# danihae/bio-image-unet

Hardware: AMD Instinct MI355X
Metric: voxels/sec fwd+bwd (higher is better)
Workload: dtype bf16; 1 GPU; cfg4: UNet3D(in_channels=1, out_channels=1, n_filter=32) input (4, 1, 128, 128, 128) per GPU, train step = forward + reference loss + backward + Adam; parallelism=dp1

## Files before the change

bio_image_unet_amd/_lib.py:

```python
from __future__ import annotations

import ctypes as C
import os

import torch

_HERE = os.path.dirname(os.path.abspath(__file__))
LIB_PATH = os.environ.get("BIU_LIB_PATH") or os.path.join(_HERE, "libbiu_hip.so")

BIU_F32, BIU_BF16 = 0, 1
BN_MAX_PARTIALS = 1024


class BiuError(RuntimeError):
    pass


class biu_act(C.Structure):
    _fields_ = [("p", C.c_void_p), ("n", C.c_int32), ("d", C.c_int32), ("h", C.c_int32), ("w", C.c_int32),
                ("c", C.c_int32), ("pitch", C.c_int32)]


class biu_pack_job(C.Structure):
    _fields_ = [("w", C.c_void_p), ("packed", C.c_void_p), ("transposed", C.c_int32), ("kind", C.c_int32), ("cin", C.c_int32),
                ("cout", C.c_int32), ("kd", C.c_int32), ("kh", C.c_int32), ("kw", C.c_int32), ("reserved", C.c_int32)]


class biu_xform(C.Structure):
    _fields_ = [("scale", C.c_void_p), ("shift", C.c_void_p), ("slope", C.c_void_p)]


class biu_mo2d_term(C.Structure):
    _fields_ = [("kind", C.c_int32), ("nb", C.c_int32), ("partial_off", C.c_longlong), ("numel", C.c_longlong), ("pixels", C.c_longlong),
                ("p0", C.c_float), ("p1", C.c_float), ("p2", C.c_float), ("weight", C.c_float)]


class biu_aug_params(C.Structure):
    _fields_ = [("flags", C.c_uint32), ("rot_k", C.c_uint32), ("blur_k", C.c_uint32), ("index", C.c_uint32), ("m", C.c_double * 6),
                ("alpha", C.c_float), ("beta", C.c_float), ("noise_a", C.c_float), ("noise_b", C.c_float),
                ("angle", C.c_float), ("scale", C.c_float), ("dx", C.c_float), ("dy", C.c_float)]


class biu_augf_params(C.Structure):
    _fields_ = [("flags", C.c_uint32), ("rot_k", C.c_uint32), ("blur_k", C.c_uint32), ("index", C.c_uint32), ("m", C.c_double * 6),
                ("cos_t", C.c_float), ("sin_t", C.c_float), ("alpha", C.c_float), ("beta", C.c_float), ("shot_s", C.c_float),
                ("gauss_sigma", C.c_float), ("angle", C.c_float), ("scale", C.c_float), ("dx", C.c_float), ("dy", C.c_float)]


_P = C.c_void_p
_A = C.POINTER(biu_act)
_X = C.POINTER(biu_xform)
_I = C.c_int
_F = C.c_float
_D = C.c_double
_Z = C.c_size_t

SIGNATURES = {
    "biu_last_error": (C.c_char_p, []),
    "biu_version": (_I, []),
    "biu_set_fp32_products": (_I, [_I]),
    "biu_set_fp32_products_3d": (_I, [_I]),
    "biu_conv_packed_bytes": (_Z, [_I, _I, _I, _I, _I, _I, _I, _I]),
    "biu_conv_pack": (_I, [_I, _P, _I, _I, _I, _I, _I, _I, _P, _P]),
    "biu_pack_batch": (_I, [_P, _I, _I, _P]),
    "biu_conv_split_workspace": (_Z, [_I, _A, _A, _I, _I, _I, _I, _I]),
    "biu_conv_fwd": (_I, [_A, _X, _P, _P, _P, _I, _I, _I, _I, _A, _P, _Z, _I, _P]),
    "biu_conv_fwd_stats_floats": (_Z, [_A, _I]),
    "biu_conv_fwd_stats": (_I, [_A, _X, _P, _P, _P, _I, _I, _I, _I, _A, _P, _Z, C.POINTER(C.c_int), _P, _Z, _I, _P]),
    "biu_conv_bwd_data": (_I, [_A, _P, _P, _I, _I, _I, _I, _A, _I, _P, _Z, _I, _P]),
    "biu_bwd_data_bnred_floats": (_Z, [_A, _I, _I]),
    "biu_conv_bwd_data_bnred": (_I, [_A, _P, _P, _I, _I, _I, _I, _A, _A, _P, _P, _P, _P, _P, _P, _Z, C.POINTER(C.c_int), _P, _Z, _I, _P]),
    "biu_convt_bwd_data_bnred": (_I, [_A, _P, _P, _I, _A, _A, _P, _P, _P, _P, _P, _P, _Z, C.POINTER(C.c_int), _I, _P]),
    "biu_conv_bwd_weight_workspace": (_Z, [_I, _I, _I, _I, _I, _I]),
    "biu_conv_bwd_weight": (_I, [_A, _X, _A, _I, _I, _I, _I, _P, _P, _P, _Z, _I, _P]),
    "biu_conv_bwd_weight_bn": (_I, [_A, _X, _A, _A, _P, _P, _P, _P, _P, _P, _I, _I, _I, _I, _P, _P, _Z, _I, _P]),
    "biu_bn_stats": (_I, [_A, _P, C.POINTER(C.c_int), _I, _P]),
    "biu_bn_finalize": (_I, [_P, _I, _I, _D, _P, _P, _P, _P, _F, _F, _P, _P, _P, _P, _P]),
    "biu_bn_eval_affine": (_I, [_I, _P, _P, _P, _P, _F, _P, _P, _P]),
    "biu_xform_apply": (_I, [_A, _X, _A, _I, _P]),
    "biu_bn_bwd_reduce": (_I, [_A, _A, _P, _P, _P, _P, _P, _P, C.POINTER(C.c_int), _I, _P]),
    "biu_bn_bwd_finalize": (_I, [_P, _I, _I, _D, _P, _P, _P, _P, _P, _P, _P, _P, _P]),
    "biu_bn_bwd_finalize_eval": (_I, [_P, _I, _I, _P, _P, _P, _P, _P, _P, _P, _P]),
    "biu_bn_bwd_apply": (_I, [_A, _A, _P, _P, _P, _P, _P, _P, _A, _I, _P]),
    "biu_maxpool_fwd": (_I, [_A, _X, _A, _I, _P]),
    "biu_maxpool_bwd": (_I, [_A, _X, _A, _A, _I, _I, _P]),
    "biu_maxpool_bwd_bnred": (_I, [_A, _X, _A, _A, _I, _P, _P, _P, _Z, C.POINTER(C.c_int), _I, _P]),
    "biu_nearest_down_fwd": (_I, [_A, _X, _A, _I, _P]),
    "biu_nearest_down_bwd": (_I, [_A, _A, _I, _I, _P]),
    "biu_nearest_up_fwd": (_I, [_A, _X, _A, _I, _P]),
    "biu_upconv_ok": (_I, [_A, _A, _I]),
    "biu_upconv_packed_bytes": (_Z, [_I, _I, _I, _I]),
    "biu_upconv_pack": (_I, [_I, _P, _I, _I, _I, _P, _P]),
    "biu_upconv_bwd_data": (_I, [_A, _P, _A, _I, _I, _P]),
    "biu_upconv_bwd_weight_workspace": (_Z, [_I, _I, _I]),
    "biu_upconv_bwd_weight_bn": (_I, [_A, _X, _A, _A, _P, _P, _P, _P, _P, _P, _P, _P, _Z, _I, _P]),
    "biu_upconv_fwd_stats_floats": (_Z, [_A, _A]),
    "biu_upconv_fwd": (_I, [_A, _X, _P, _P, _A, _P, _Z, C.POINTER(C.c_int), _I, _P]),
    "biu_nearest_up_bwd": (_I, [_A, _A, _I, _I, _P]),
    "biu_bce_dice_blocks": (_I, [C.c_longlong]),
    "biu_bce_dice_fwd": (_I, [_P, _P, _I, C.c_longlong, _P, _P]),
    "biu_bce_dice_bwd": (_I, [_P, _P, _I, C.c_longlong, _P, _P, _I, _P]),
    "biu_pair_smooth_l1_blocks": (_I, [C.c_longlong]),
    "biu_pair_smooth_l1_fwd": (_I, [_P, _I, C.c_longlong, _P, _P]),
    "biu_pair_smooth_l1_bwd": (_I, [_P, _I, C.c_longlong, _P, _P, _I, _P]),
    "biu_seg_loss_finish": (_I, [_P, _I, _I, C.c_longlong, _P, _I, _F, _F, _F, _I, _F, _F, _F, _I, _F, _P, _P]),
    "biu_seg_loss_coef": (_I, [_P, _P, _I, C.c_longlong, _F, _F, _F, _I, _F, _F, _F, _I, _F, _P, _P, _P]),
    "biu_head_dlogits": (_I, [_P, _P, _P, _I, _I, _I, C.c_longlong, _P, _I, _I, _P]),
    "biu_mo2d_loss_blocks": (_I, [C.c_longlong]),
    "biu_mo2d_loss_fwd": (_I, [_I, _F, _F, _P, _I, _P, _I, _I, _I, _I, _P, _P]),
    "biu_mo2d_loss_finish": (_I, [_P, _I, _P, _P, _P]),
    "biu_mo2d_loss_coef": (_I, [_P, _I, _P, _P, _P, _P]),
    "biu_mo2d_loss_bwd": (_I, [_I, _F, _F, _P, _I, _P, _I, _I, _I, _I, _P, _P, _P]),
    "biu_trilinear_up_fwd": (_I, [_A, _X, _A, _I, _P]),
    "biu_trilinear_up_bwd": (_I, [_A, _A, _I, _I, _P]),
    "biu_bilinear_up_fwd": (_I, [_A, _X, _A, _I, _P]),
    "biu_bilinear_up_bwd": (_I, [_A, _A, _I, _I, _P]),
    "biu_xcorr_fwd": (_I, [_A, _X, _A, _X, _A, _I, _P]),
    "biu_xcorr_bwd": (_I, [_A, _X, _A, _X, _A, _A, _A, _I, _I, _P]),
    "biu_conv_cat_ok": (_I, [_A, _A, _A, _I, _I, _I, _I, _I]),
    "biu_conv_fwd_cat": (_I, [_A, _X, _A, _X, _P, _P, _P, _I, _I, _I, _I, _A, _P, _Z, C.POINTER(C.c_int), _P, _Z, _I, _P]),
    "biu_conv_bwd_data_cat": (_I, [_A, _P, _P, _I, _I, _I, _I, _A, _I, _A, _I, _P, _Z, _I, _P]),
    "biu_conv_bwd_weight_cat": (_I, [_A, _X, _A, _X, _A, _A, _P, _P, _P, _P, _P, _P, _I, _I, _I, _I, _P, _P, _Z, _I, _P]),
    "biu_convt_packed_bytes": (_Z, [_I, _I, _I, _I, _I]),
    "biu_convt_pack": (_I, [_I, _P, _I, _I, _I, _I, _P, _P]),
    "biu_foldt_ok": (_I, [_A, _A, _A, _I]),
    "biu_foldt_packed_bytes": (_Z, [_I, _I, _I, _I]),
    "biu_foldt_pack": (_I, [_P, _P, _P, _P, _I, _I, _I, _I, _I, _P, _P]),
    "biu_foldt_fwd_stats_floats": (_Z, [_A, _A]),
    "biu_foldt_fwd_form": (_I, [_A, _A, _A, _I]),
    "biu_foldt_fwd": (_I, [_A, _X, _A, _X, _P, _A, _P, _Z, C.POINTER(C.c_int), _I, _P]),
    "biu_foldt_bwd_data_bnred_floats": (_Z, [_A]),
    "biu_foldt_bwd_data": (_I, [_A, _P, _A, _I, _A, _I, _A, _P, _P, _P, _P, _P, _P, _Z, C.POINTER(C.c_int), _P, _Z, _I, _P]),
    "biu_foldt_bwd_weight_workspace": (_Z, [_I, _I, _I, _I]),
    "biu_foldt_bwd_weight_bn": (_I, [_A, _X, _A, _X, _A, _A, _P, _P, _P, _P, _P, _P, _P, _P, _P, _P, _I, _P, _P, _P, _P, _Z, _I, _P]),
    "biu_foldt_bwd_weight_bn_phase": (_I, [_A, _X, _A, _X, _A, _A, _P, _P, _P, _P, _P, _P, _P, _P, _P, _P, _I, _P, _P, _P, _P, _Z, _I, _I, _P]),
    "biu_convt_fwd": (_I, [_A, _X, _P, _P, _P, _I, _A, _I, _P]),
    "biu_convt_bwd_data": (_I, [_A, _P, _P, _I, _A, _I, _I, _P]),
    "biu_convt_bwd_weight_workspace": (_Z, [_I, _I, _I, _I]),
    "biu_convt_bwd_weight": (_I, [_A, _X, _A, _I, _P, _P, _P, _Z, _I, _P]),
    "biu_head_fwd": (_I, [_A, _X, _P, _P, _I, _I, _P, _P, _I, _P]),
    "biu_head_bwd_workspace": (_Z, [_I]),
    "biu_head_bwd": (_I, [_A, _X, _P, _I, _P, _A, _P, _P, _P, _Z, _I, _P]),
    "biu_head_bwd_bnred": (_I, [_A, _X, _P, _I, _P, _A, _P, _P, _P, _Z, _P, _P, _P, _Z, C.POINTER(C.c_int), _I, _P]),
    "biu_max_join_fwd": (_I, [_A, _X, _A, _X, _A, _I, _P]),
    "biu_max_join_bwd": (_I, [_A, _X, _A, _X, _A, _A, _A, _I, _I, _P]),
    "biu_act_add": (_I, [_A, _A, _I, _I, _P]),
    "biu_add_relu_fwd": (_I, [_A, _X, _A, _X, _A, _I, _P]),
    "biu_add_relu_bwd": (_I, [_A, _A, _A, _A, _I, _I, _P]),
    "biu_gate_fwd": (_I, [_A, _X, _A, _X, _A, _I, _P]),
    "biu_gate_bwd": (_I, [_A, _X, _A, _X, _A, _A, _I, _A, _I, _P]),
    "biu_from_nchw": (_I, [_P, _A, _I, _P]),
    "biu_from_nchw_u8": (_I, [_P, _F, _A, _I, _P]),
    "biu_u8_to_f32": (_I, [_P, _F, _P, C.c_longlong, _P]),
    "biu_quantize_u8": (_I, [_P, _F, _P, C.c_longlong, _P]),
    "biu_stitch_add": (_I, [_P, _I, _P, _I, _I, _I, _I, _P, _P, _I, _I, _I, _I, _I, _I, _I, _P]),
    "biu_stitch_finish": (_I, [_P, _P, _I, _I, C.c_longlong, _P, _I, _P]),
    "biu_to_nchw": (_I, [_A, _X, _P, _I, _P]),
    "biu_augment_u8": (_I, [_P, _P, _I, _I, _I, _I, _I, _P, _I, _I, C.c_ulonglong, C.c_uint, C.c_uint, _P]),
    "biu_augment_f32": (_I, [_P, _I, _P, _I, _I, _I, _I, _I, _P, _I, C.c_ulonglong, C.c_uint, C.c_uint, _P]),
    "biu_philox_u32": (_I, [_P, C.c_longlong, C.c_ulonglong, C.c_uint, C.c_uint, C.c_uint, C.c_uint, _P]),
    "biu_adam_step": (_I, [_I, _P, _P, _P, _P, _P, _F, _F, _F, _F, _I, _F, _P]),
    "biu_adam_set_hyper": (_I, [_P, _F, _F, _F, _F, _I, _F, _P]),
    "biu_adam_step_hyper": (_I, [_I, _P, _P, _P, _P, _P, _P, _P]),
    "biu_grad_clip_scratch_floats": (_Z, [_I]),
    "biu_grad_clip": (_I, [_I, _P, _P, _F, _P, _Z, _P, _P]),
}


def _load():
    if not os.path.exists(LIB_PATH):
        raise ImportError(
            f"{LIB_PATH} is missing: the HIP kernels are not built. Run `python -c 'import __graft_entry__ as g; "
            f"g.build()'` from the repository root (needs hipcc). There is no CPU fallback.")
    lib = C.CDLL(LIB_PATH)
    for name, (res, args) in SIGNATURES.items():
        fn = getattr(lib, name)
        fn.restype = res
        fn.argtypes = args
    return lib


class _Lib:

    def __init__(self, cdll):
        object.__setattr__(self, "_c", cdll)
        object.__setattr__(self, "prof", None)
        object.__setattr__(self, "watch", None)
        object.__setattr__(self, "watched", [])
        object.__setattr__(self, "label", "")

    def __setattr__(self, k, v):
        object.__setattr__(self, k, v)

    def __getattr__(self, name):
        fn = getattr(self._c, name)
        if self.prof is None and self.watch is None:
            return fn
        if self.prof is None and self.watch != (name, self.label):
            return fn
        import torch

        def timed(*args):
            e0, e1 = torch.cuda.Event(enable_timing=True), torch.cuda.Event(enable_timing=True)
            e0.record()
            rc = fn(*args)
            e1.record()
            (self.prof if self.prof is not None else self.watched).append((name, self.label, e0, e1))
            return rc

        return timed


lib = _Lib(_load())


def check(status: int, what: str = ""):
    if status != 0:
        msg = lib.biu_last_error()
        raise BiuError(f"{what}: biu status {status}: {msg.decode() if msg else ''}")
```

bio_image_unet_amd/csrc/biu_api.hip:

```cpp
#include "biu_common.h"
#include "biu_internal.h"

#include <stdlib.h>
#include <string.h>

static const char* const kOffTokens[] = {
    "conv_fwd", "conv_dgrad", "conv_wgrad", "convt_fwd", "convt_dgrad", "convt_wgrad", "convt_all", "c1", "c1_mfma", "cat",
    "fused_stats", "wgrad_bn", "dgrad_bnred", "pool_pair", "pool_pipe", "pool_bnred", "head_bnred", "ksplit", "m16", "m16x2", "rr16",
    "wroll", "wroll16", "wroll2d", "upconv", "foldt", "foldall", "foldck8", "foldgemm", "croll", "froll", "prepack", "wsplitbn",
    "capturefork", "sidechain",
};
constexpr int kNumOffTokens = sizeof(kOffTokens) / sizeof(kOffTokens[0]);
static_assert(kNumOffTokens <= 64, "BiuEnv::off holds one bit per token");

static int off_index(const char* tok, size_t n) {
    for (int i = 0; i < kNumOffTokens; ++i)
        if (strlen(kOffTokens[i]) == n && strncmp(kOffTokens[i], tok, n) == 0) return i;
    return -1;
}
static void env_unknown(const char* var, const char* val, int n) {
    fprintf(stderr, "[biu] %s: unknown %s '%.*s' ignored\n", var, strcmp(var, "BIU_DISABLE") == 0 ? "token" : "value", n, val);
}
static bool parse_int(const char* s, int* v) {
    char* end = nullptr;
    const long r = strtol(s, &end, 10);
    if (end == s || *end) return false;
    *v = (int)r;
    return true;
}

const BiuEnv& biu_env() {
    static const BiuEnv env = [] {
        BiuEnv v{0, false, false, 0, 2, 0, 128};
        if (const char* p = getenv("BIU_DISABLE")) {
            while (true) {
                const size_t n = strcspn(p, ",");
                const int i = off_index(p, n);
                if (i >= 0) v.off |= 1ull << i;
                else if (n > 0) env_unknown("BIU_DISABLE", p, (int)n);
                if (!p[n]) break;
                p += n + 1;
            }
        }
        if (const char* e = getenv("BIU_ROLL"); e && *e) {
            if (strcmp(e, "always") == 0) v.roll_always = true;
            else env_unknown("BIU_ROLL", e, (int)strlen(e));
        }
        if (const char* e = getenv("BIU_FOLDT"); e && *e) {
            int n = 0;
            if (strcmp(e, "always") == 0) v.foldt_always = true;
            else if (strncmp(e, "cmax:", 5) == 0 && parse_int(e + 5, &n) && n > 0) v.foldt_cmax = n;
            else if (strcmp(e, "size") != 0) env_unknown("BIU_FOLDT", e, (int)strlen(e));
        }
        if (const char* e = getenv("BIU_FP32_PRODUCTS"); e && *e) {
            if (strcmp(e, "exact") == 0) v.fp32_products = 0;
            else if (strcmp(e, "bf16x3") == 0) v.fp32_products = 1;
            else if (strcmp(e, "bf16x6") != 0) env_unknown("BIU_FP32_PRODUCTS", e, (int)strlen(e));
        }
        if (const char* e = getenv("BIU_FP32_PRODUCTS_3D"); e && *e) {
            if (strcmp(e, "bf16x3") == 0) v.fp32_products_3d = 1;
            else if (strcmp(e, "bf16x6") == 0) v.fp32_products_3d = 2;
            else if (strcmp(e, "exact") != 0) env_unknown("BIU_FP32_PRODUCTS_3D", e, (int)strlen(e));
        }
        if (const char* e = getenv("BIU_FALL_MAXCA"); e && *e) {
            int n = 0;
            if (parse_int(e, &n)) v.fall_maxca = n;
            else env_unknown("BIU_FALL_MAXCA", e, (int)strlen(e));
        }
        return v;
    }();
    return env;
}

bool biu_off(const char* token) {
    const int i = off_index(token, strlen(token));
    return i >= 0 && ((biu_env().off >> i) & 1);
}

static void warn_slow_path(const char* op, const biu_act* x, const biu_act* y, int taps) {
    const double macs = (double)nvox(y) * x->c * y->c * taps;
    if (macs < 4e9) return;
    static int shown = 0;
    if (shown++ < 8)
        fprintf(stderr, "[biu] %s: %d->%d channels on %lld voxels takes the any-shape kernel (%.1f GMAC): expect it to be slow; "
                        "the MFMA path needs channel counts that are multiples of 8 (>= 16), dilation 1, 16-byte aligned slices "
                        "and samples under 4 GB\n", op, x->c, y->c, (long long)nvox(y), macs * 1e-9);
}

static bool conv_args_ok(const biu_act* x, const biu_act* y, int kd, int kh, int kw, int dil) {
    if (!valid_act(x) || !valid_act(y) || !same_space(x, y)) return false;
    if (!((kd == 1 || kd == 3) && kh == 3 && kw == 3) && !(kd == 1 && kh == 1 && kw == 1)) return false;
    return dil >= 1;
}

extern "C" size_t biu_conv_packed_bytes(int kind, int cin, int cout, int kd, int kh, int kw, int dilation, int dtype) {
    return biu_mfma_packed_bytes(kind, cin, cout, kd, kh, kw, dilation, dtype);
}

extern "C" int biu_conv_pack(int kind, const float* w, int cin, int cout, int kd, int kh, int kw, int dtype,
                             void* packed, biu_stream stream) {
    BIU_REQUIRE(w && packed, BIU_ERR_SHAPE, "conv_pack: null pointer");
    BIU_REQUIRE(biu_mfma_packed_bytes(kind, cin, cout, kd, kh, kw, 1, dtype) > 0, BIU_ERR_UNSUPPORTED,
                "conv_pack: shape (cin=%d, cout=%d, k=%dx%dx%d) is served by the direct kernels", cin, cout, kd, kh, kw);
    return biu_mfma_pack(kind, w, cin, cout, kd, kh, kw, dtype, packed, (hipStream_t)stream);
}

extern "C" int biu_pack_batch(const biu_pack_job* jobs, int n, int dtype, biu_stream stream) {
    BIU_REQUIRE(n >= 0 && (jobs || n == 0), BIU_ERR_SHAPE, "pack_batch: null job table");
    BIU_REQUIRE(n <= 65535, BIU_ERR_UNSUPPORTED, "pack_batch: more than 65535 jobs");
    return biu_mfma_pack_batch(jobs, n, dtype, (hipStream_t)stream);
}

static bool will_split(int cin, const biu_act* y, const biu_act* y1, int kd, int dtype, const void* ws, size_t ws_bytes) {
    const size_t need = biu_mfma_conv_split_bytes(cin, y, y1, kd, dtype);
    return need > 0 && ws && ws_bytes >= need;
}

extern "C" size_t biu_conv_split_workspace(int cin, const biu_act* y, const biu_act* y1, int kd, int kh, int kw, int dilation, int dtype) {
    if (!y || !valid_act(y) || (y1 && !valid_act(y1)) || kh != 3 || kw != 3 || (kd != 1 && kd != 3) || dilation != 1) return 0;
    biu_act xprobe = *y;
    xprobe.c = xprobe.pitch = cin;
    biu_act yall = *y;
    if (y1) yall.c = y->c + y1->c;
    if (!biu_mfma_conv_ok(&xprobe, &yall, kd, kh, kw, dilation, dtype)) return 0;
    return biu_mfma_conv_split_bytes(cin, y, y1, kd, dtype);
}

extern "C" int biu_conv_fwd_stats(const biu_act* x, const biu_xform* xf, const float* w, const void* packed,
                                  const float* bias, int kd, int kh, int kw, int dilation, const biu_act* y,
                                  float* bn_partial, size_t bn_partial_floats, int* bn_nblk, void* ws, size_t ws_bytes, int dtype,
                                  biu_stream stream) {
    BIU_REQUIRE(conv_args_ok(x, y, kd, kh, kw, dilation), BIU_ERR_SHAPE,
                "conv_fwd: x/y extents differ or unsupported kernel %dx%dx%d dil %d", kd, kh, kw, dilation);
    BIU_REQUIRE(w && bn_partial && bn_nblk, BIU_ERR_SHAPE, "conv_fwd_stats: null pointer");
    *bn_nblk = 0;
    if (!biu_off("c1") && !biu_off("fused_stats") && biu_c1m_ok(x, y, kd, kh, kw, dilation, dtype)) {
        const int nb = biu_c1m_fwd_rows(y, kd);
        if ((size_t)nb * y->c * 2 <= bn_partial_floats) {
            int rc = biu_c1m_fwd(x, xf, w, bias, kd, y, bn_partial, (hipStream_t)stream);
            if (rc == BIU_OK) *bn_nblk = nb;
            return rc;
        }
    }
    if (packed && !biu_off("conv_fwd") && !biu_off("fused_stats") && biu_mfma_conv_ok(x, y, kd, kh, kw, dilation, dtype) &&
        !will_split(x->c, y, nullptr, kd, dtype, ws, ws_bytes)) {
        const int nb = biu_mfma_conv_stat_rows(y, kd, x, dtype);
        if ((size_t)nb * y->c * 2 <= bn_partial_floats) {
            int rc = biu_mfma_conv(x, xf, packed, bias, kd, kh, kw, y, 0, bn_partial, dtype, (hipStream_t)stream);
            if (rc == BIU_OK) *bn_nblk = nb;
            return rc;
        }
    }
    int rc = biu_conv_fwd(x, xf, w, packed, bias, kd, kh, kw, dilation, y, ws, ws_bytes, dtype, stream);
    if (rc != BIU_OK) return rc;
    BIU_REQUIRE(bn_partial_floats >= (size_t)BIU_BN_MAX_PARTIALS * y->c * 2, BIU_ERR_WORKSPACE, "conv_fwd_stats: partial buffer too small");
    return biu_bn_stats(y, bn_partial, bn_nblk, dtype, stream);
}

extern "C" size_t biu_conv_fwd_stats_floats(const biu_act* y, int kd) {
    size_t a = (size_t)BIU_BN_MAX_PARTIALS * y->c * 2, b = (size_t)biu_mfma_conv_bricks(y, kd == 3 ? 3 : 1) * y->c * 2;
    return a > b ? a : b;
}

extern "C" int biu_conv_fwd(const biu_act* x, const biu_xform* xf, const float* w, const void* packed,
                            const float* bias, int kd, int kh, int kw, int dilation, const biu_act* y, void* ws, size_t ws_bytes,
                            int dtype, biu_stream stream) {
    BIU_REQUIRE(conv_args_ok(x, y, kd, kh, kw, dilation), BIU_ERR_SHAPE,
                "conv_fwd: x/y extents differ or unsupported kernel %dx%dx%d dil %d", kd, kh, kw, dilation);
    BIU_REQUIRE(w, BIU_ERR_SHAPE, "conv_fwd: null weight");
    if (!biu_off("c1") && biu_c1m_ok(x, y, kd, kh, kw, dilation, dtype))
        return biu_c1m_fwd(x, xf, w, bias, kd, y, nullptr, (hipStream_t)stream);
    if (!biu_off("c1") && biu_c1_conv_ok(x, y, kd, kh, kw, dilation, dtype))
        return biu_c1_conv_fwd(x, xf, w, bias, kd, y, dtype, (hipStream_t)stream);
    if (packed && !biu_off("conv_fwd") && biu_mfma_conv_ok(x, y, kd, kh, kw, dilation, dtype))
        return biu_mfma_conv(x, xf, packed, bias, kd, kh, kw, y, 0, nullptr, dtype, (hipStream_t)stream, nullptr, nullptr, ws, ws_bytes);
    warn_slow_path("conv_fwd", x, y, kd * kh * kw);
    return biu_conv_fwd_direct(x, xf, w, bias, kd, kh, kw, dilation, y, dtype, (hipStream_t)stream);
}

extern "C" int biu_conv_bwd_data(const biu_act* dy, const float* w, const void* packed, int kd, int kh, int kw,
                                 int dilation, const biu_act* dx, int accumulate, void* ws, size_t ws_bytes, int dtype, biu_stream stream) {
    BIU_REQUIRE(conv_args_ok(dy, dx, kd, kh, kw, dilation), BIU_ERR_SHAPE, "conv_bwd_data: dy/dx extents differ");
    BIU_REQUIRE(w, BIU_ERR_SHAPE, "conv_bwd_data: null weight");
    if (packed && !biu_off("conv_dgrad") && biu_mfma_conv_ok(dy, dx, kd, kh, kw, dilation, dtype))
        return biu_mfma_conv(dy, nullptr, packed, nullptr, kd, kh, kw, dx, accumulate, nullptr, dtype, (hipStream_t)stream, nullptr, nullptr, ws, ws_bytes);
    warn_slow_path("conv_bwd_data", dx, dy, kd * kh * kw);
    return biu_conv_bwd_data_direct(dy, w, kd, kh, kw, dilation, dx, accumulate, dtype, (hipStream_t)stream);
}

extern "C" size_t biu_bwd_data_bnred_floats(const biu_act* dx, int kd, int transposed) {
    size_t a = (size_t)BIU_BN_MAX_PARTIALS * dx->c * 2;
    size_t b = (size_t)(transposed ? biu_mfma_convt_dgrad_bricks(dx, kd) : biu_mfma_conv_bricks(dx, kd == 3 ? 3 : 1)) * dx->c * 2;
    return a > b ? a : b;
}
extern "C" int biu_conv_bwd_data_bnred(const biu_act* dy, const float* w, const void* packed, int kd, int kh, int kw, int dilation,
                                       const biu_act* dx, const biu_act* y_up, const float* scale, const float* shift,
                                       const float* slope, const float* mean, const float* invstd, float* partial,
                                       size_t partial_floats, int* nblk, void* ws, size_t ws_bytes, int dtype, biu_stream stream) {
    BIU_REQUIRE(conv_args_ok(dy, dx, kd, kh, kw, dilation) && valid_act(y_up) && same_space(y_up, dx) && y_up->c == dx->c, BIU_ERR_SHAPE,
                "conv_bwd_data_bnred: extents differ");
    BIU_REQUIRE(w && scale && shift && mean && invstd && partial && nblk, BIU_ERR_SHAPE, "conv_bwd_data_bnred: null pointer");
    const size_t es = dsize(dtype);
    const bool yok = ((uintptr_t)y_up->p % 16) == 0 && ((size_t)y_up->pitch * es) % 16 == 0;
    if (packed && yok && !biu_off("conv_dgrad") && !biu_off("dgrad_bnred") && biu_mfma_conv_ok(dy, dx, kd, kh, kw, dilation, dtype) &&
        !will_split(dy->c, dx, nullptr, kd, dtype, ws, ws_bytes)) {
        const int nb = biu_mfma_conv_stat_rows(dx, kd, dy, dtype, true);
        if ((size_t)nb * dx->c * 2 <= partial_floats) {
            BnRedFuse red{y_up, scale, shift, slope, mean, invstd};
            int rc = biu_mfma_conv(dy, nullptr, packed, nullptr, kd, kh, kw, dx, 0, partial, dtype, (hipStream_t)stream, &red);
            if (rc == BIU_OK) *nblk = nb;
            return rc;
        }
    }
    int rc = biu_conv_bwd_data(dy, w, packed, kd, kh, kw, dilation, dx, 0, ws, ws_bytes, dtype, stream);
    if (rc != BIU_OK) return rc;
    BIU_REQUIRE(partial_floats >= (size_t)BIU_BN_MAX_PARTIALS * dx->c * 2, BIU_ERR_WORKSPACE, "conv_bwd_data_bnred: partial buffer too small");
    return biu_bn_bwd_reduce(dx, y_up, scale, shift, slope, mean, invstd, partial, nblk, dtype, stream);
}
extern "C" int biu_convt_bwd_data_bnred(const biu_act* dy, const float* w, const void* packed, int kd, const biu_act* dx,
                                        const biu_act* y_up, const float* scale, const float* shift, const float* slope,
                                        const float* mean, const float* invstd, float* partial, size_t partial_floats, int* nblk,
                                        int dtype, biu_stream stream) {
    BIU_REQUIRE(valid_act(dx) && valid_act(dy) && w && biu_convt_shapes_ok(dx, dy, kd) && valid_act(y_up) && same_space(y_up, dx) &&
                    y_up->c == dx->c, BIU_ERR_SHAPE, "convt_bwd_data_bnred: extents differ");
    BIU_REQUIRE(scale && shift && mean && invstd && partial && nblk, BIU_ERR_SHAPE, "convt_bwd_data_bnred: null pointer");
    const size_t es = dsize(dtype);
    const bool yok = ((uintptr_t)y_up->p % 16) == 0 && ((size_t)y_up->pitch * es) % 16 == 0;
    if (packed && yok && !biu_off("convt_dgrad") && !biu_off("dgrad_bnred") && biu_mfma_convt_ok(1, dx, dy, kd, dtype) &&
        biu_convt_all_ok(dx, dy, kd, dtype)) {
        const int nb = biu_convt_all_dgrad_rows(dx, dy, kd);
        if ((size_t)nb * dx->c * 2 <= partial_floats) {
            BnRedFuse red{y_up, scale, shift, slope, mean, invstd};
            int rc = biu_convt_all_dgrad(dy, packed, kd, dx, 0, (hipStream_t)stream, partial, &red);
            if (rc == BIU_OK) *nblk = nb;
            return rc;
        }
    }
    if (packed && yok && !biu_off("convt_dgrad") && !biu_off("dgrad_bnred") && biu_mfma_convt_ok(1, dx, dy, kd, dtype)) {
        const int nb = biu_mfma_convt_dgrad_rows(dx, kd, dy->c, dtype);
        if ((size_t)nb * dx->c * 2 <= partial_floats) {
            BnRedFuse red{y_up, scale, shift, slope, mean, invstd};
            int rc = biu_mfma_convt_dgrad(dy, packed, kd, dx, 0, dtype, (hipStream_t)stream, partial, &red);
            if (rc == BIU_OK) *nblk = nb;
            return rc;
        }
    }
    int rc = biu_convt_bwd_data(dy, w, packed, kd, dx, 0, dtype, stream);
    if (rc != BIU_OK) return rc;
    BIU_REQUIRE(partial_floats >= (size_t)BIU_BN_MAX_PARTIALS * dx->c * 2, BIU_ERR_WORKSPACE, "convt_bwd_data_bnred: partial buffer too small");
    return biu_bn_bwd_reduce(dx, y_up, scale, shift, slope, mean, invstd, partial, nblk, dtype, stream);
}

extern "C" size_t biu_conv_bwd_weight_workspace(int cin, int cout, int kd, int kh, int kw, int dtype) {
    if (cin == 1 && kh == 3 && kw == 3) {
        const size_t a = biu_c1_wgrad_workspace(cout, kd), b = biu_c1m_wgrad_workspace(cout, kd);
        return a > b ? a : b;
    }
    return biu_mfma_wgrad_workspace(cin, cout, kd, kh, kw, dtype);
}

extern "C" int biu_conv_bwd_weight(const biu_act* x, const biu_xform* xf, const biu_act* dy, int kd, int kh, int kw,
                                   int dilation, float* dw, float* dbias, void* ws, size_t ws_bytes, int dtype,
                                   biu_stream stream) {
    BIU_REQUIRE(conv_args_ok(x, dy, kd, kh, kw, dilation), BIU_ERR_SHAPE, "conv_bwd_weight: x/dy extents differ");
    BIU_REQUIRE(dw, BIU_ERR_SHAPE, "conv_bwd_weight: null dw");
    if (!biu_off("c1") && biu_c1m_ok(x, dy, kd, kh, kw, dilation, dtype) && ws && ws_bytes >= biu_c1m_wgrad_workspace(dy->c, kd)) {
        int rc = biu_c1m_wgrad(x, xf, dy, nullptr, kd, dw, ws, ws_bytes, (hipStream_t)stream);
        if (rc == BIU_OK && dbias) rc = biu_chan_sum(dy, dbias, dtype, (hipStream_t)stream);
        return rc;
    }
    if (!biu_off("c1") && biu_c1_conv_ok(x, dy, kd, kh, kw, dilation, dtype) && ws && ws_bytes >= biu_c1_wgrad_workspace(dy->c, kd)) {
        int rc = biu_c1_conv_wgrad(x, xf, dy, kd, dw, ws, ws_bytes, dtype, (hipStream_t)stream);
        if (rc == BIU_OK && dbias) rc = biu_chan_sum(dy, dbias, dtype, (hipStream_t)stream);
        return rc;
    }
    if (!biu_off("conv_wgrad") && biu_mfma_wgrad_ok(x, dy, kd, kh, kw, dilation, dtype)) {
        BIU_REQUIRE(ws && ws_bytes >= biu_mfma_wgrad_workspace(x->c, dy->c, kd, kh, kw, dtype), BIU_ERR_WORKSPACE,
                    "conv_bwd_weight: workspace too small");
        return biu_mfma_wgrad(x, xf, dy, kd, kh, kw, dw, dbias, ws, ws_bytes, dtype, (hipStream_t)stream);
    }
    warn_slow_path("conv_bwd_weight", x, dy, kd * kh * kw);
    return biu_conv_bwd_weight_direct(x, xf, dy, kd, kh, kw, dilation, dw, dbias, dtype, (hipStream_t)stream);
}

extern "C" int biu_conv_bwd_weight_bn(const biu_act* x, const biu_xform* xf, const biu_act* da, const biu_act* y,
                                      const float* scale, const float* shift, const float* slope, const float* coefA,
                                      const float* coefB, const float* coefC, int kd, int kh, int kw, int dilation,
                                      float* dw, void* ws, size_t ws_bytes, int dtype, biu_stream stream) {
    BIU_REQUIRE(conv_args_ok(x, da, kd, kh, kw, dilation) && valid_act(y) && same_space(y, da) && y->c == da->c, BIU_ERR_SHAPE,
                "conv_bwd_weight_bn: extents differ");
    BIU_REQUIRE(dw && scale && shift && coefA && coefB && coefC, BIU_ERR_SHAPE, "conv_bwd_weight_bn: null pointer");
    const size_t es = dsize(dtype);
    const bool yok = ((uintptr_t)y->p % 16) == 0 && ((size_t)y->pitch * es) % 16 == 0 &&
                     (i64)y->d * y->h * y->w * y->pitch * (i64)es < (1LL << 32) - 65536;
    if (!biu_off("c1") && !biu_off("wgrad_bn") && yok && biu_c1m_ok(x, da, kd, kh, kw, dilation, dtype) && ws &&
        ws_bytes >= biu_c1m_wgrad_workspace(da->c, kd)) {
        BnBwdFuse bn{y, scale, shift, slope, coefA, coefB, coefC};
        return biu_c1m_wgrad(x, xf, da, &bn, kd, dw, ws, ws_bytes, (hipStream_t)stream);
    }
    if (!biu_off("conv_wgrad") && !biu_off("wgrad_bn") && yok && biu_mfma_wgrad_ok(x, da, kd, kh, kw, dilation, dtype)) {
        BIU_REQUIRE(ws && ws_bytes >= biu_mfma_wgrad_workspace(x->c, da->c, kd, kh, kw, dtype), BIU_ERR_WORKSPACE,
                    "conv_bwd_weight_bn: workspace too small");
        BnBwdFuse bn{y, scale, shift, slope, coefA, coefB, coefC};
        return biu_mfma_wgrad(x, xf, da, kd, kh, kw, dw, nullptr, ws, ws_bytes, dtype, (hipStream_t)stream, &bn);
    }
    int rc = biu_bn_bwd_apply(da, y, scale, shift, slope, coefA, coefB, coefC, da, dtype, stream);
    if (rc != BIU_OK) return rc;
    return biu_conv_bwd_weight(x, xf, da, kd, kh, kw, dilation, dw, nullptr, ws, ws_bytes, dtype, stream);
}

extern "C" int biu_conv_cat_ok(const biu_act* x0, const biu_act* x1, const biu_act* y, int kd, int kh, int kw, int dilation, int dtype) {
    if (!x0 || !x1 || !y || !valid_act(x0) || !valid_act(x1) || !valid_act(y) || !same_space(x0, y) || !same_space(x1, y)) return 0;
    if (biu_off("conv_fwd") || biu_off("conv_dgrad") || biu_off("conv_wgrad") || biu_off("cat")) return 0;
    return biu_mfma_conv_cat_ok(x0, x1, y, kd, kh, kw, dilation, dtype) ? 1 : 0;
}
extern "C" int biu_conv_fwd_cat(const biu_act* x0, const biu_xform* xf0, const biu_act* x1, const biu_xform* xf1, const float* w,
                                const void* packed, const float* bias, int kd, int kh, int kw, int dilation, const biu_act* y,
                                float* bn_partial, size_t bn_partial_floats, int* bn_nblk, void* ws, size_t ws_bytes, int dtype,
                                biu_stream stream) {
    BIU_REQUIRE(biu_conv_cat_ok(x0, x1, y, kd, kh, kw, dilation, dtype) && w && packed, BIU_ERR_UNSUPPORTED,
                "conv_fwd_cat: shapes not served by the two-source kernels (ask biu_conv_cat_ok)");
    ConvCat cat{x1, xf1, nullptr, 0};
    if (bn_partial && will_split(x0->c + x1->c, y, nullptr, kd, dtype, ws, ws_bytes)) {
        BIU_REQUIRE(bn_nblk, BIU_ERR_SHAPE, "conv_fwd_cat: null bn_nblk");
        int rc = biu_mfma_conv(x0, xf0, packed, bias, kd, kh, kw, y, 0, nullptr, dtype, (hipStream_t)stream, nullptr, &cat, ws, ws_bytes);
        if (rc != BIU_OK) return rc;
        BIU_REQUIRE(bn_partial_floats >= (size_t)BIU_BN_MAX_PARTIALS * y->c * 2, BIU_ERR_WORKSPACE, "conv_fwd_cat: partial buffer too small");
        return biu_bn_stats(y, bn_partial, bn_nblk, dtype, stream);
    }
    if (bn_partial) {
        BIU_REQUIRE(bn_nblk, BIU_ERR_SHAPE, "conv_fwd_cat: null bn_nblk");
        const int nb = dtype == BIU_F32 ? biu_mfma_conv_stat_rows(y, kd, x0, dtype, false, x0->c + x1->c) : biu_mfma_conv_stat_rows(y, kd);
        BIU_REQUIRE((size_t)nb * y->c * 2 <= bn_partial_floats, BIU_ERR_WORKSPACE, "conv_fwd_cat: partial buffer too small");
        int rc = biu_mfma_conv(x0, xf0, packed, bias, kd, kh, kw, y, 0, bn_partial, dtype, (hipStream_t)stream, nullptr, &cat);
        if (rc == BIU_OK) *bn_nblk = nb;
        return rc;
    }
    return biu_mfma_conv(x0, xf0, packed, bias, kd, kh, kw, y, 0, nullptr, dtype, (hipStream_t)stream, nullptr, &cat, ws, ws_bytes);
}
extern "C" int biu_conv_bwd_data_cat(const biu_act* dy, const float* w, const void* packed, int kd, int kh, int kw, int dilation,
                                     const biu_act* dx0, int accumulate0, const biu_act* dx1, int accumulate1, void* ws, size_t ws_bytes,
                                     int dtype, biu_stream stream) {
    BIU_REQUIRE(biu_conv_cat_ok(dx0, dx1, dy, kd, kh, kw, dilation, dtype) && w && packed, BIU_ERR_UNSUPPORTED,
                "conv_bwd_data_cat: shapes not served by the two-source kernels (ask biu_conv_cat_ok)");
    ConvCat cat{nullptr, nullptr, dx1, accumulate1};
    return biu_mfma_conv(dy, nullptr, packed, nullptr, kd, kh, kw, dx0, accumulate0, nullptr, dtype, (hipStream_t)stream, nullptr, &cat, ws, ws_bytes);
}
extern "C" int biu_conv_bwd_weight_cat(const biu_act* x0, const biu_xform* xf0, const biu_act* x1, const biu_xform* xf1,
                                       const biu_act* da, const biu_act* y, const float* scale, const float* shift,
                                       const float* slope, const float* coefA, const float* coefB, const float* coefC, int kd,
                                       int kh, int kw, int dilation, float* dw, void* ws, size_t ws_bytes, int dtype,
                                       biu_stream stream) {
    BIU_REQUIRE(biu_conv_cat_ok(x0, x1, da, kd, kh, kw, dilation, dtype) && dw, BIU_ERR_UNSUPPORTED,
                "conv_bwd_weight_cat: shapes not served by the two-source kernels (ask biu_conv_cat_ok)");
    BIU_REQUIRE(ws && ws_bytes >= biu_mfma_wgrad_workspace(x0->c + x1->c, da->c, kd, kh, kw, dtype), BIU_ERR_WORKSPACE,
                "conv_bwd_weight_cat: workspace too small");
    if (y) {
        const size_t es = dsize(dtype);
        BIU_REQUIRE(valid_act(y) && same_space(y, da) && y->c == da->c && scale && shift && coefA && coefB && coefC, BIU_ERR_SHAPE,
                    "conv_bwd_weight_cat: BatchNorm operands missing");
        BIU_REQUIRE(((uintptr_t)y->p % 16) == 0 && ((size_t)y->pitch * es) % 16 == 0 && (i64)y->d * y->h * y->w * y->pitch * (i64)es < (1LL << 32) - 65536,
                    BIU_ERR_UNSUPPORTED, "conv_bwd_weight_cat: y alignment / size");
        BnBwdFuse bn{y, scale, shift, slope, coefA, coefB, coefC};
        return biu_mfma_wgrad(x0, xf0, da, kd, kh, kw, dw, nullptr, ws, ws_bytes, dtype, (hipStream_t)stream, &bn, x1, xf1);
    }
    return biu_mfma_wgrad(x0, xf0, da, kd, kh, kw, dw, nullptr, ws, ws_bytes, dtype, (hipStream_t)stream, nullptr, x1, xf1);
}

extern "C" size_t biu_convt_packed_bytes(int kind, int cin, int cout, int kd, int dtype) {
    return biu_mfma_convt_packed_bytes(kind, cin, cout, kd, dtype);
}
extern "C" int biu_convt_pack(int kind, const float* w, int cin, int cout, int kd, int dtype, void* packed, biu_stream stream) {
    BIU_REQUIRE(w && packed, BIU_ERR_SHAPE, "convt_pack: null pointer");
    return biu_mfma_convt_pack(kind, w, cin, cout, kd, dtype, packed, (hipStream_t)stream);
}
extern "C" int biu_upconv_ok(const biu_act* x, const biu_act* y, int dtype) {
    return (x && y && !biu_off("upconv") && biu_mfma_upconv_ok(x, y, dtype)) ? 1 : 0;
}
extern "C" size_t biu_upconv_packed_bytes(int kind, int cin, int cout, int dtype) { return biu_mfma_upconv_packed_bytes(kind, cin, cout, dtype); }
extern "C" int biu_upconv_pack(int kind, const float* w, int cin, int cout, int dtype, void* packed, biu_stream stream) {
    BIU_REQUIRE(w && packed && biu_mfma_upconv_packed_bytes(kind, cin, cout, dtype) > 0, BIU_ERR_SHAPE,
                "upconv_pack: null pointer, kind %d or unsupported channels %d -> %d", kind, cin, cout);
    return biu_mfma_upconv_pack(kind, w, cin, cout, dtype, packed, (hipStream_t)stream);
}
extern "C" size_t biu_upconv_bwd_weight_workspace(int cin, int cout, int dtype) { return biu_mfma_upconv_wgrad_workspace(cin, cout, dtype); }
extern "C" int biu_upconv_bwd_weight_bn(const biu_act* x, const biu_xform* xf, const biu_act* da, const biu_act* y, const float* scale,
                                        const float* shift, const float* slope, const float* coefA, const float* coefB, const float* coefC,
                                        float* dw, void* ws, size_t ws_bytes, int dtype, biu_stream stream) {
    BIU_REQUIRE(x && da && dw && ws, BIU_ERR_SHAPE, "upconv_bwd_weight_bn: null pointer");
    BIU_REQUIRE(biu_mfma_upconv_ok(x, da, dtype) && biu_mfma_upconv_wgrad_workspace(x->c, da->c, dtype) > 0, BIU_ERR_UNSUPPORTED,
                "upconv_bwd_weight_bn: shape %dx%dx%dx%d c%d / %dx%dx%dx%d c%d is not served by the folded kernel", x->n, x->d, x->h, x->w, x->c,
                da->n, da->d, da->h, da->w, da->c);
    if (y) {
        BIU_REQUIRE(valid_act(y) && same_space(y, da) && y->c == da->c && scale && shift && coefA && coefB && coefC, BIU_ERR_SHAPE,
                    "upconv_bwd_weight_bn: y / coefficient vectors do not match da");
        const size_t es = dsize(dtype);
        BIU_REQUIRE(((uintptr_t)y->p % 16) == 0 && ((size_t)y->pitch * es) % 16 == 0 && (i64)y->d * y->h * y->w * y->pitch * (i64)es < (1LL << 32) - 65536,
                    BIU_ERR_UNSUPPORTED, "upconv_bwd_weight_bn: y is not 16-byte aligned or a sample exceeds 4 GB");
        BnBwdFuse bn{y, scale, shift, slope, coefA, coefB, coefC};
        return biu_mfma_upconv_wgrad(x, xf, da, dw, ws, ws_bytes, dtype, (hipStream_t)stream, &bn);
    }
    return biu_mfma_upconv_wgrad(x, xf, da, dw, ws, ws_bytes, dtype, (hipStream_t)stream, nullptr);
}
extern "C" int biu_upconv_bwd_data(const biu_act* dy, const void* packed, const biu_act* dx, int accumulate, int dtype, biu_stream stream) {
    BIU_REQUIRE(dy && dx && packed, BIU_ERR_SHAPE, "upconv_bwd_data: null pointer");
    BIU_REQUIRE(biu_mfma_upconv_ok(dx, dy, dtype) && biu_mfma_upconv_packed_bytes(1, dx->c, dy->c, dtype) > 0, BIU_ERR_UNSUPPORTED,
                "upconv_bwd_data: shape %dx%dx%dx%d c%d <- %dx%dx%dx%d c%d is not served by the folded kernel", dx->n, dx->d, dx->h, dx->w, dx->c,
                dy->n, dy->d, dy->h, dy->w, dy->c);
    return biu_mfma_upconv_dgrad(dy, packed, dx, accumulate, dtype, (hipStream_t)stream);
}
extern "C" size_t biu_upconv_fwd_stats_floats(const biu_act* x, const biu_act* y) {
    return (size_t)biu_mfma_upconv_stat_rows(x, y) * y->c * 2;
}
extern "C" int biu_upconv_fwd(const biu_act* x, const biu_xform* xf, const void* packed, const float* bias, const biu_act* y,
                              float* bn_partial, size_t bn_partial_floats, int* bn_nblk, int dtype, biu_stream stream) {
    BIU_REQUIRE(x && y && packed, BIU_ERR_SHAPE, "upconv_fwd: null pointer");
    BIU_REQUIRE(biu_mfma_upconv_ok(x, y, dtype), BIU_ERR_UNSUPPORTED, "upconv_fwd: shape %dx%dx%dx%d c%d -> %dx%dx%dx%d c%d is not served by the folded kernel",
                x->n, x->d, x->h, x->w, x->c, y->n, y->d, y->h, y->w, y->c);
    if (bn_nblk) *bn_nblk = 0;
    if (bn_partial) {
        BIU_REQUIRE(bn_nblk, BIU_ERR_SHAPE, "upconv_fwd: bn_partial without bn_nblk");
        const int nb = biu_mfma_upconv_stat_rows(x, y);
        BIU_REQUIRE((size_t)nb * y->c * 2 <= bn_partial_floats, BIU_ERR_WORKSPACE, "upconv_fwd: partial buffer too small (%zu floats, need %zu)",
                    bn_partial_floats, (size_t)nb * y->c * 2);
        int rc = biu_mfma_upconv_fwd(x, xf, packed, bias, y, bn_partial, dtype, (hipStream_t)stream);
        if (rc == BIU_OK) *bn_nblk = nb;
        return rc;
    }
    return biu_mfma_upconv_fwd(x, xf, packed, bias, y, nullptr, dtype, (hipStream_t)stream);
}

extern "C" int biu_foldt_ok(const biu_act* x_low, const biu_act* skip, const biu_act* y, int dtype) {
    if (!(x_low && skip && y) || biu_off("foldt") || !biu_mfma_foldt_ok(x_low, skip, y, dtype)) return 0;
    const BiuEnv& env = biu_env();
    if (env.foldt_cmax > 0) return x_low->c <= env.foldt_cmax ? 1 : 0;
    return (env.foldt_always || biu_mfma_foldt_worth(x_low, y)) ? 1 : 0;
}
extern "C" size_t biu_foldt_packed_bytes(int cin_low, int cskip, int cout, int dtype) { return biu_mfma_foldt_packed_bytes(cin_low, cskip, cout, dtype); }
extern "C" int biu_foldt_pack(const float* w_conv, const float* b_conv, const float* w_t, const float* b_t, int cin_low, int cup, int cskip, int cout,
                              int dtype, void* packed, biu_stream stream) {
    BIU_REQUIRE(w_conv && w_t && packed && cin_low > 0 && cup > 0 && cskip > 0 && cout > 0, BIU_ERR_SHAPE, "foldt_pack: null pointer or empty shape");
    return biu_mfma_foldt_pack(w_conv, b_conv, w_t, b_t, cin_low, cup, cskip, cout, dtype, packed, (hipStream_t)stream);
}
extern "C" int biu_foldt_fwd_form(const biu_act* x_low, const biu_act* skip, const biu_act* y, int dtype) {
    if (!x_low || !skip || !y) return 0;
    return biu_mfma_foldt_form(x_low, skip, y, dtype);
}
extern "C" size_t biu_foldt_fwd_stats_floats(const biu_act* x_low, const biu_act* y) {
    const size_t a = (size_t)biu_mfma_foldt_stat_rows(x_low, y) * y->c * 2, b = (size_t)1024 * y->c * 2;
    return a > b ? a : b;
}
extern "C" int biu_foldt_fwd(const biu_act* x_low, const biu_xform* xf_low, const biu_act* skip, const biu_xform* xf_skip, const void* packed,
                             const biu_act* y, float* bn_partial, size_t bn_partial_floats, int* bn_nblk, int dtype, biu_stream stream) {
    BIU_REQUIRE(x_low && skip && y && packed, BIU_ERR_SHAPE, "foldt_fwd: null pointer");
    BIU_REQUIRE(biu_mfma_foldt_ok(x_low, skip, y, dtype), BIU_ERR_UNSUPPORTED, "foldt_fwd: shapes are not served by the folded kernels");
    if (bn_nblk) *bn_nblk = 0;
    if (bn_partial) {
        BIU_REQUIRE(bn_nblk, BIU_ERR_SHAPE, "foldt_fwd: bn_partial without bn_nblk");
        const int nb = biu_mfma_foldt_stat_rows(x_low, y, skip, dtype);
        BIU_REQUIRE((size_t)nb * y->c * 2 <= bn_partial_floats, BIU_ERR_WORKSPACE, "foldt_fwd: partial buffer too small");
        int rc = biu_mfma_foldt_fwd(x_low, xf_low, skip, xf_skip, packed, y, bn_partial, dtype, (hipStream_t)stream);
        if (rc == BIU_OK) *bn_nblk = nb;
        return rc;
    }
    return biu_mfma_foldt_fwd(x_low, xf_low, skip, xf_skip, packed, y, nullptr, dtype, (hipStream_t)stream);
}

extern "C" size_t biu_foldt_bwd_data_bnred_floats(const biu_act* dx_low) { return (size_t)biu_mfma_upconv_dgrad_rows(dx_low) * dx_low->c * 2; }
extern "C" int biu_foldt_bwd_data(const biu_act* dy, const void* packed, const biu_act* dx_low, int acc_low, const biu_act* dskip, int acc_skip,
                                  const biu_act* y_low, const float* scale, const float* shift, const float* slope, const float* mean,
                                  const float* invstd, float* partial, size_t partial_floats, int* nblk, void* ws, size_t ws_bytes, int dtype,
                                  biu_stream stream) {
    BIU_REQUIRE(dy && packed && dx_low && dskip, BIU_ERR_SHAPE, "foldt_bwd_data: null pointer");
    BIU_REQUIRE(biu_mfma_foldt_ok(dx_low, dskip, dy, dtype), BIU_ERR_UNSUPPORTED, "foldt_bwd_data: shapes are not served by the folded kernels");
    if (nblk) *nblk = 0;
    if (y_low) {
        BIU_REQUIRE(!acc_low && valid_act(y_low) && same_space(y_low, dx_low) && y_low->c == dx_low->c && scale && shift && mean && invstd && partial && nblk,
                    BIU_ERR_SHAPE, "foldt_bwd_data: fused reduction needs acc_low = 0, y_low like dx_low and its vectors");
        const int nb = biu_mfma_upconv_dgrad_rows(dx_low);
        BIU_REQUIRE((size_t)nb * dx_low->c * 2 <= partial_floats, BIU_ERR_WORKSPACE, "foldt_bwd_data: partial buffer too small");
        BnRedFuse red{y_low, scale, shift, slope, mean, invstd};
        int rc = biu_mfma_foldt_dgrad(dy, packed, dx_low, 0, dskip, acc_skip, dtype, (hipStream_t)stream, partial, &red, ws, ws_bytes);
        if (rc == BIU_OK) *nblk = nb;
        return rc;
    }
    return biu_mfma_foldt_dgrad(dy, packed, dx_low, acc_low, dskip, acc_skip, dtype, (hipStream_t)stream, nullptr, nullptr, ws, ws_bytes);
}
extern "C" size_t biu_foldt_bwd_weight_workspace(int cin_low, int cskip, int cout, int dtype) { return biu_mfma_foldt_wgrad_workspace(cin_low, cskip, cout, dtype); }
extern "C" int biu_foldt_bwd_weight_bn_phase(const biu_act* x_low, const biu_xform* xf_low, const biu_act* skip, const biu_xform* xf_skip, const biu_act* da,
                                             const biu_act* y, const float* scale, const float* shift, const float* slope, const float* coefA,
                                             const float* coefB, const float* coefC, const float* dy_sum, const float* w_conv, const float* w_t, const float* b_t,
                                             int cup, float* dw_conv, float* dw_t, float* db_t, void* ws, size_t ws_bytes, int dtype, int phases, biu_stream stream) {
    BIU_REQUIRE(phases >= 1 && phases <= 7, BIU_ERR_SHAPE, "foldt_bwd_weight_bn: phases is a mask of 1 (skip half, da -> dy), 4 (G), 2 (border sums + chain rule)");
    BIU_REQUIRE(x_low && skip && da && w_conv && w_t && dw_conv && dw_t && ws && cup > 0, BIU_ERR_SHAPE, "foldt_bwd_weight_bn: null pointer");
    BIU_REQUIRE(biu_mfma_foldt_ok(x_low, skip, da, dtype) && biu_mfma_wgrad_ok(skip, da, 3, 3, 3, 1, dtype), BIU_ERR_UNSUPPORTED,
                "foldt_bwd_weight_bn: shapes are not served by the folded kernels");
    BIU_REQUIRE(y || dy_sum || !(b_t || db_t), BIU_ERR_UNSUPPORTED,
                "foldt_bwd_weight_bn: a plain dy (y = NULL) needs dy_sum, its per-channel sum over all voxels (it is zero only behind a train-mode BatchNorm)");
    if (y) {
        BIU_REQUIRE(valid_act(y) && same_space(y, da) && y->c == da->c && scale && shift && coefA && coefB && coefC, BIU_ERR_SHAPE,
                    "foldt_bwd_weight_bn: y / coefficient vectors do not match da");
        const size_t es = dsize(dtype);
        const bool yok = ((uintptr_t)y->p % 16) == 0 && ((size_t)y->pitch * es) % 16 == 0 &&
                         (i64)y->d * y->h * y->w * y->pitch * (i64)es < (1LL << 32) - 65536;
        if (!yok) {
            int rc = (phases & 1) ? biu_bn_bwd_apply(da, y, scale, shift, slope, coefA, coefB, coefC, da, dtype, stream) : BIU_OK;
            if (rc != BIU_OK) return rc;
            return biu_mfma_foldt_wgrad(x_low, xf_low, skip, xf_skip, da, nullptr, dy_sum, w_conv, w_t, b_t, cup, dw_conv, dw_t, db_t, ws, ws_bytes, dtype,
                                        (hipStream_t)stream, phases);
        }
        BnBwdFuse bn{y, scale, shift, slope, coefA, coefB, coefC};
        return biu_mfma_foldt_wgrad(x_low, xf_low, skip, xf_skip, da, &bn, dy_sum, w_conv, w_t, b_t, cup, dw_conv, dw_t, db_t, ws, ws_bytes, dtype, (hipStream_t)stream, phases);
    }
    return biu_mfma_foldt_wgrad(x_low, xf_low, skip, xf_skip, da, nullptr, dy_sum, w_conv, w_t, b_t, cup, dw_conv, dw_t, db_t, ws, ws_bytes, dtype, (hipStream_t)stream, phases);
}

extern "C" int biu_foldt_bwd_weight_bn(const biu_act* x_low, const biu_xform* xf_low, const biu_act* skip, const biu_xform* xf_skip, const biu_act* da,
                                       const biu_act* y, const float* scale, const float* shift, const float* slope, const float* coefA,
                                       const float* coefB, const float* coefC, const float* dy_sum, const float* w_conv, const float* w_t, const float* b_t,
                                       int cup, float* dw_conv, float* dw_t, float* db_t, void* ws, size_t ws_bytes, int dtype, biu_stream stream) {
    return biu_foldt_bwd_weight_bn_phase(x_low, xf_low, skip, xf_skip, da, y, scale, shift, slope, coefA, coefB, coefC, dy_sum, w_conv, w_t, b_t, cup, dw_conv, dw_t,
                                         db_t, ws, ws_bytes, dtype, 7, stream);
}

extern "C" int biu_convt_fwd(const biu_act* x, const biu_xform* xf, const float* w, const void* packed, const float* bias,
                             int kd, const biu_act* y, int dtype, biu_stream stream) {
    BIU_REQUIRE(valid_act(x) && valid_act(y) && w && biu_convt_shapes_ok(x, y, kd), BIU_ERR_SHAPE,
                "convt_fwd: output must be 2x the input extent (kd=%d)", kd);
    if (packed && !biu_off("convt_fwd") && biu_mfma_convt_ok(0, x, y, kd, dtype)) {
        if (biu_convt_all_ok(x, y, kd, dtype)) return biu_convt_all_fwd(x, xf, packed, bias, kd, y, (hipStream_t)stream);
        return biu_mfma_convt_fwd(x, xf, packed, bias, kd, y, dtype, (hipStream_t)stream);
    }
    return biu_convt_fwd_direct(x, xf, w, bias, kd, y, dtype, (hipStream_t)stream);
}
extern "C" int biu_convt_bwd_data(const biu_act* dy, const float* w, const void* packed, int kd, const biu_act* dx,
                                  int accumulate, int dtype, biu_stream stream) {
    BIU_REQUIRE(valid_act(dx) && valid_act(dy) && w && biu_convt_shapes_ok(dx, dy, kd), BIU_ERR_SHAPE,
                "convt_bwd_data: dy must be 2x the dx extent (kd=%d)", kd);
    if (packed && !biu_off("convt_dgrad") && biu_mfma_convt_ok(1, dx, dy, kd, dtype)) {
        if (biu_convt_all_ok(dx, dy, kd, dtype)) return biu_convt_all_dgrad(dy, packed, kd, dx, accumulate, (hipStream_t)stream);
        return biu_mfma_convt_dgrad(dy, packed, kd, dx, accumulate, dtype, (hipStream_t)stream);
    }
    return biu_convt_bwd_data_direct(dy, w, kd, dx, accumulate, dtype, (hipStream_t)stream);
}
extern "C" size_t biu_convt_bwd_weight_workspace(int cin, int cout, int kd, int dtype) {
    return biu_mfma_wgrad_workspace(cin, cout, kd, 2, 2, dtype);
}
extern "C" int biu_convt_bwd_weight(const biu_act* x, const biu_xform* xf, const biu_act* dy, int kd, float* dw,
                                    float* dbias, void* ws, size_t ws_bytes, int dtype, biu_stream stream) {
    BIU_REQUIRE(valid_act(x) && valid_act(dy) && dw && biu_convt_shapes_ok(x, dy, kd), BIU_ERR_SHAPE,
                "convt_bwd_weight: dy must be 2x the x extent (kd=%d)", kd);
    if (!biu_off("convt_wgrad") && biu_mfma_convt_wgrad_ok(x, dy, kd, dtype)) {
        BIU_REQUIRE(ws && ws_bytes >= biu_mfma_wgrad_workspace(x->c, dy->c, kd, 2, 2, dtype), BIU_ERR_WORKSPACE,
                    "convt_bwd_weight: workspace too small");
        return biu_mfma_convt_wgrad(x, xf, dy, kd, dw, dbias, ws, ws_bytes, dtype, (hipStream_t)stream);
    }
    return biu_convt_bwd_weight_direct(x, xf, dy, kd, dw, dbias, dtype, (hipStream_t)stream);
}
```

bio_image_unet_amd/csrc/biu_c1.hip:

```cpp
#include "biu_internal.h"
#include <stdlib.h>
#include <string.h>

namespace {

typedef float floatx16 __attribute__((ext_vector_type(16)));
typedef __bf16 bf16x8 __attribute__((ext_vector_type(8)));
typedef __bf16 bf16x4 __attribute__((ext_vector_type(4)));
typedef unsigned u32x2 __attribute__((ext_vector_type(2)));

constexpr int ROWB = 80;

struct C1Args {
    const char* x; int xpitch;
    char* y; int ypitch;
    const char* yraw; int yrawpitch;
    const float* w;
    const float* bias;
    const float* xs; const float* xb; const float* xl;
    int N, D, H, W, co0, cout;
    int nbd, nbh, nbw, nbricks;
    float* partial;
    int ctot;
    const float* bn_scale; const float* bn_shift; const float* bn_slope; const float* bn_cA; const float* bn_cB; const float* bn_cC;
};

__device__ __forceinline__ unsigned pack2(float a, float b) {
    typedef __bf16 bf2 __attribute__((ext_vector_type(2)));
    const bf2 p = {(__bf16)a, (__bf16)b};
    return __builtin_bit_cast(unsigned, p);
}
__device__ __forceinline__ void unpack8(const uint4& v, float* f) {
    const unsigned u[4] = {v.x, v.y, v.z, v.w};
#pragma unroll
    for (int i = 0; i < 4; ++i) { f[2 * i] = __uint_as_float(u[i] << 16); f[2 * i + 1] = __uint_as_float(u[i] & 0xffff0000u); }
}
__device__ __forceinline__ float bf2f(unsigned short u) { return __uint_as_float((unsigned)u << 16); }

template <int KD, int HALF = 0> struct Geo {
    static constexpr int TD = (KD == 3) ? (HALF ? 1 : 2) : 1, TH = (KD == 3) ? 8 : (HALF ? 8 : 16), TW = 32;
    static constexpr int BV = TD * TH * TW;
    static constexpr int HD = TD + KD - 1, HH = TH + 2, HW = TW + 2;
    static constexpr int HV = HD * HH * HW;
    static constexpr int TAPS = KD * 9;
};

template <int KD, int NTHR, int HALF = 0>
struct XpRegs { unsigned short v[(Geo<KD, HALF>::HV + NTHR - 1) / NTHR]; unsigned inside; };

template <int KD, int NTHR, int HALF = 0>
__device__ __forceinline__ void xp_request(const C1Args& a, int n, int d0, int h0, int w0, XpRegs<KD, NTHR, HALF>& xr) {
    using G = Geo<KD, HALF>;
    constexpr int NX = (G::HV + NTHR - 1) / NTHR;
    const int tid = threadIdx.x;
    xr.inside = 0;
#pragma unroll
    for (int k = 0; k < NX; ++k) {
        const int i = tid + NTHR * k;
        const int hw = i % G::HW, t = i / G::HW;
        const int hh = t % G::HH, hd = t / G::HH;
        const int gd = d0 + hd - (KD == 3 ? 1 : 0), gh = h0 + hh - 1, gw = w0 + hw - 1;
        const bool ok = i < G::HV && gd >= 0 && gd < a.D && gh >= 0 && gh < a.H && gw >= 0 && gw < a.W;
        xr.v[k] = ok ? *(const unsigned short*)(a.x + ((size_t)(((size_t)n * a.D + gd) * a.H + gh) * a.W + gw) * a.xpitch * 2) : (unsigned short)0;
        xr.inside |= ok ? (1u << k) : 0u;
    }
}
template <int KD, int NTHR, int HALF = 0>
__device__ __forceinline__ void xp_commit(const C1Args& a, const XpRegs<KD, NTHR, HALF>& xr, unsigned short* lx, char* lxp) {
    using G = Geo<KD, HALF>;
    constexpr int NX = (G::HV + NTHR - 1) / NTHR;
    const int tid = threadIdx.x;
    const bool has_xf = a.xs != nullptr;
    const float xs = has_xf ? a.xs[0] : 1.f, xb = has_xf ? a.xb[0] : 0.f, xl = has_xf ? a.xl[0] : 1.f;
#pragma unroll
    for (int k = 0; k < NX; ++k) {
        const int i = tid + NTHR * k;
        if (i < G::HV) {
            unsigned short v = xr.v[k];
            if (has_xf && ((xr.inside >> k) & 1u)) {
                const float tt = fmaf(xs, bf2f(v), xb);
                const float o = tt > 0.f ? tt : xl * tt;
                v = (unsigned short)(pack2(o, 0.f) & 0xffffu);
            }
            lx[i] = v;
        }
    }
    __syncthreads();
    for (int v = tid; v < G::BV; v += NTHR) {
        const int lw = v % G::TW, t = v / G::TW;
        const int lh = t % G::TH, ld = t / G::TH;
        unsigned short val[32];
#pragma unroll
        for (int tap = 0; tap < 32; ++tap) {
            if (tap < G::TAPS) {
                const int ta = tap / 9, tb = (tap / 3) % 3, tc = tap % 3;
                val[tap] = lx[((ld + ta) * G::HH + (lh + tb)) * G::HW + (lw + tc)];
            } else {
                val[tap] = 0;
            }
        }
        uint4* dst = (uint4*)(lxp + v * ROWB);
#pragma unroll
        for (int q = 0; q < 4; ++q)
            dst[q] = make_uint4(val[8 * q] | ((unsigned)val[8 * q + 1] << 16), val[8 * q + 2] | ((unsigned)val[8 * q + 3] << 16),
                                val[8 * q + 4] | ((unsigned)val[8 * q + 5] << 16), val[8 * q + 6] | ((unsigned)val[8 * q + 7] << 16));
    }
    __syncthreads();
}

template <int KD, int NQ >
__global__ __launch_bounds__(256) void k_c1_fwd_mfma(C1Args a) {
    using G = Geo<KD>;
    __shared__ __attribute__((aligned(16))) char smem[G::BV * ROWB + G::HV * 2 + 16 + 4 * 64 * 4 + 32 * 4];
    char* lxp = smem;
    unsigned short* lx = (unsigned short*)(smem + G::BV * ROWB);
    float* lred = (float*)(smem + G::BV * ROWB + ((G::HV * 2 + 15) & ~15));
    float* lbias = lred + 4 * 64;
    const int tid = threadIdx.x, lane = tid & 63, wave = tid >> 6, r = lane & 31, hf = lane >> 5;
    lred[tid] = 0.f;
    if (tid < 32) lbias[tid] = (a.bias && tid < a.cout) ? a.bias[a.co0 + tid] : 0.f;
    uint4 wf[2];
#pragma unroll
    for (int ks = 0; ks < 2; ++ks) {
        float f[8];
#pragma unroll
        for (int e = 0; e < 8; ++e) {
            const int tap = 16 * ks + 8 * hf + e;
            f[e] = (r < a.cout && tap < G::TAPS) ? a.w[(size_t)(a.co0 + r) * G::TAPS + tap] : 0.f;
        }
        wf[ks] = make_uint4(pack2(f[0], f[1]), pack2(f[2], f[3]), pack2(f[4], f[5]), pack2(f[6], f[7]));
    }
    float s1[NQ][8], s2[NQ][8];
#pragma unroll
    for (int q = 0; q < NQ; ++q)
#pragma unroll
        for (int e = 0; e < 8; ++e) s1[q][e] = s2[q][e] = 0.f;
    __syncthreads();

    auto origin_of = [&](int brick, int& n, int& d0, int& h0, int& w0) {
        int b = brick;
        w0 = (b % a.nbw) * G::TW; b /= a.nbw;
        h0 = (b % a.nbh) * G::TH; b /= a.nbh;
        d0 = (b % a.nbd) * G::TD;
        n = b / a.nbd;
    };
    XpRegs<KD, 256> xr;
    if ((int)blockIdx.x < a.nbricks) { int n, d0, h0, w0; origin_of(blockIdx.x, n, d0, h0, w0); xp_request<KD, 256>(a, n, d0, h0, w0, xr); }
    for (int brick = blockIdx.x; brick < a.nbricks; brick += gridDim.x) {
        int n, d0, h0, w0;
        origin_of(brick, n, d0, h0, w0);
        xp_commit<KD, 256>(a, xr, lx, lxp);
        if (brick + (int)gridDim.x < a.nbricks) { int n2, d2, h2, w2; origin_of(brick + gridDim.x, n2, d2, h2, w2); xp_request<KD, 256>(a, n2, d2, h2, w2, xr); }
        for (int tile = wave; tile < G::BV / 32; tile += 4) {
            const int v = tile * 32 + r;
            floatx16 acc;
#pragma unroll
            for (int e = 0; e < 16; ++e) acc[e] = lbias[8 * (e >> 2) + 4 * hf + (e & 3)];
#pragma unroll
            for (int ks = 0; ks < 2; ++ks) {
                const uint4 bx = *(const uint4*)(lxp + v * ROWB + (16 * ks + 8 * hf) * 2);
                acc = __builtin_amdgcn_mfma_f32_32x32x16_bf16(__builtin_bit_cast(bf16x8, wf[ks]), __builtin_bit_cast(bf16x8, bx), acc, 0, 0, 0);
            }
            const int lw = v % G::TW, t = v / G::TW;
            const int gd = d0 + t / G::TH, gh = h0 + t % G::TH, gw = w0 + lw;
            const bool vok = gd < a.D && gh < a.H && gw < a.W;
            char* orow = a.y + ((size_t)(((size_t)n * a.D + gd) * a.H + gh) * a.W + gw) * a.ypitch * 2;
#pragma unroll
            for (int q = 0; q < NQ; ++q) {
                unsigned a0 = pack2(acc[8 * q + 0], acc[8 * q + 1]), a1 = pack2(acc[8 * q + 2], acc[8 * q + 3]);
                unsigned b0 = pack2(acc[8 * q + 4], acc[8 * q + 5]), b1 = pack2(acc[8 * q + 6], acc[8 * q + 7]);
                const u32x2 r0 = __builtin_amdgcn_permlane32_swap(a0, b0, false, false);
                const u32x2 r1 = __builtin_amdgcn_permlane32_swap(a1, b1, false, false);
                const uint4 piece = make_uint4(r0[0], r1[0], r0[1], r1[1]);
                const int c = 16 * q + 8 * hf;
                if (vok && c < a.cout) {
                    *(uint4*)(orow + (size_t)(a.co0 + c) * 2) = piece;
                    float f[8];
                    unpack8(piece, f);
#pragma unroll
                    for (int e = 0; e < 8; ++e) { s1[q][e] += f[e]; s2[q][e] = fmaf(f[e], f[e], s2[q][e]); }
                }
            }
        }
        __syncthreads();
    }
    if (a.partial) {
#pragma unroll
        for (int q = 0; q < NQ; ++q)
#pragma unroll
            for (int e = 0; e < 8; ++e) {
                float u = s1[q][e], w_ = s2[q][e];
#pragma unroll
                for (int o = 16; o > 0; o >>= 1) { u += __shfl_xor(u, o, 64); w_ += __shfl_xor(w_, o, 64); }
                if (r == 0) { lred[wave * 64 + 2 * (16 * q + 8 * hf + e)] = u; lred[wave * 64 + 2 * (16 * q + 8 * hf + e) + 1] = w_; }
            }
        __syncthreads();
        if (tid < a.cout) {
            float* dst = a.partial + ((size_t)blockIdx.x * a.ctot + a.co0 + tid) * 2;
            dst[0] = (lred[2 * tid] + lred[64 + 2 * tid]) + (lred[128 + 2 * tid] + lred[192 + 2 * tid]);
            dst[1] = (lred[2 * tid + 1] + lred[64 + 2 * tid + 1]) + (lred[128 + 2 * tid + 1] + lred[192 + 2 * tid + 1]);
        }
    }
}

template <int KD>
__global__ __launch_bounds__(256, 3) void k_c1_wgrad_mfma(C1Args a) {
    using G = Geo<KD, 1>;
    constexpr int NTHR = 256, NWV = 4;
    extern __shared__ __attribute__((aligned(16))) char smem[];
    char* lxp = smem;
    char* ldy = smem + G::BV * ROWB;
    unsigned short* lx = (unsigned short*)(ldy + G::BV * ROWB);
    float* lacc = (float*)((char*)lx + ((G::HV * 2 + 15) & ~15));
    const int tid = threadIdx.x, lane = tid & 63, wave = tid >> 6;
    const bool fused = a.yraw != nullptr;
    const int ppv = a.cout / 8;
    const int mypiece = tid % 4;
    float ks[8], kh[8], kl[8], ka[8], kb[8], kc[8];
    if (fused && mypiece < ppv) {
#pragma unroll
        for (int e = 0; e < 8; ++e) {
            const int c = a.co0 + mypiece * 8 + e;
            ks[e] = a.bn_scale[c]; kh[e] = a.bn_shift[c]; kl[e] = a.bn_slope ? a.bn_slope[c] : 1.f;
            ka[e] = a.bn_cA[c]; kb[e] = a.bn_cB[c]; kc[e] = a.bn_cC[c];
        }
    }
    for (int i = tid; i < 32 * 32; i += NTHR) lacc[i] = 0.f;
    floatx16 acc;
#pragma unroll
    for (int e = 0; e < 16; ++e) acc[e] = 0.f;
    const int g = lane >> 4, li = lane & 15, qrow = li >> 2, p = li & 3, cg = g & 1, h = g >> 1;
    const int tr_lane = (8 * h + qrow) * ROWB + (16 * cg + 4 * p) * 2;

    constexpr int NPC = G::BV * 4 / NTHR;
    uint4 pda[NPC], pyr[NPC];
    size_t pvox[NPC];
    unsigned pmask = 0;
    auto origin = [&](int brick, int& n, int& d0, int& h0, int& w0) {
        int b = brick;
        w0 = (b % a.nbw) * G::TW; b /= a.nbw;
        h0 = (b % a.nbh) * G::TH; b /= a.nbh;
        d0 = (b % a.nbd) * G::TD;
        n = b / a.nbd;
    };
    auto request = [&](int brick) {
        int n, d0, h0, w0;
        origin(brick, n, d0, h0, w0);
        pmask = 0;
#pragma unroll
        for (int k = 0; k < NPC; ++k) {
            const int v = (tid + NTHR * k) / 4;
            const int lw = v % G::TW, t = v / G::TW;
            const int gd = d0 + t / G::TH, gh = h0 + t % G::TH, gw = w0 + lw;
            pda[k] = make_uint4(0, 0, 0, 0);
            pyr[k] = make_uint4(0, 0, 0, 0);
            if (mypiece < ppv && gd < a.D && gh < a.H && gw < a.W) {
                const size_t vox = (((size_t)n * a.D + gd) * a.H + gh) * a.W + gw;
                pvox[k] = vox;
                pda[k] = *(const uint4*)(a.y + (vox * a.ypitch + a.co0 + mypiece * 8) * 2);
                if (fused) pyr[k] = *(const uint4*)(a.yraw + (vox * a.yrawpitch + a.co0 + mypiece * 8) * 2);
                pmask |= 1u << k;
            }
        }
    };
    XpRegs<KD, NTHR, 1> xr;
    if ((int)blockIdx.x < a.nbricks) {
        request(blockIdx.x);
        int n0, d00, h00, w00;
        origin(blockIdx.x, n0, d00, h00, w00);
        xp_request<KD, NTHR, 1>(a, n0, d00, h00, w00, xr);
    }
    for (int brick = blockIdx.x; brick < a.nbricks; brick += gridDim.x) {
        int n, d0, h0, w0;
        origin(brick, n, d0, h0, w0);
#pragma unroll
        for (int k = 0; k < NPC; ++k) {
            const int v = (tid + NTHR * k) / 4;
            uint4 out = pda[k];
            if (fused && ((pmask >> k) & 1u)) {
                float gg[8], yy[8];
                unpack8(out, gg);
                unpack8(pyr[k], yy);
#pragma unroll
                for (int e = 0; e < 8; ++e) {
                    const float dz = gg[e] * (fmaf(ks[e], yy[e], kh[e]) > 0.f ? 1.f : kl[e]);
                    gg[e] = fmaf(ka[e], dz, fmaf(kb[e], yy[e], kc[e]));
                }
                out = make_uint4(pack2(gg[0], gg[1]), pack2(gg[2], gg[3]), pack2(gg[4], gg[5]), pack2(gg[6], gg[7]));
                *(uint4*)(a.y + (pvox[k] * a.ypitch + a.co0 + mypiece * 8) * 2) = out;
            }
            *(uint4*)(ldy + v * ROWB + mypiece * 16) = out;
        }
        xp_commit<KD, NTHR, 1>(a, xr, lx, lxp);
        if (brick + (int)gridDim.x < a.nbricks) {
            request(brick + gridDim.x);
            int n2, d2, h2, w2;
            origin(brick + gridDim.x, n2, d2, h2, w2);
            xp_request<KD, NTHR, 1>(a, n2, d2, h2, w2, xr);
        }
        typedef bf16x4 __attribute__((address_space(3))) * lp;
        for (int ksx = wave; ksx < G::BV / 16; ksx += NWV) {
            const char* ap = lxp + ksx * 16 * ROWB + tr_lane;
            const char* bp = ldy + ksx * 16 * ROWB + tr_lane;
            const bf16x4 a0 = __builtin_amdgcn_ds_read_tr16_b64_v4bf16((lp)(ap));
            const bf16x4 a1 = __builtin_amdgcn_ds_read_tr16_b64_v4bf16((lp)(ap + 4 * ROWB));
            const bf16x4 b0 = __builtin_amdgcn_ds_read_tr16_b64_v4bf16((lp)(bp));
            const bf16x4 b1 = __builtin_amdgcn_ds_read_tr16_b64_v4bf16((lp)(bp + 4 * ROWB));
            acc = __builtin_amdgcn_mfma_f32_32x32x16_bf16(__builtin_shufflevector(a0, a1, 0, 1, 2, 3, 4, 5, 6, 7),
                                                          __builtin_shufflevector(b0, b1, 0, 1, 2, 3, 4, 5, 6, 7), acc, 0, 0, 0);
        }
        __syncthreads();
    }
    {
        const int j = lane & 31, hf = lane >> 5;
#pragma unroll
        for (int e = 0; e < 16; ++e) atomicAdd(&lacc[((e & 3) + 8 * (e >> 2) + 4 * hf) * 32 + j], acc[e]);
    }
    __syncthreads();
    for (int i = tid; i < G::TAPS * a.cout; i += NTHR) {
        const int tap = i / a.cout, co = i % a.cout;
        a.partial[(size_t)blockIdx.x * (G::TAPS * a.cout) + i] = lacc[tap * 32 + co];
    }
}

__global__ void k_c1m_finalize(const float* __restrict__ partial, int nblk, int taps, int cout, int co0, float* __restrict__ dw) {
    __shared__ double red[256];
    const int o = blockIdx.x;
    double s = 0;
    for (int b = threadIdx.x; b < nblk; b += 256) s += partial[(size_t)b * (taps * cout) + o];
    red[threadIdx.x] = s;
    __syncthreads();
    for (int st = 128; st > 0; st >>= 1) {
        if (threadIdx.x < st) red[threadIdx.x] += red[threadIdx.x + st];
        __syncthreads();
    }
    if (threadIdx.x == 0) dw[(size_t)(co0 + o % cout) * taps + o / cout] = (float)red[0];
}

int cus() {
    static int n = 0;
    if (!n) {
        hipDeviceProp_t p;
        int dev = 0;
        if (hipGetDevice(&dev) == hipSuccess && hipGetDeviceProperties(&p, dev) == hipSuccess) n = p.multiProcessorCount;
        if (n <= 0) n = 256;
    }
    return n;
}

template <int KD, int HALF = 0> void bricks_of(C1Args& a) {
    using G = Geo<KD, HALF>;
    a.nbd = (a.D + G::TD - 1) / G::TD; a.nbh = (a.H + G::TH - 1) / G::TH; a.nbw = (a.W + G::TW - 1) / G::TW;
    a.nbricks = a.N * a.nbd * a.nbh * a.nbw;
}

}

bool biu_c1m_ok(const biu_act* x, const biu_act* y, int kd, int kh, int kw, int dil, int dtype) {
    if (biu_off("c1_mfma") || dtype != BIU_BF16 || x->c != 1 || dil != 1 || kh != 3 || kw != 3 || (kd != 1 && kd != 3)) return false;
    if (y->c % 16 != 0 || y->c < 16) return false;
    if ((uintptr_t)y->p % 16 || (y->pitch * 2) % 16 || (uintptr_t)x->p % 2) return false;
    return nvox(y) < (1LL << 31);
}

int biu_c1m_fwd_rows(const biu_act* y, int kd) {
    C1Args a{};
    a.N = y->n; a.D = y->d; a.H = y->h; a.W = y->w;
    if (kd == 3) bricks_of<3>(a); else bricks_of<1>(a);
    const int g = 3 * cus();
    return g < a.nbricks ? g : a.nbricks;
}

int biu_c1m_fwd(const biu_act* x, const biu_xform* xf, const float* w, const float* bias, int kd, const biu_act* y, float* bn_partial, hipStream_t st) {
    C1Args a{};
    a.x = (const char*)x->p; a.xpitch = x->pitch; a.y = (char*)y->p; a.ypitch = y->pitch; a.w = w; a.bias = bias;
    if (xf && (xf->scale || xf->shift || xf->slope)) {
        BIU_REQUIRE(xf->scale && xf->shift && xf->slope, BIU_ERR_UNSUPPORTED, "c1 conv: partial biu_xform");
        a.xs = xf->scale; a.xb = xf->shift; a.xl = xf->slope;
    }
    a.N = y->n; a.D = y->d; a.H = y->h; a.W = y->w; a.ctot = y->c; a.partial = bn_partial;
    const int rows = biu_c1m_fwd_rows(y, kd);
    if (kd == 3) bricks_of<3>(a); else bricks_of<1>(a);
    for (int co0 = 0; co0 < y->c;) {
        const int chunk = (y->c - co0) >= 32 ? 32 : 16;
        a.co0 = co0; a.cout = chunk;
        if (kd == 3) { if (chunk == 32) hipLaunchKernelGGL((k_c1_fwd_mfma<3, 2>), dim3(rows), dim3(256), 0, st, a); else hipLaunchKernelGGL((k_c1_fwd_mfma<3, 1>), dim3(rows), dim3(256), 0, st, a); }
        else { if (chunk == 32) hipLaunchKernelGGL((k_c1_fwd_mfma<1, 2>), dim3(rows), dim3(256), 0, st, a); else hipLaunchKernelGGL((k_c1_fwd_mfma<1, 1>), dim3(rows), dim3(256), 0, st, a); }
        co0 += chunk;
    }
    BIU_CHECK_LAUNCH("c1_fwd_mfma");
    return BIU_OK;
}

size_t biu_c1m_wgrad_workspace(int cout, int kd) { return (size_t)3 * cus() * kd * 9 * 32 * sizeof(float); }

int biu_c1m_wgrad(const biu_act* x, const biu_xform* xf, const biu_act* da, const BnBwdFuse* bn, int kd, float* dw, void* ws, size_t ws_bytes,
                  hipStream_t st) {
    BIU_REQUIRE(ws && ws_bytes >= biu_c1m_wgrad_workspace(da->c, kd), BIU_ERR_WORKSPACE, "c1_wgrad_mfma: workspace too small");
    C1Args a{};
    if (xf && (xf->scale || xf->shift || xf->slope)) {
        BIU_REQUIRE(xf->scale && xf->shift && xf->slope, BIU_ERR_UNSUPPORTED, "c1 conv: partial biu_xform");
        a.xs = xf->scale; a.xb = xf->shift; a.xl = xf->slope;
    }
    a.x = (const char*)x->p; a.xpitch = x->pitch; a.y = (char*)da->p; a.ypitch = da->pitch;
    a.N = da->n; a.D = da->d; a.H = da->h; a.W = da->w; a.partial = (float*)ws; a.ctot = da->c;
    if (bn) {
        a.yraw = (const char*)bn->y->p; a.yrawpitch = bn->y->pitch;
        a.bn_scale = bn->scale; a.bn_shift = bn->shift; a.bn_slope = bn->slope; a.bn_cA = bn->cA; a.bn_cB = bn->cB; a.bn_cC = bn->cC;
    }
    const int taps = kd * 9;
    if (kd == 3) bricks_of<3, 1>(a); else bricks_of<1, 1>(a);
    int grid = 3 * cus();
    if (grid > a.nbricks) grid = a.nbricks;
    const size_t hv = kd == 3 ? (size_t)Geo<3, 1>::HV : (size_t)Geo<1, 1>::HV;
    const size_t lds = (size_t)2 * 256 * ROWB + ((hv * 2 + 15) & ~(size_t)15) + 32 * 32 * sizeof(float);
    for (int co0 = 0; co0 < da->c;) {
        const int chunk = (da->c - co0) >= 32 ? 32 : 16;
        a.co0 = co0; a.cout = chunk;
        if (kd == 3) hipLaunchKernelGGL(k_c1_wgrad_mfma<3>, dim3(grid), dim3(256), lds, st, a);
        else hipLaunchKernelGGL(k_c1_wgrad_mfma<1>, dim3(grid), dim3(256), lds, st, a);
        BIU_CHECK_LAUNCH("c1_wgrad_mfma");
        hipLaunchKernelGGL(k_c1m_finalize, dim3(taps * chunk), dim3(256), 0, st, (const float*)ws, grid, taps, chunk, co0, dw);
        BIU_CHECK_LAUNCH("c1_wgrad_mfma_finalize");
        co0 += chunk;
    }
    return BIU_OK;
}
```

bio_image_unet_amd/csrc/biu_internal.h:

```cpp
#pragma once
#include "biu_common.h"

struct BiuEnv {
    unsigned long long off;
    bool roll_always;
    bool foldt_always;
    int foldt_cmax;
    int fp32_products;
    int fp32_products_3d;
    int fall_maxca;
};
const BiuEnv& biu_env();
bool biu_off(const char* token);

#define BIU_HIDDEN __attribute__((visibility("hidden")))
extern "C" BIU_HIDDEN int biu_conv_fwd_direct(const biu_act* x, const biu_xform* xf, const float* w, const float* bias, int kd,
                                   int kh, int kw, int dil, const biu_act* y, int dtype, hipStream_t st);
extern "C" BIU_HIDDEN int biu_conv_bwd_data_direct(const biu_act* dy, const float* w, int kd, int kh, int kw, int dil,
                                        const biu_act* dx, int accumulate, int dtype, hipStream_t st);
extern "C" BIU_HIDDEN int biu_conv_bwd_weight_direct(const biu_act* x, const biu_xform* xf, const biu_act* dy, int kd, int kh,
                                          int kw, int dil, float* dw, float* dbias, int dtype, hipStream_t st);
extern "C" BIU_HIDDEN int biu_convt_fwd_direct(const biu_act* x, const biu_xform* xf, const float* w, const float* bias, int kd,
                                    const biu_act* y, int dtype, hipStream_t st);
extern "C" BIU_HIDDEN int biu_convt_bwd_data_direct(const biu_act* dy, const float* w, int kd, const biu_act* dx, int accumulate,
                                         int dtype, hipStream_t st);
extern "C" BIU_HIDDEN int biu_convt_bwd_weight_direct(const biu_act* x, const biu_xform* xf, const biu_act* dy, int kd, float* dw,
                                           float* dbias, int dtype, hipStream_t st);
int biu_chan_sum(const biu_act* a, float* out, int dtype, hipStream_t st);
bool biu_convt_shapes_ok(const biu_act* lo, const biu_act* hi, int kd);

size_t biu_mfma_packed_bytes(int kind, int cin, int cout, int kd, int kh, int kw, int dilation, int dtype);
int biu_mfma_pack(int kind, const float* w, int cin, int cout, int kd, int kh, int kw, int dtype, void* packed,
                  hipStream_t st);
bool biu_mfma_conv_ok(const biu_act* x, const biu_act* y, int kd, int kh, int kw, int dilation, int dtype);
struct BnRedFuse {
    const biu_act* y;
    const float *scale, *shift, *slope, *mean, *invstd;
};
bool biu_mfma_conv_cat_ok(const biu_act* x0, const biu_act* x1, const biu_act* y, int kd, int kh, int kw, int dilation, int dtype);
struct ConvCat {
    const biu_act* x1; const biu_xform* xf1;
    const biu_act* y1; int accumulate1;
};
int biu_mfma_conv(const biu_act* x, const biu_xform* xf, const void* packed, const float* bias, int kd, int kh, int kw,
                  const biu_act* y, int accumulate, float* bn_partial, int dtype, hipStream_t st, const BnRedFuse* red = nullptr,
                  const ConvCat* cat = nullptr, void* split_ws = nullptr, size_t split_ws_bytes = 0);
bool biu_conv_roll_ok(const biu_act* x, const biu_act* y, int dtype, bool has_cat, int accumulate, bool red);
int biu_conv_roll_mshape(const biu_act* x, const biu_act* y, int dtype);
int biu_conv_roll_rows(const biu_act* x, const biu_act* y, int dtype);
int biu_conv_roll(const biu_act* x, const biu_xform* xf, const void* packed, const float* bias, const biu_act* y, float* bn_partial, const BnRedFuse* red,
                  hipStream_t st, int accumulate = 0);
bool biu_fold_roll_ok(const biu_act* x_low, const biu_act* y, int dtype);
int biu_fold_roll(const biu_act* x_low, const biu_xform* xf, const void* packed_fwd, const float* bias_sum, const float* fix, const biu_act* y, hipStream_t st);
size_t biu_fold_gemm_layout_floats(int cin_low, int cup, int cout);
bool biu_fold_gemm_ok(int cin_low, int cup, int cout);
int biu_fold_gemm_layouts(const float* w_conv, int ccat, int cup, int cout, const float* w_t, int cin_low, float* layouts, hipStream_t st);
int biu_fold_gemm_compose(const float* layouts, int cin_low, int cup, int cout, const float* b_t, float* wfold, float* wb, hipStream_t st);
int biu_fold_gemm_chain(const float* G, size_t slice_f, const float* layouts, int cin_low, int cup, int cout, int ccat, float* dw_conv, float* dw_t,
                        const float* b_t, const float* Sk, hipStream_t st);
size_t biu_mfma_conv_split_bytes(int cin, const biu_act* y, const biu_act* y1, int kd, int dtype);
int biu_mfma_convt_dgrad_bricks(const biu_act* dx, int kd);
int biu_mfma_convt_dgrad_rows(const biu_act* dx, int kd, int cdy, int dtype);
int biu_mfma_pack_batch(const biu_pack_job* jobs_device, int n, int dtype, hipStream_t st);
int biu_mfma_set_fp32_products(int mode);
int biu_mfma_set_fp32_products_3d(int mode);
int biu_mfma_conv_ksplit(int cin, const biu_act* y, int kd, int dtype);
int biu_mfma_conv_stat_rows(const biu_act* y, int kd, const biu_act* x = nullptr, int dtype = -1, bool red = false, int cin = -1);
int biu_mfma_conv_bricks(const biu_act* y, int kd, const biu_act* x = nullptr, int dtype = -1, int cin = -1);
size_t biu_mfma_wgrad_workspace(int cin, int cout, int kd, int kh, int kw, int dtype);
bool biu_mfma_wgrad_ok(const biu_act* x, const biu_act* dy, int kd, int kh, int kw, int dilation, int dtype);
struct BnBwdFuse {
    const biu_act* y;
    const float *scale, *shift, *slope, *cA, *cB, *cC;
};
int biu_mfma_wgrad(const biu_act* x, const biu_xform* xf, const biu_act* dy, int kd, int kh, int kw, float* dw,
                   float* dbias, void* ws, size_t ws_bytes, int dtype, hipStream_t st, const BnBwdFuse* bn = nullptr,
                   const biu_act* x1 = nullptr, const biu_xform* xf1 = nullptr, int dw_ld_cols = 0, int dw_c_off = 0);

size_t biu_mfma_convt_packed_bytes(int kind, int cin, int cout, int kd, int dtype);
int biu_mfma_convt_pack(int kind, const float* w, int cin, int cout, int kd, int dtype, void* packed, hipStream_t st);
bool biu_mfma_upconv_ok(const biu_act* x, const biu_act* y, int dtype);
size_t biu_mfma_upconv_packed_bytes(int kind, int cin, int cout, int dtype);
int biu_mfma_upconv_pack(int kind, const float* w, int cin, int cout, int dtype, void* packed, hipStream_t st, const float* wf = nullptr);
int biu_mfma_upconv_dgrad_rows(const biu_act* dx);
int biu_mfma_upconv_dgrad(const biu_act* dy, const void* packed, const biu_act* dx, int accumulate, int dtype, hipStream_t st, float* bn_partial = nullptr,
                          const BnRedFuse* red = nullptr);
struct BnBwdFuse;
size_t biu_mfma_upconv_wgrad_workspace(int cin, int cout, int dtype);
int biu_mfma_upconv_wgrad(const biu_act* x, const biu_xform* xf, const biu_act* dy, float* dw, void* ws, size_t ws_bytes, int dtype,
                          hipStream_t st, const BnBwdFuse* bn);
int biu_mfma_upconv_stat_rows(const biu_act* x, const biu_act* y);
int biu_mfma_upconv_fwd(const biu_act* x, const biu_xform* xf, const void* packed, const float* bias, const biu_act* y, float* bn_partial,
                        int dtype, hipStream_t st, int accumulate = 0);
bool biu_mfma_foldt_ok(const biu_act* x_low, const biu_act* skip, const biu_act* y, int dtype);
bool biu_mfma_foldt_worth(const biu_act* x_low, const biu_act* y);
size_t biu_mfma_foldt_packed_bytes(int cin_low, int cskip, int cout, int dtype);
int biu_mfma_foldt_pack(const float* w_conv, const float* b_conv, const float* w_t, const float* b_t, int cin_low, int cup, int cskip, int cout, int dtype,
                        void* packed, hipStream_t st);
int biu_mfma_foldt_stat_rows(const biu_act* x_low, const biu_act* y, const biu_act* skip = nullptr, int dtype = -1);
int biu_mfma_foldt_form(const biu_act* x_low, const biu_act* skip, const biu_act* y, int dtype);
int biu_mfma_foldt_fwd(const biu_act* x_low, const biu_xform* xf_low, const biu_act* skip, const biu_xform* xf_skip, const void* packed, const biu_act* y,
                       float* bn_partial, int dtype, hipStream_t st);
int biu_mfma_foldt_dgrad(const biu_act* dy, const void* packed, const biu_act* dx_low, int acc_low, const biu_act* dskip, int acc_skip, int dtype,
                         hipStream_t st, float* bn_partial_low, const BnRedFuse* red_low, void* ws, size_t ws_bytes);
size_t biu_mfma_foldt_wgrad_workspace(int cin_low, int cskip, int cout, int dtype);
int biu_mfma_foldt_wgrad(const biu_act* x_low, const biu_xform* xf_low, const biu_act* skip, const biu_xform* xf_skip, const biu_act* da, const BnBwdFuse* bn,
                         const float* dy_sum, const float* w_conv, const float* w_t, const float* b_t, int cup, float* dw_conv, float* dw_t, float* db_t, void* ws, size_t ws_bytes,
                         int dtype, hipStream_t st, int phases = 7);
bool biu_mfma_convt_ok(int kind, const biu_act* lo, const biu_act* hi, int kd, int dtype);
int biu_mfma_convt_fwd(const biu_act* x, const biu_xform* xf, const void* packed, const float* bias, int kd, const biu_act* y,
                       int dtype, hipStream_t st);
int biu_mfma_convt_dgrad(const biu_act* dy, const void* packed, int kd, const biu_act* dx, int accumulate, int dtype, hipStream_t st,
                         float* bn_partial = nullptr, const BnRedFuse* red = nullptr);
bool biu_mfma_convt_wgrad_ok(const biu_act* x, const biu_act* dy, int kd, int dtype);
int biu_mfma_convt_wgrad(const biu_act* x, const biu_xform* xf, const biu_act* dy, int kd, float* dw, float* dbias, void* ws,
                         size_t ws_bytes, int dtype, hipStream_t st);

bool biu_c1_conv_ok(const biu_act* x, const biu_act* y, int kd, int kh, int kw, int dil, int dtype);
int biu_c1_conv_fwd(const biu_act* x, const biu_xform* xf, const float* w, const float* bias, int kd, const biu_act* y, int dtype, hipStream_t st);
size_t biu_c1_wgrad_workspace(int cout, int kd);
int biu_c1_conv_wgrad(const biu_act* x, const biu_xform* xf, const biu_act* dy, int kd, float* dw, void* ws, size_t ws_bytes, int dtype, hipStream_t st);
bool biu_vec_reduce_ok(const biu_act* a, int dtype);
int biu_bn_stats_vec(const biu_act* y, float* partial, int* nblk_out, int dtype, hipStream_t st);
int biu_bn_bwd_reduce_vec(const biu_act* da, const biu_act* y, const float* scale, const float* shift, const float* slope,
                          const float* mean, const float* invstd, float* partial, int* nblk_out, int dtype, hipStream_t st);
size_t biu_chan_sum_workspace(int c);
int biu_chan_sum_vec(const biu_act* a, float* out, void* ws, int dtype, hipStream_t st);
bool biu_head_bwd_fused_ok(const biu_act* x, const biu_act* dx, int cout, int dtype);
size_t biu_head_bwd_fused_workspace(int cin);
bool biu_head_bwd_bnred_ok(const biu_act* x, const biu_act* dx, int cout, int dtype);
int biu_head_bwd_bnred_fused(const biu_act* x, const biu_xform* xf, const float* w, int cout, const float* dl, const biu_act* dx, float* dw,
                             float* db, void* ws, const float* mean, const float* invstd, float* bn_partial, int* bn_nblk, int dtype,
                             hipStream_t st);
int biu_head_bwd_fused(const biu_act* x, const biu_xform* xf, const float* w, int cout, const float* dl, const biu_act* dx, float* dw,
                       float* db, void* ws, size_t ws_bytes, int dtype, hipStream_t st);
bool biu_rowvec_ok(const biu_act* a, int dtype);
int biu_bn_bwd_apply_rv(const biu_act* da, const biu_act* y, const float* scale, const float* shift, const float* slope,
                        const float* A, const float* B, const float* Cc, const biu_act* dy, int dtype, hipStream_t st);
int biu_xform_apply_rv(const biu_act* x, const biu_xform* xf, const biu_act* out, int dtype, hipStream_t st);
int biu_maxpool_fwd_rv(const biu_act* x, const biu_xform* xf, const biu_act* out, int pd, int dtype, hipStream_t st);
int biu_maxpool_bwd_rv(const biu_act* x, const biu_xform* xf, const biu_act* dout, const biu_act* dx, int pd, int accumulate, int dtype, hipStream_t st);
int biu_maxpool_bwd_bnred_rv(const biu_act* x, const biu_xform* xf, const biu_act* dout, const biu_act* dx, int pd, int accumulate,
                             const float* mean, const float* invstd, float* partial, size_t partial_floats, int* nblk, int dtype,
                             hipStream_t st);
int biu_nearest_rv(int mode, const biu_act* src, const biu_xform* xf, const biu_act* dst, int pd, int accumulate, int dtype, hipStream_t st);

bool biu_convt_all_ok(const biu_act* lo, const biu_act* hi, int kd, int dtype);
int biu_convt_all_fwd(const biu_act* x, const biu_xform* xf, const void* packed, const float* bias, int kd, const biu_act* y, hipStream_t st);
int biu_convt_all_dgrad_rows(const biu_act* dx, const biu_act* dy, int kd);
int biu_convt_all_dgrad(const biu_act* dy, const void* packed, int kd, const biu_act* dx, int accumulate, hipStream_t st,
                        float* bn_partial = nullptr, const BnRedFuse* red = nullptr);

bool biu_c1m_ok(const biu_act* x, const biu_act* y, int kd, int kh, int kw, int dil, int dtype);
int biu_c1m_fwd_rows(const biu_act* y, int kd);
int biu_c1m_fwd(const biu_act* x, const biu_xform* xf, const float* w, const float* bias, int kd, const biu_act* y, float* bn_partial, hipStream_t st);
size_t biu_c1m_wgrad_workspace(int cout, int kd);
int biu_c1m_wgrad(const biu_act* x, const biu_xform* xf, const biu_act* da, const BnBwdFuse* bn, int kd, float* dw, void* ws, size_t ws_bytes,
                  hipStream_t st);
```

bio_image_unet_amd/engine.py:

```python
from __future__ import annotations

import ctypes as C
import os
import weakref
from typing import Dict, List, Optional, Sequence, Tuple

import torch
from torch import nn

from . import _lib
from ._lib import BIU_BF16, BIU_F32, BN_MAX_PARTIALS, biu_act, biu_xform, check, lib

LRELU_SLOPE = 0.1


def _stream():
    return C.c_void_p(torch.cuda.current_stream().cuda_stream)


def _ptr(t: Optional[torch.Tensor]):
    return C.c_void_p(t.data_ptr()) if t is not None else None


def _disabled(token: str, env: Optional[str] = None) -> bool:
    return token in (os.environ.get("BIU_DISABLE", "") if env is None else env).split(",")


_NO_CAPTURE_FORK = _disabled("capturefork")
_NO_SIDE_CHAIN = _disabled("sidechain")
_NO_PREPACK = _disabled("prepack")
_SIDE_WGRAD_VOX = int(os.environ.get("BIU_SIDE_WGRAD_VOX", str(4 * 32 ** 3)))

class Buf:

    def __init__(self, eng: "Engine", n, d, h, w, c):
        self.eng = eng
        self.shape = (n, d, h, w, c)
        self.t = torch.empty(self.shape, dtype=eng.tdtype, device=eng.device)
        self.g: Optional[torch.Tensor] = None
        self.scale = torch.ones(c, dtype=torch.float32, device=eng.device)
        self.shift = torch.zeros(c, dtype=torch.float32, device=eng.device)
        self.slope = torch.ones(c, dtype=torch.float32, device=eng.device)
        self.leaves: Dict[Tuple[int, int], bool] = {}
        self.lazy: Dict[Tuple[int, int], bool] = {}
        self.ncons: Dict[Tuple[int, int], int] = {}
        self.nwr: Dict[Tuple[int, int], int] = {}
        self.producer: Dict[Tuple[int, int], "Node"] = {}
        self.acts = []

    def slice(self, c0: int, c: int, lazy: bool) -> "Act":
        self.leaves[(c0, c)] = False
        self.lazy[(c0, c)] = lazy
        return Act(self, c0, c, [(c0, c)])

    def span(self, c0: int, c: int) -> "Act":
        keys = sorted(k for k in self.leaves if c0 <= k[0] < c0 + c)
        cov = c0
        for k0, kc in keys:
            assert k0 == cov, "span has a hole"
            cov += kc
        assert cov == c0 + c, "span does not end on a slice boundary"
        return Act(self, c0, c, keys)

    def full(self) -> "Act":
        keys = sorted(self.leaves)
        cov = 0
        for c0, c in keys:
            assert c0 == cov, "concat buffer has a hole"
            cov += c
        assert cov == self.shape[4]
        return Act(self, 0, cov, keys)

    def grad(self) -> torch.Tensor:
        assert self.t is not None, "a released buffer has no gradient either"
        if self.g is None:
            self.g = torch.empty(self.shape, dtype=self.eng.tdtype, device=self.eng.device)
        return self.g

    def release(self):
        self.t = None
        self.g = None
        for a in self.acts:
            a._a.p = None


class Act:

    def __init__(self, buf: Buf, c0: int, c: int, leaves):
        self.buf, self.c0, self.c, self.leaves = buf, c0, c, leaves
        n, d, h, w, ctot = buf.shape
        isz = buf.t.element_size()
        self.n, self.d, self.h, self.w = n, d, h, w
        self._a = biu_act(buf.t.data_ptr() + c0 * isz, n, d, h, w, c, ctot)
        self._g = None
        self._x = None
        self.is_input = False
        buf.acts.append(self)

    @property
    def nvox(self):
        return self.n * self.d * self.h * self.w

    @property
    def space(self):
        return (self.n, self.d, self.h, self.w)

    def a(self):
        return C.byref(self._a)

    def g(self):
        if self._g is None:
            gt = self.buf.grad()
            self._g = biu_act(gt.data_ptr() + self.c0 * gt.element_size(), self.n, self.d, self.h, self.w, self.c,
                              self.buf.shape[4])
        return C.byref(self._g)

    def is_lazy(self):
        return any(self.buf.lazy[k] for k in self.leaves)

    def xf(self):
        if not self.is_lazy():
            return None
        if self._x is None:
            o = 4 * self.c0
            self._x = biu_xform(self.buf.scale.data_ptr() + o, self.buf.shift.data_ptr() + o,
                                self.buf.slope.data_ptr() + o)
        return C.byref(self._x)

    def vec(self, name):
        return getattr(self.buf, name)[self.c0:self.c0 + self.c]

    def g_written(self) -> bool:
        flags = [self.buf.leaves[k] for k in self.leaves]
        assert all(flags) or not any(flags), "partially written concat gradient"
        return flags[0]

    def g_accumulate(self) -> int:
        flags = [self.buf.leaves[k] for k in self.leaves]
        if all(flags) or not any(flags):
            return int(flags[0])
        g = self.buf.grad()
        for k, f in zip(self.leaves, flags):
            if not f:
                g[..., k[0]:k[0] + k[1]].zero_()
                self.buf.leaves[k] = True
        return 1

    def mark_g(self):
        for k in self.leaves:
            self.buf.leaves[k] = True
            self.buf.nwr[k] = self.buf.nwr.get(k, 0) + 1

    def last_writer_producer(self):
        if len(self.leaves) != 1:
            return None
        k = self.leaves[0]
        if self.buf.ncons.get(k, 0) - self.buf.nwr.get(k, 0) != 1:
            return None
        up = self.buf.producer.get(k)
        if up is None or not getattr(up, "batch_stats", False) or up.y.c != self.c or up.y.c0 != self.c0:
            return None
        return up

    def consumed(self):
        for k in self.leaves:
            self.buf.ncons[k] = self.buf.ncons.get(k, 0) + 1

    def sole_conv_block_producer(self):
        if len(self.leaves) != 1 or self.buf.ncons.get(self.leaves[0], 0) != 1:
            return None
        return self.buf.producer.get(self.leaves[0])


class CatAct:

    def __init__(self, p0: Act, p1: Act):
        assert p0.space == p1.space
        self.parts = (p0, p1)
        self.c = p0.c + p1.c
        self.n, self.d, self.h, self.w = p0.n, p0.d, p0.h, p0.w
        self.is_input = False

    @property
    def nvox(self):
        return self.parts[0].nvox

    @property
    def space(self):
        return self.parts[0].space

    def consumed(self):
        for p in self.parts:
            p.consumed()


class CatBuf:

    def __init__(self, eng: "Engine", space, c_first, c_second):
        n, d, h, w = space
        self.c_first, self.c_second = c_first, c_second
        self.bufs = (eng.new_buf(n, d, h, w, c_first), eng.new_buf(n, d, h, w, c_second))
        self.acts = [None, None]

    def slice(self, c0: int, c: int, lazy: bool) -> Act:
        k = 0 if (c0, c) == (0, self.c_first) else 1
        assert (c0, c) == ((0, self.c_first) if k == 0 else (self.c_first, self.c_second)), "a planar concat has exactly two slices"
        self.acts[k] = self.bufs[k].slice(0, c, lazy)
        return self.acts[k]

    def full(self) -> CatAct:
        assert self.acts[0] is not None and self.acts[1] is not None, "both parts must be produced before the concatenation is read"
        return CatAct(self.acts[0], self.acts[1])


class Node:
    params: Sequence[nn.Parameter] = ()
    label = "node"

    def fwd(self, eng: "Engine"):
        raise NotImplementedError

    def bwd(self, eng: "Engine"):
        raise NotImplementedError


def _ksize(w: torch.Tensor):
    if w.dim() == 5:
        return tuple(w.shape[2:])
    return (1,) + tuple(w.shape[2:])


class ConvBlockNode(Node):

    def __init__(self, eng, seq: nn.Sequential, xin: Act, yout: Act, dropout_follows: bool = False, fold_src: Optional[Act] = None,
                 convt: Optional["ConvTNode"] = None):
        conv, bn = seq[0], seq[1]
        self.conv, self.bn, self.xin, self.y = conv, bn, xin, yout
        self.fold_src, self.fold_slot, self.fold_dg_slot, self.fold_wg, self.fold_all = None, None, None, False, False
        self.foldt, self.foldt_blob, self.foldt_ver = None, None, None
        self.fold_ws, self.fold_ev = None, None
        self.wg_ws, self.wg_ev = None, None
        act = seq[2] if len(seq) > 2 else None
        self.slope = float(act.negative_slope) if isinstance(act, nn.LeakyReLU) else (0.0 if isinstance(act, nn.ReLU) else 1.0)
        xin.consumed()
        if len(yout.leaves) == 1:
            yout.buf.producer[yout.leaves[0]] = self
        self.red_partial: Optional[torch.Tensor] = None
        self.red_nblk = 0
        self.kd, self.kh, self.kw = _ksize(conv.weight)
        self.dil = int(conv.dilation[0])
        drop = seq[3] if len(seq) > 3 else None
        if drop is not None and getattr(drop, "p", 0.0) != 0.0 and not dropout_follows:
            raise NotImplementedError("Dropout p != 0 needs a DropoutNode behind the block (models.Unet_v0 / BabyUnet build one)")
        assert tuple(conv.weight.shape[:2]) == (yout.c, xin.c), (conv.weight.shape, yout.c, xin.c)
        assert xin.space == yout.space
        self.params = [conv.weight, conv.bias, bn.weight, bn.bias]
        cout = yout.c
        dev = eng.device
        self.save_mean = torch.empty(cout, dtype=torch.float32, device=dev)
        self.save_invstd = torch.empty(cout, dtype=torch.float32, device=dev)
        yout.vec("slope").fill_(self.slope)
        eng.need_partial(cout)
        eng.need_partial_floats(lib.biu_conv_fwd_stats_floats(yout.a(), self.kd))
        if (convt is not None and isinstance(xin, CatAct) and len(xin.parts) == 2 and xin.parts[0] is convt.y and convt.kd == 2
                and (self.kd, self.kh, self.kw, self.dil) == (3, 3, 3, 1) and convt.up.bias is not None
                and lib.biu_foldt_ok(convt.xin.a(), xin.parts[1].a(), yout.a(), eng.dtype)
                and lib.biu_foldt_bwd_weight_workspace(convt.xin.c, xin.parts[1].c, cout, eng.dtype) > 0):
            self.foldt = convt
            lo, skip = convt.xin, xin.parts[1]
            self.foldt_blob = torch.empty(lib.biu_foldt_packed_bytes(lo.c, skip.c, cout, eng.dtype), dtype=torch.uint8, device=dev)
            eng.need_partial_floats(lib.biu_foldt_fwd_stats_floats(lo.a(), yout.a()))
            eng.need_ws(lib.biu_foldt_bwd_weight_workspace(lo.c, skip.c, cout, eng.dtype))
            self.params = [conv.weight, conv.bias, bn.weight, bn.bias]
        if (fold_src is not None and (self.kd, self.kh, self.kw, self.dil) == (3, 3, 3, 1) and not isinstance(xin, CatAct)
                and fold_src.c == xin.c and lib.biu_upconv_ok(fold_src.a(), yout.a(), eng.dtype)):
            self.fold_src = fold_src
            self.fold_slot = {"buf": torch.empty(lib.biu_upconv_packed_bytes(0, xin.c, cout, eng.dtype), dtype=torch.uint8, device=dev), "ver": None}
            nb1 = lib.biu_upconv_packed_bytes(1, xin.c, cout, eng.dtype)
            if nb1:
                self.fold_dg_slot = {"buf": torch.empty(nb1, dtype=torch.uint8, device=dev), "ver": None}
            wsf = lib.biu_upconv_bwd_weight_workspace(xin.c, cout, eng.dtype)
            if wsf:
                self.fold_wg = True
                eng.need_ws(wsf)
            self.fold_all = self.fold_dg_slot is not None and self.fold_wg
            eng.need_partial_floats(lib.biu_upconv_fwd_stats_floats(fold_src.a(), yout.a()))
        self.pk_f = eng.packed_slot(0, xin.c, cout, self.kd, self.kh, self.kw, self.dil)
        self.pk_b = eng.packed_slot(1, xin.c, cout, self.kd, self.kh, self.kw, self.dil)
        self.ws_bytes = lib.biu_conv_bwd_weight_workspace(xin.c, cout, self.kd, self.kh, self.kw, eng.dtype)
        eng.need_ws(self.ws_bytes)
        eng.need_ws(lib.biu_conv_split_workspace(xin.c, yout.a(), None, self.kd, self.kh, self.kw, self.dil, eng.dtype))
        if isinstance(xin, CatAct):
            eng.need_ws(lib.biu_conv_split_workspace(cout, xin.parts[0].a(), xin.parts[1].a(), self.kd, self.kh, self.kw, self.dil, eng.dtype))
        else:
            eng.need_ws(lib.biu_conv_split_workspace(cout, xin.a(), None, self.kd, self.kh, self.kw, self.dil, eng.dtype))

    def fwd(self, eng):
        st = _stream()
        w, b = self.conv.weight.data, self.conv.bias.data if self.conv.bias is not None else None
        packed = eng.pack(self.pk_f, 0, self.conv.weight, self.xin.c, self.y.c, self.kd, self.kh, self.kw)
        bn = self.bn
        scale, shift = self.y.vec("scale"), self.y.vec("shift")
        cat = self.xin.parts if isinstance(self.xin, CatAct) else None
        if self.foldt is not None:
            return self._fwd_foldt(eng, st)
        folded = None
        if self.fold_src is not None:
            ver = (self.conv.weight.data_ptr(), self.conv.weight._version)
            if self.fold_slot["ver"] != ver:
                check(lib.biu_upconv_pack(0, _ptr(w), self.xin.c, self.y.c, eng.dtype, _ptr(self.fold_slot["buf"]), st), "upconv_pack")
                self.fold_slot["ver"] = ver
            folded = _ptr(self.fold_slot["buf"])
        if eng.bn_training(bn):
            nblk = C.c_int(0)
            if folded:
                check(lib.biu_upconv_fwd(self.fold_src.a(), self.fold_src.xf(), folded, _ptr(b), self.y.a(), _ptr(eng.partial),
                                         eng.partial.numel(), C.byref(nblk), eng.dtype, st), "upconv_fwd")
            elif cat:
                check(lib.biu_conv_fwd_cat(cat[0].a(), cat[0].xf(), cat[1].a(), cat[1].xf(), _ptr(w), packed, _ptr(b), self.kd,
                                           self.kh, self.kw, self.dil, self.y.a(), _ptr(eng.partial), eng.partial.numel(),
                                           C.byref(nblk), _ptr(eng.ws), eng.ws_bytes, eng.dtype, st), "conv_fwd_cat")
            else:
                check(lib.biu_conv_fwd_stats(self.xin.a(), self.xin.xf(), _ptr(w), packed, _ptr(b), self.kd, self.kh, self.kw,
                                             self.dil, self.y.a(), _ptr(eng.partial), eng.partial.numel(), C.byref(nblk), _ptr(eng.ws), eng.ws_bytes,
                                             eng.dtype, st), "conv_fwd_stats")
            mom = bn.momentum if bn.momentum is not None else 0.1
            track = bn.track_running_stats and bn.running_mean is not None
            check(lib.biu_bn_finalize(_ptr(eng.partial), nblk.value, self.y.c, float(self.y.nvox), _ptr(bn.weight.data),
                                      _ptr(bn.bias.data), _ptr(bn.running_mean) if track else None,
                                      _ptr(bn.running_var) if track else None, mom, bn.eps, _ptr(scale), _ptr(shift),
                                      _ptr(self.save_mean), _ptr(self.save_invstd), st), "bn_finalize")
            if track and bn.num_batches_tracked is not None:
                eng.nbt_bump.append(bn.num_batches_tracked)
            self.batch_stats = True
        else:
            if folded:
                check(lib.biu_upconv_fwd(self.fold_src.a(), self.fold_src.xf(), folded, _ptr(b), self.y.a(), None, 0, None, eng.dtype, st),
                      "upconv_fwd")
            elif cat:
                check(lib.biu_conv_fwd_cat(cat[0].a(), cat[0].xf(), cat[1].a(), cat[1].xf(), _ptr(w), packed, _ptr(b), self.kd,
                                           self.kh, self.kw, self.dil, self.y.a(), None, 0, None, _ptr(eng.ws), eng.ws_bytes, eng.dtype, st), "conv_fwd_cat")
            else:
                check(lib.biu_conv_fwd(self.xin.a(), self.xin.xf(), _ptr(w), packed, _ptr(b), self.kd, self.kh, self.kw,
                                       self.dil, self.y.a(), _ptr(eng.ws), eng.ws_bytes, eng.dtype, st), "conv_fwd")
            check(lib.biu_bn_eval_affine(self.y.c, _ptr(bn.weight.data), _ptr(bn.bias.data), _ptr(bn.running_mean),
                                         _ptr(bn.running_var), bn.eps, _ptr(scale), _ptr(shift), st), "bn_eval_affine")
            self._eval_saved(eng)
            self.batch_stats = False

    def _eval_saved(self, eng):
        if eng.grad_mode:
            bn = self.bn
            self.save_mean.copy_(bn.running_mean)
            torch.rsqrt(bn.running_var.float() + bn.eps, out=self.save_invstd)

    def _foldt_version(self):
        ct = self.foldt
        ps = (self.conv.weight, self.conv.bias, ct.up.weight, ct.up.bias)
        return tuple((p.data_ptr(), p._version) for p in ps if p is not None)

    def _foldt_packed(self, st, eng=None):
        ct = self.foldt
        ver = self._foldt_version()
        if self.foldt_ver != ver:
            check(lib.biu_foldt_pack(_ptr(self.conv.weight.data), _ptr(self.conv.bias.data) if self.conv.bias is not None else None,
                                     _ptr(ct.up.weight.data), _ptr(ct.up.bias.data), ct.xin.c, ct.y.c, self.xin.parts[1].c, self.y.c, self._dtype,
                                     _ptr(self.foldt_blob), st), "foldt_pack")
            self.foldt_ver = ver
        elif eng is not None and eng._fold_ev is not None:
            torch.cuda.current_stream().wait_event(eng._fold_ev)
        return _ptr(self.foldt_blob)

    def _fwd_foldt(self, eng, st):
        self._dtype = eng.dtype
        ct, skip, bn = self.foldt, self.xin.parts[1], self.bn
        blob = self._foldt_packed(st, eng)
        scale, shift = self.y.vec("scale"), self.y.vec("shift")
        if eng.bn_training(bn):
            nblk = C.c_int(0)
            check(lib.biu_foldt_fwd(ct.xin.a(), ct.xin.xf(), skip.a(), skip.xf(), blob, self.y.a(), _ptr(eng.partial), eng.partial.numel(), C.byref(nblk),
                                    eng.dtype, st), "foldt_fwd")
            mom = bn.momentum if bn.momentum is not None else 0.1
            track = bn.track_running_stats and bn.running_mean is not None
            check(lib.biu_bn_finalize(_ptr(eng.partial), nblk.value, self.y.c, float(self.y.nvox), _ptr(bn.weight.data),
                                      _ptr(bn.bias.data), _ptr(bn.running_mean) if track else None,
                                      _ptr(bn.running_var) if track else None, mom, bn.eps, _ptr(scale), _ptr(shift),
                                      _ptr(self.save_mean), _ptr(self.save_invstd), st), "bn_finalize")
            if track and bn.num_batches_tracked is not None:
                eng.nbt_bump.append(bn.num_batches_tracked)
            self.batch_stats = True
        else:
            check(lib.biu_foldt_fwd(ct.xin.a(), ct.xin.xf(), skip.a(), skip.xf(), blob, self.y.a(), None, 0, None, eng.dtype, st), "foldt_fwd")
            check(lib.biu_bn_eval_affine(self.y.c, _ptr(bn.weight.data), _ptr(bn.bias.data), _ptr(bn.running_mean),
                                         _ptr(bn.running_var), bn.eps, _ptr(scale), _ptr(shift), st), "bn_eval_affine")
            self._eval_saved(eng)
            self.batch_stats = False

    def _bwd_foldt(self, eng, st, scale, shift, slope, A, B, Cc, dw, dy_sum=None):
        ct, skip, y = self.foldt, self.xin.parts[1], self.y
        lo = ct.xin
        dwt, dbt = eng.new_grad(ct.up.weight), eng.new_grad(ct.up.bias)
        side = eng.chain_stream()
        if side is None:
            check(lib.biu_foldt_bwd_weight_bn(lo.a(), lo.xf(), skip.a(), skip.xf(), y.g(), y.a(), scale, shift, slope, _ptr(A), _ptr(B), _ptr(Cc), _ptr(dy_sum),
                                              _ptr(self.conv.weight.data), _ptr(ct.up.weight.data), _ptr(ct.up.bias.data), ct.y.c, _ptr(dw), _ptr(dwt),
                                              _ptr(dbt), _ptr(eng.ws), eng.ws_bytes, eng.dtype, st), "foldt_bwd_weight_bn")
            eng.add_grad(ct.up.weight, dwt)
            eng.add_grad(ct.up.bias, dbt)
            deferred = False
        else:
            if self.fold_ws is None:
                self.fold_ws = torch.empty(lib.biu_foldt_bwd_weight_workspace(lo.c, skip.c, y.c, eng.dtype), dtype=torch.uint8, device=eng.device)
                self.fold_ev = (torch.cuda.Event(), torch.cuda.Event())
            args = (lo.a(), lo.xf(), skip.a(), skip.xf(), y.g(), y.a(), scale, shift, slope, _ptr(A), _ptr(B), _ptr(Cc), _ptr(dy_sum),
                    _ptr(self.conv.weight.data), _ptr(ct.up.weight.data), _ptr(ct.up.bias.data), ct.y.c, _ptr(dw), _ptr(dwt), _ptr(dbt),
                    _ptr(self.fold_ws), self.fold_ws.numel(), eng.dtype)
            check(lib.biu_foldt_bwd_weight_bn_phase(*args, 1 | 4, st), "foldt_bwd_weight_bn_phase(1 | 4)")
            cur = torch.cuda.current_stream()
            ready, done = self.fold_ev
            ready.record(cur)
            side.wait_event(ready)
            label = lib.label
            with torch.cuda.stream(side):
                lib.label = label + "/chain"
                check(lib.biu_foldt_bwd_weight_bn_phase(*args, 2, _stream()), "foldt_bwd_weight_bn_phase(2)")
                done.record(side)
            lib.label = label
            eng.defer_grads(done, [(ct.up.weight, dwt), (ct.up.bias, dbt), (self.conv.weight, dw)], keep=(A, B, Cc, dy_sum))
            deferred = True
        blob = self._foldt_packed(st)
        want_lo = eng.wants_grad(lo)
        up = _fusable_producer(lo) if want_lo else None
        if not want_lo:
            raise NotImplementedError("foldt: the coarse input of a decoder level always wants its gradient")
        if up is not None:
            need = lib.biu_foldt_bwd_data_bnred_floats(lo.a())
            if up.red_partial is None or up.red_partial.numel() < need:
                up.red_partial = torch.empty(need, dtype=torch.float32, device=eng.device)
            n_up = C.c_int(0)
            check(lib.biu_foldt_bwd_data(y.g(), blob, lo.g(), 0, skip.g(), int(skip.g_written()), lo.a(), *up.red_coeffs(), _ptr(up.red_partial),
                                         up.red_partial.numel(), C.byref(n_up), _ptr(eng.ws), eng.ws_bytes, eng.dtype, st), "foldt_bwd_data")
            up.red_nblk = n_up.value
        else:
            check(lib.biu_foldt_bwd_data(y.g(), blob, lo.g(), int(lo.g_written()), skip.g(), int(skip.g_written()), None, None, None, None, None, None,
                                         None, 0, None, _ptr(eng.ws), eng.ws_bytes, eng.dtype, st), "foldt_bwd_data")
        lo.mark_g()
        skip.mark_g()
        return deferred

    def bwd(self, eng):
        if not self.y.g_written():
            return
        st = _stream()
        y, cout = self.y, self.y.c
        scale, shift, slope = _ptr(y.vec("scale")), _ptr(y.vec("shift")), _ptr(y.vec("slope"))
        nblk = C.c_int(0)
        if self.red_nblk:
            partial, nblk.value, self.red_nblk = self.red_partial, self.red_nblk, 0
        else:
            partial = eng.partial
            check(lib.biu_bn_bwd_reduce(y.g(), y.a(), scale, shift, slope, _ptr(self.save_mean), _ptr(self.save_invstd),
                                        _ptr(partial), C.byref(nblk), eng.dtype, st), "bn_bwd_reduce")
        dgamma, dbeta = eng.new_grad(self.bn.weight), eng.new_grad(self.bn.bias)
        A, B, Cc = eng.coef[0][:cout], eng.coef[1][:cout], eng.coef[2][:cout]
        dw = eng.new_grad(self.conv.weight)
        dy_sum = None
        if self.batch_stats:
            check(lib.biu_bn_bwd_finalize(_ptr(partial), nblk.value, cout, float(y.nvox), scale, _ptr(self.save_mean),
                                          _ptr(self.save_invstd), _ptr(dgamma), _ptr(dbeta), _ptr(A), _ptr(B), _ptr(Cc), st),
                  "bn_bwd_finalize")
            db = eng.zero_like_bias(self.conv.bias) if self.conv.bias is not None else None
        else:
            dy_sum = torch.empty(cout, dtype=torch.float32, device=eng.device)
            check(lib.biu_bn_bwd_finalize_eval(_ptr(partial), nblk.value, cout, scale, _ptr(dgamma), _ptr(dbeta), _ptr(dy_sum), _ptr(A), _ptr(B),
                                               _ptr(Cc), st), "bn_bwd_finalize_eval")
            db = dy_sum if self.conv.bias is not None else None
        cat = self.xin.parts if isinstance(self.xin, CatAct) else None
        if self.foldt is not None:
            if not self._bwd_foldt(eng, st, scale, shift, slope, A, B, Cc, dw, dy_sum):
                eng.add_grad(self.conv.weight, dw)
            if db is not None:
                eng.add_grad(self.conv.bias, db)
            eng.add_grad(self.bn.weight, dgamma)
            eng.add_grad(self.bn.bias, dbeta)
            return
        if cat:
            check(lib.biu_conv_bwd_weight_cat(cat[0].a(), cat[0].xf(), cat[1].a(), cat[1].xf(), y.g(), y.a(), scale, shift, slope,
                                              _ptr(A), _ptr(B), _ptr(Cc), self.kd, self.kh, self.kw, self.dil, _ptr(dw), _ptr(eng.ws),
                                              eng.ws_bytes, eng.dtype, st), "conv_bwd_weight_cat")
        elif self.fold_wg:
            check(lib.biu_upconv_bwd_weight_bn(self.fold_src.a(), self.fold_src.xf(), y.g(), y.a(), scale, shift, slope, _ptr(A), _ptr(B),
                                               _ptr(Cc), _ptr(dw), _ptr(eng.ws), eng.ws_bytes, eng.dtype, st), "upconv_bwd_weight_bn")
        elif self.kd == 3 and eng.tdtype == torch.bfloat16 and y.nvox <= _SIDE_WGRAD_VOX and eng.chain_stream() is not None:
            side = eng.chain_stream()
            check(lib.biu_bn_bwd_apply(y.g(), y.a(), scale, shift, slope, _ptr(A), _ptr(B), _ptr(Cc), y.g(), eng.dtype, st), "bn_bwd_apply")
            if self.wg_ws is None:
                self.wg_ws = torch.empty(max(lib.biu_conv_bwd_weight_workspace(self.xin.c, cout, self.kd, self.kh, self.kw, eng.dtype), 16), dtype=torch.uint8,
                                         device=eng.device)
                self.wg_ev = (torch.cuda.Event(), torch.cuda.Event())
            ready, done = self.wg_ev
            ready.record(torch.cuda.current_stream())
            side.wait_event(ready)
            label = lib.label
            with torch.cuda.stream(side):
                lib.label = label + "/wgrad"
                check(lib.biu_conv_bwd_weight(self.xin.a(), self.xin.xf(), y.g(), self.kd, self.kh, self.kw, self.dil, _ptr(dw), None, _ptr(self.wg_ws),
                                              self.wg_ws.numel(), eng.dtype, _stream()), "conv_bwd_weight")
                done.record(side)
            lib.label = label
            eng.defer_grads(done, [(self.conv.weight, dw)])
            dw = None
        else:
            check(lib.biu_conv_bwd_weight_bn(self.xin.a(), self.xin.xf(), y.g(), y.a(), scale, shift, slope, _ptr(A), _ptr(B),
                                             _ptr(Cc), self.kd, self.kh, self.kw, self.dil, _ptr(dw), _ptr(eng.ws), eng.ws_bytes,
                                             eng.dtype, st), "conv_bwd_weight_bn")
        if dw is not None:
            eng.add_grad(self.conv.weight, dw)
        if db is not None:
            eng.add_grad(self.conv.bias, db)
        eng.add_grad(self.bn.weight, dgamma)
        eng.add_grad(self.bn.bias, dbeta)
        if cat:
            packed = eng.pack(self.pk_b, 1, self.conv.weight, self.xin.c, cout, self.kd, self.kh, self.kw)
            check(lib.biu_conv_bwd_data_cat(y.g(), _ptr(self.conv.weight.data), packed, self.kd, self.kh, self.kw, self.dil,
                                            cat[0].g(), cat[0].g_accumulate(), cat[1].g(), cat[1].g_accumulate(), _ptr(eng.ws), eng.ws_bytes, eng.dtype, st),
                  "conv_bwd_data_cat")
            cat[0].mark_g()
            cat[1].mark_g()
        elif self.fold_dg_slot is not None and eng.wants_grad(self.fold_src):
            ver = (self.conv.weight.data_ptr(), self.conv.weight._version)
            if self.fold_dg_slot["ver"] != ver:
                check(lib.biu_upconv_pack(1, _ptr(self.conv.weight.data), self.xin.c, cout, eng.dtype, _ptr(self.fold_dg_slot["buf"]), st), "upconv_pack")
                self.fold_dg_slot["ver"] = ver
            check(lib.biu_upconv_bwd_data(y.g(), _ptr(self.fold_dg_slot["buf"]), self.fold_src.g(), int(self.fold_src.g_written()), eng.dtype, st),
                  "upconv_bwd_data")
            self.fold_src.mark_g()
        elif eng.wants_grad(self.xin):
            packed = eng.pack(self.pk_b, 1, self.conv.weight, self.xin.c, cout, self.kd, self.kh, self.kw)
            up = _fusable_producer(self.xin)
            if up is not None:
                part = up.red_buffer(eng, self.kd, 0)
                n_up = C.c_int(0)
                check(lib.biu_conv_bwd_data_bnred(y.g(), _ptr(self.conv.weight.data), packed, self.kd, self.kh, self.kw,
                                                  self.dil, self.xin.g(), self.xin.a(), *up.red_coeffs(), _ptr(part),
                                                  part.numel(), C.byref(n_up), _ptr(eng.ws), eng.ws_bytes, eng.dtype, st), "conv_bwd_data_bnred")
                up.red_nblk = n_up.value
            else:
                check(lib.biu_conv_bwd_data(y.g(), _ptr(self.conv.weight.data), packed, self.kd, self.kh, self.kw, self.dil,
                                            self.xin.g(), int(self.xin.g_written()), _ptr(eng.ws), eng.ws_bytes, eng.dtype, st), "conv_bwd_data")
            self.xin.mark_g()

    def red_buffer(self, eng, kd, transposed) -> torch.Tensor:
        need = lib.biu_bwd_data_bnred_floats(self.y.a(), kd, transposed)
        if self.red_partial is None or self.red_partial.numel() < need:
            self.red_partial = torch.empty(need, dtype=torch.float32, device=eng.device)
        return self.red_partial

    def red_coeffs(self):
        y = self.y
        return (_ptr(y.vec("scale")), _ptr(y.vec("shift")), _ptr(y.vec("slope")), _ptr(self.save_mean),
                _ptr(self.save_invstd))


def _fusable_producer(xin: Act):
    if xin.g_written():
        return None
    up = xin.sole_conv_block_producer()
    if up is None or not getattr(up, "batch_stats", False) or up.y.c != xin.c or up.y.c0 != xin.c0:
        return None
    return up


class ConvTNode(Node):

    def __init__(self, eng, up: nn.Module, xin: Act, yout: Act):
        self.up, self.xin, self.y = up, xin, yout
        xin.consumed()
        w = up.weight
        self.kd = 2 if w.dim() == 5 else 1
        assert tuple(w.shape[:2]) == (xin.c, yout.c)
        self.params = [up.weight, up.bias]
        self.folded_into = None
        self.pk_f = eng.packed_slot_convt(0, xin.c, yout.c, self.kd)
        self.pk_b = eng.packed_slot_convt(1, xin.c, yout.c, self.kd)
        eng.need_ws(lib.biu_convt_bwd_weight_workspace(xin.c, yout.c, self.kd, eng.dtype))

    def fwd(self, eng):
        if self.folded_into is not None:
            return
        packed = eng.pack_convt(self.pk_f, 0, self.up.weight, self.xin.c, self.y.c, self.kd)
        check(lib.biu_convt_fwd(self.xin.a(), self.xin.xf(), _ptr(self.up.weight.data), packed, _ptr(self.up.bias.data),
                                self.kd, self.y.a(), eng.dtype, _stream()), "convt_fwd")

    def bwd(self, eng):
        if self.folded_into is not None or not self.y.g_written():
            return
        st = _stream()
        dw, db = eng.new_grad(self.up.weight), eng.new_grad(self.up.bias)
        check(lib.biu_convt_bwd_weight(self.xin.a(), self.xin.xf(), self.y.g(), self.kd, _ptr(dw), _ptr(db), _ptr(eng.ws),
                                       eng.ws_bytes, eng.dtype, st), "convt_bwd_weight")
        eng.add_grad(self.up.weight, dw)
        eng.add_grad(self.up.bias, db)
        if eng.wants_grad(self.xin):
            packed = eng.pack_convt(self.pk_b, 1, self.up.weight, self.xin.c, self.y.c, self.kd)
            up = _fusable_producer(self.xin)
            if up is not None:
                part = up.red_buffer(eng, self.kd, 1)
                n_up = C.c_int(0)
                check(lib.biu_convt_bwd_data_bnred(self.y.g(), _ptr(self.up.weight.data), packed, self.kd, self.xin.g(),
                                                   self.xin.a(), *up.red_coeffs(), _ptr(part), part.numel(), C.byref(n_up),
                                                   eng.dtype, st), "convt_bwd_data_bnred")
                up.red_nblk = n_up.value
            else:
                check(lib.biu_convt_bwd_data(self.y.g(), _ptr(self.up.weight.data), packed, self.kd, self.xin.g(),
                                             int(self.xin.g_written()), eng.dtype, st), "convt_bwd_data")
            self.xin.mark_g()


class ResampleNode(Node):

    def __init__(self, eng, kind: str, xin: Act, yout: Act):
        assert kind in ("maxpool", "down", "up", "trilinear", "bilinear")
        self.kind, self.xin, self.y = kind, xin, yout
        self.only_for_backward = False
        self.skip = False
        xin.consumed()

    def fwd(self, eng):
        if self.skip or (self.only_for_backward and not eng.grad_mode):
            return
        f = {"maxpool": lib.biu_maxpool_fwd, "down": lib.biu_nearest_down_fwd, "up": lib.biu_nearest_up_fwd,
             "trilinear": lib.biu_trilinear_up_fwd, "bilinear": lib.biu_bilinear_up_fwd}[self.kind]
        check(f(self.xin.a(), self.xin.xf(), self.y.a(), eng.dtype, _stream()), self.kind + "_fwd")

    def bwd(self, eng):
        if not self.y.g_written() or not eng.wants_grad(self.xin):
            return
        acc, st = int(self.xin.g_written()), _stream()
        if self.kind == "maxpool":
            up = self.xin.last_writer_producer() if self.xin.xf() is not None else None
            if up is not None:
                part = up.red_buffer(eng, up.kd, 0)
                n_up = C.c_int(0)
                check(lib.biu_maxpool_bwd_bnred(self.xin.a(), self.xin.xf(), self.y.g(), self.xin.g(), acc, _ptr(up.save_mean),
                                                _ptr(up.save_invstd), _ptr(part), part.numel(), C.byref(n_up), eng.dtype, st),
                      "maxpool_bwd_bnred")
                up.red_nblk = n_up.value
            else:
                check(lib.biu_maxpool_bwd(self.xin.a(), self.xin.xf(), self.y.g(), self.xin.g(), acc, eng.dtype, st), "maxpool_bwd")
        elif self.kind == "down":
            check(lib.biu_nearest_down_bwd(self.y.g(), self.xin.g(), acc, eng.dtype, st), "nearest_down_bwd")
        elif self.kind == "trilinear":
            check(lib.biu_trilinear_up_bwd(self.y.g(), self.xin.g(), acc, eng.dtype, st), "trilinear_up_bwd")
        elif self.kind == "bilinear":
            check(lib.biu_bilinear_up_bwd(self.y.g(), self.xin.g(), acc, eng.dtype, st), "bilinear_up_bwd")
        else:
            check(lib.biu_nearest_up_bwd(self.y.g(), self.xin.g(), acc, eng.dtype, st), "nearest_up_bwd")
        self.xin.mark_g()


class MaxJoinNode(Node):

    def __init__(self, eng, a: Act, b: Act, out: Act):
        self.a_, self.b_, self.y = a, b, out
        a.consumed()
        b.consumed()

    def fwd(self, eng):
        check(lib.biu_max_join_fwd(self.a_.a(), self.a_.xf(), self.b_.a(), self.b_.xf(), self.y.a(), eng.dtype, _stream()),
              "max_join_fwd")

    def bwd(self, eng):
        if not self.y.g_written():
            return
        assert self.a_.g_written() == self.b_.g_written()
        check(lib.biu_max_join_bwd(self.a_.a(), self.a_.xf(), self.b_.a(), self.b_.xf(), self.y.g(), self.a_.g(),
                                   self.b_.g(), int(self.a_.g_written()), eng.dtype, _stream()), "max_join_bwd")
        self.a_.mark_g()
        self.b_.mark_g()


class XCorrNode(Node):

    def __init__(self, eng, a: Act, b: Act, out: Act):
        self.a_, self.b_, self.y = a, b, out
        a.consumed()
        b.consumed()

    def fwd(self, eng):
        check(lib.biu_xcorr_fwd(self.a_.a(), self.a_.xf(), self.b_.a(), self.b_.xf(), self.y.a(), eng.dtype, _stream()), "xcorr_fwd")

    def bwd(self, eng):
        if not self.y.g_written():
            return
        assert self.a_.g_written() == self.b_.g_written()
        check(lib.biu_xcorr_bwd(self.a_.a(), self.a_.xf(), self.b_.a(), self.b_.xf(), self.y.g(), self.a_.g(), self.b_.g(),
                                int(self.a_.g_written()), eng.dtype, _stream()), "xcorr_bwd")
        self.a_.mark_g()
        self.b_.mark_g()


class CopyNode(Node):

    def __init__(self, eng, xin: Act, out: Act):
        self.xin, self.y = xin, out
        xin.consumed()

    def fwd(self, eng):
        check(lib.biu_xform_apply(self.xin.a(), self.xin.xf(), self.y.a(), eng.dtype, _stream()), "xform_apply")

    def bwd(self, eng):
        if not self.y.g_written() or not eng.wants_grad(self.xin):
            return
        check(lib.biu_act_add(self.y.g(), self.xin.g(), self.xin.g_accumulate(), eng.dtype, _stream()), "act_add")
        self.xin.mark_g()


class DropoutNode(Node):

    def __init__(self, eng, drop: nn.Module, xin: Act, out: Act):
        self.drop, self.xin, self.y = drop, xin, out
        xin.consumed()
        self.mask_override: Optional[torch.Tensor] = None
        self.factor: Optional[torch.Tensor] = None
        self._keep = []

    def _sample(self, act: Act, tensor: torch.Tensor, n: int) -> biu_act:
        per = act.d * act.h * act.w * act.buf.shape[4] * tensor.element_size()
        return biu_act(tensor.data_ptr() + act.c0 * tensor.element_size() + n * per, 1, act.d, act.h, act.w, act.c, act.buf.shape[4])

    def fwd(self, eng):
        x, st = self.xin, _stream()
        p = float(self.drop.p)
        if self.drop.training and p > 0.0:
            if self.mask_override is not None:
                keep = self.mask_override.to(device=eng.device, dtype=torch.float32)
            else:
                keep = torch.bernoulli(torch.full((x.n, x.c), 1.0 - p, device=eng.device))
            self.factor = keep / (1.0 - p)
        else:
            self.factor = torch.ones((x.n, x.c), device=eng.device)
        sc = (x.vec("scale")[None, :] * self.factor).contiguous()
        sh = (x.vec("shift")[None, :] * self.factor).contiguous()
        sl = x.vec("slope").contiguous()
        self._keep = [sc, sh, sl]
        for n in range(x.n):
            xf = biu_xform(sc[n].data_ptr(), sh[n].data_ptr(), sl.data_ptr())
            a_in, a_out = self._sample(x, x.buf.t, n), self._sample(self.y, self.y.buf.t, n)
            check(lib.biu_xform_apply(C.byref(a_in), C.byref(xf), C.byref(a_out), eng.dtype, st), "dropout_fwd")

    def bwd(self, eng):
        if not self.y.g_written() or not eng.wants_grad(self.xin):
            return
        assert not self.xin.g_written(), "DropoutNode is the only reader of its input"
        st = _stream()
        f = self.factor.contiguous()
        zero, one = torch.zeros_like(f[0]), torch.ones_like(f[0])
        self._keep += [f, zero, one]
        for n in range(self.xin.n):
            xf = biu_xform(f[n].data_ptr(), zero.data_ptr(), one.data_ptr())
            g_out, g_in = self._sample(self.y, self.y.buf.grad(), n), self._sample(self.xin, self.xin.buf.grad(), n)
            check(lib.biu_xform_apply(C.byref(g_out), C.byref(xf), C.byref(g_in), eng.dtype, st), "dropout_bwd")
        self.xin.mark_g()


class AddReluNode(Node):

    def __init__(self, eng, a: Act, b: Act, out: Act):
        self.a_, self.b_, self.y = a, b, out
        a.consumed()
        b.consumed()

    def fwd(self, eng):
        check(lib.biu_add_relu_fwd(self.a_.a(), self.a_.xf(), self.b_.a(), self.b_.xf(), self.y.a(), eng.dtype, _stream()), "add_relu_fwd")

    def bwd(self, eng):
        if not self.y.g_written():
            return
        assert self.a_.g_written() == self.b_.g_written()
        check(lib.biu_add_relu_bwd(self.y.a(), self.y.g(), self.a_.g(), self.b_.g(), int(self.a_.g_written()), eng.dtype, _stream()),
              "add_relu_bwd")
        self.a_.mark_g()
        self.b_.mark_g()


class GateNode(Node):

    def __init__(self, eng, e: Act, psi: Act, out: Act):
        assert psi.c == 1 and e.c == out.c
        self.e_, self.psi_, self.y = e, psi, out
        e.consumed()
        psi.consumed()

    def fwd(self, eng):
        check(lib.biu_gate_fwd(self.e_.a(), self.e_.xf(), self.psi_.a(), self.psi_.xf(), self.y.a(), eng.dtype, _stream()), "gate_fwd")

    def bwd(self, eng):
        if not self.y.g_written():
            return
        assert not self.psi_.g_written()
        check(lib.biu_gate_bwd(self.e_.a(), self.e_.xf(), self.psi_.a(), self.psi_.xf(), self.y.g(), self.e_.g(),
                               int(self.e_.g_written()), self.psi_.g(), eng.dtype, _stream()), "gate_bwd")
        self.e_.mark_g()
        self.psi_.mark_g()


_ACT_CODE = {None: 0, "none": 0, "sigmoid": 1, "tanh": 2, "relu": 3}


class HeadNode(Node):

    def __init__(self, eng, conv: nn.Module, xin: Act, activation, want_logits: bool, want_act: bool):
        self.conv, self.xin = conv, xin
        xin.consumed()
        self.cout = conv.weight.shape[0]
        assert conv.weight.shape[1] == xin.c
        if activation not in _ACT_CODE:
            activation = None
        self.activation = activation
        self.act = _ACT_CODE[activation]
        self.want_logits, self.want_act = want_logits, want_act
        self.params = [conv.weight, conv.bias]
        eng.need_ws(lib.biu_head_bwd_workspace(xin.c))
        self.logits = self.activated = None

    def out_shape(self, eng):
        x = self.xin
        return (x.n, self.cout, x.d, x.h, x.w) if eng.nd == 3 else (x.n, self.cout, x.h, x.w)

    def fwd(self, eng):
        shp = self.out_shape(eng)
        self.logits = torch.empty(shp, dtype=torch.float32, device=eng.device) if self.want_logits else None
        self.activated = torch.empty(shp, dtype=torch.float32, device=eng.device) if self.want_act else None
        w = self.conv.weight.data.reshape(self.cout, self.xin.c)
        check(lib.biu_head_fwd(self.xin.a(), self.xin.xf(), _ptr(w), _ptr(self.conv.bias.data), self.cout, self.act,
                               _ptr(self.logits), _ptr(self.activated), eng.dtype, _stream()), "head_fwd")

    def dlogits(self, eng, g_logits, g_act, a, dst=None, ctot=None, c0=0):
        if g_act is None and dst is None and g_logits.dtype == torch.float32 and g_logits.is_contiguous():
            return g_logits
        shp = self.out_shape(eng)
        n, spatial = shp[0], 1
        for v in shp[2:]:
            spatial *= v
        if dst is None:
            dst, ctot, c0 = torch.empty(shp, dtype=torch.float32, device=eng.device), self.cout, 0
        f32 = lambda t: None if t is None else t.contiguous().float()
        gl, ga = f32(g_logits), f32(g_act)
        self._keep = (gl, ga, a)
        check(lib.biu_head_dlogits(_ptr(gl), _ptr(ga), _ptr(a) if ga is not None else None, self.act, n, self.cout, spatial,
                                   _ptr(dst), ctot, c0, _stream()), "head_dlogits")
        return dst

    def bwd_with(self, eng, dl: Optional[torch.Tensor]):
        if dl is None:
            return
        dl = dl.contiguous().float()
        st = _stream()
        dw, db = eng.new_grad(self.conv.weight), eng.new_grad(self.conv.bias)
        want_dx = eng.wants_grad(self.xin)
        assert not self.xin.g_written(), "heads that share a trunk go through Engine._backward_heads"
        up = self.xin.last_writer_producer() if (want_dx and self.xin.xf() is not None) else None
        if up is not None:
            part = up.red_buffer(eng, up.kd, 0)
            n_up = C.c_int(0)
            check(lib.biu_head_bwd_bnred(self.xin.a(), self.xin.xf(), _ptr(self.conv.weight.data), self.cout, _ptr(dl),
                                         self.xin.g(), _ptr(dw), _ptr(db), _ptr(eng.ws), eng.ws_bytes, _ptr(up.save_mean),
                                         _ptr(up.save_invstd), _ptr(part), part.numel(), C.byref(n_up), eng.dtype, st),
                  "head_bwd_bnred")
            up.red_nblk = n_up.value
        else:
            check(lib.biu_head_bwd(self.xin.a(), self.xin.xf(), _ptr(self.conv.weight.data), self.cout, _ptr(dl),
                                   self.xin.g() if want_dx else None, _ptr(dw), _ptr(db), _ptr(eng.ws), eng.ws_bytes,
                                   eng.dtype, st), "head_bwd")
        eng.add_grad(self.conv.weight, dw)
        eng.add_grad(self.conv.bias, db)
        if want_dx:
            self.xin.mark_g()


class Engine:

    def __init__(self, device, tdtype, nd: int):
        if torch.device(device).type != "cuda":
            raise RuntimeError("bio_image_unet_amd executes only through its HIP kernels on an MI355X; "
                               f"got device '{device}'. There is no CPU fallback.")
        self.device, self.tdtype, self.nd = torch.device(device), tdtype, nd
        self.dtype = {torch.float32: BIU_F32, torch.bfloat16: BIU_BF16}[tdtype]
        self.nodes: List[Node] = []
        self.heads: List[HeadNode] = []
        self.bufs: List[Buf] = []
        self.inputs: List[Act] = []
        self._partial_c = 0
        self.ws_bytes = 0
        self.partial = self.ws = None
        self.coef = None
        self.grads: Dict[nn.Parameter, torch.Tensor] = {}
        self.nbt_bump: List[torch.Tensor] = []
        self.grad_mode = False
        self.module_training = True
        self.input_requires_grad = False
        self._packed: Dict[int, dict] = {}
        self._zero_flat, self._zero_used = None, 0
        self._slots: List[dict] = []
        self._job_key, self._job_tab = None, None
        self.grad_hook = None
        self.grad_alloc = None
        self.trace = None
        self.generation = 0
        self._live = None
        self._side = None
        self._deferred = []
        self._fold_ev = None

    def busy(self) -> bool:
        return self._live is not None and self._live() is not None

    def invalidate_packed(self):
        for s in self._slots:
            s["ver"] = None
        for nd_ in self.nodes:
            for name in ("fold_slot", "fold_dg_slot"):
                s = getattr(nd_, name, None)
                if s is not None:
                    s["ver"] = None
            if getattr(nd_, "foldt_ver", None) is not None:
                nd_.foldt_ver = None

    def new_buf(self, n, d, h, w, c) -> Buf:
        b = Buf(self, n, d, h, w, c)
        self.bufs.append(b)
        return b

    def new_cat(self, space, c_first, c_second, consumer_cout, kd):
        n, d, h, w = space
        probe = lambda c: biu_act(256, n, d, h, w, c, c)
        a0, a1, ay = probe(c_first), probe(c_second), probe(consumer_cout)
        if lib.biu_conv_cat_ok(C.byref(a0), C.byref(a1), C.byref(ay), kd, 3, 3, 1, self.dtype) == 1:
            return CatBuf(self, space, c_first, c_second)
        return self.new_buf(n, d, h, w, c_first + c_second)

    def new_act(self, space, c, lazy: bool) -> Act:
        n, d, h, w = space
        return self.new_buf(n, d, h, w, c).slice(0, c, lazy)

    def add(self, node: Node):
        self.nodes.append(node)
        return node

    def need_partial(self, c):
        self._partial_c = max(self._partial_c, c)

    def need_partial_floats(self, n):
        self._partial_floats = max(getattr(self, "_partial_floats", 0), int(n))

    def need_ws(self, nbytes):
        self.ws_bytes = max(self.ws_bytes, int(nbytes))

    def finalize(self):
        dev = self.device
        c = max(self._partial_c, 1)
        self.partial = torch.empty(max(BN_MAX_PARTIALS * c * 2, getattr(self, "_partial_floats", 0)), dtype=torch.float32,
                                   device=dev)
        self.coef = torch.empty((3, c), dtype=torch.float32, device=dev)
        self.ws = torch.empty(max(self.ws_bytes, 16), dtype=torch.uint8, device=dev)
        self.params: List[nn.Parameter] = []
        seen = set()
        self._pcount: Dict[nn.Parameter, int] = {}
        for nd_ in self.nodes:
            for p in nd_.params:
                if p is not None:
                    self._pcount[p] = self._pcount.get(p, 0) + 1
                    if id(p) not in seen:
                        seen.add(id(p))
                        self.params.append(p)

    def packed_slot(self, kind, cin, cout, kd, kh, kw, dil):
        nbytes = lib.biu_conv_packed_bytes(kind, cin, cout, kd, kh, kw, dil, self.dtype)
        if nbytes == 0:
            return None
        slot = {"buf": torch.empty(nbytes, dtype=torch.uint8, device=self.device), "ver": None,
                "job": (0, kind, cin, cout, kd, kh, kw), "weight": None}
        self._slots.append(slot)
        return slot

    def pack(self, slot, kind, weight: nn.Parameter, cin, cout, kd, kh, kw):
        if slot is None:
            return None
        slot["weight"] = weight
        ver = (weight.data_ptr(), weight._version)
        if slot["ver"] != ver:
            check(lib.biu_conv_pack(kind, _ptr(weight.data), cin, cout, kd, kh, kw, self.dtype, _ptr(slot["buf"]), _stream()),
                  "conv_pack")
            slot["ver"] = ver
        return _ptr(slot["buf"])

    def packed_slot_convt(self, kind, cin, cout, kd):
        nbytes = lib.biu_convt_packed_bytes(kind, cin, cout, kd, self.dtype)
        if nbytes == 0:
            return None
        slot = {"buf": torch.empty(nbytes, dtype=torch.uint8, device=self.device), "ver": None,
                "job": (1, kind, cin, cout, kd, 2, 2), "weight": None}
        self._slots.append(slot)
        return slot

    def pack_convt(self, slot, kind, weight: nn.Parameter, cin, cout, kd):
        if slot is None:
            return None
        slot["weight"] = weight
        ver = (weight.data_ptr(), weight._version)
        if slot["ver"] != ver:
            check(lib.biu_convt_pack(kind, _ptr(weight.data), cin, cout, kd, self.dtype, _ptr(slot["buf"]), _stream()),
                  "convt_pack")
            slot["ver"] = ver
        return _ptr(slot["buf"])

    def pack_all(self):
        stale = [s for s in self._slots if s["weight"] is not None and s["ver"] != (s["weight"].data_ptr(), s["weight"]._version)]
        if len(stale) < 2:
            return
        key = tuple((id(s), s["weight"].data_ptr()) for s in stale)
        if self._job_key != key:
            from ._lib import biu_pack_job
            arr = (biu_pack_job * len(stale))()
            for j, s in zip(arr, stale):
                tr, kind, cin, cout, kd, kh, kw = s["job"]
                j.w, j.packed = s["weight"].data_ptr(), s["buf"].data_ptr()
                j.transposed, j.kind, j.cin, j.cout, j.kd, j.kh, j.kw, j.reserved = tr, kind, cin, cout, kd, kh, kw, 0
            raw = torch.frombuffer(bytearray(bytes(arr)), dtype=torch.uint8)
            self._job_tab = raw.to(self.device)
            self._job_key = key
        check(lib.biu_pack_batch(_ptr(self._job_tab), len(stale), self.dtype, _stream()), "pack_batch")
        for s in stale:
            s["ver"] = (s["weight"].data_ptr(), s["weight"]._version)

    def bn_training(self, bn: nn.Module) -> bool:
        return bn.training or bn.running_mean is None

    def wants_grad(self, act: Act) -> bool:
        return self.input_requires_grad if act.is_input else True

    def new_input(self, space, c) -> Act:
        a = self.new_act(space, c, lazy=False)
        a.is_input = True
        self.inputs.append(a)
        return a

    def new_grad(self, p: nn.Parameter) -> torch.Tensor:
        if self.grad_alloc is not None and self._pcount.get(p, 1) == 1:
            v = self.grad_alloc(p)
            if v is not None:
                return v
        return torch.empty(p.shape, dtype=torch.float32, device=self.device)

    def zero_like_bias(self, b: torch.Tensor) -> torch.Tensor:
        n = b.numel()
        if self._zero_flat is None or self._zero_used + n > self._zero_flat.numel() or self._zero_flat.dtype != b.dtype:
            self._zero_flat = torch.zeros(max(4096, 4 * n), dtype=b.dtype, device=b.device)
            self._zero_used = 0
        v = self._zero_flat[self._zero_used:self._zero_used + n].view_as(b)
        self._zero_used += n
        return v

    def add_grad(self, p: nn.Parameter, g: torch.Tensor):
        if p in self.grads:
            self.grads[p] = self.grads[p] + g
        else:
            self.grads[p] = g
        if self.grad_hook is not None:
            self._pseen[p] = self._pseen.get(p, 0) + 1
            if self._pseen[p] == self._pcount.get(p, 1):
                self.grad_hook(p, self.grads[p])

    def load_inputs(self, xs: Sequence[torch.Tensor]):
        st = _stream()
        for act, x in zip(self.inputs, xs):
            x = x.detach()
            if x.dtype == torch.uint8:
                x = x.contiguous()
                check(lib.biu_from_nchw_u8(_ptr(x), 1.0 / 255.0, act.a(), self.dtype, st), "from_nchw_u8")
                continue
            if x.dtype != torch.float32:
                x = x.float()
            x = x.contiguous()
            check(lib.biu_from_nchw(_ptr(x), act.a(), self.dtype, st), "from_nchw")

    def _prepack_folds(self):
        self._fold_ev = None
        if _NO_PREPACK or (torch.cuda.is_current_stream_capturing() and _NO_CAPTURE_FORK):
            return
        stale = [n for n in self.nodes if isinstance(n, ConvBlockNode) and n.foldt is not None and n.foldt_ver != n._foldt_version()]
        if not stale:
            return
        cur = torch.cuda.current_stream()
        if self._side is None:
            self._side = torch.cuda.Stream(device=self.device)
        self._side.wait_stream(cur)
        with torch.cuda.stream(self._side):
            st = _stream()
            for n in stale:
                n._dtype = self.dtype
                lib.label = n.label + ":pack"
                n._foldt_packed(st)
            self._fold_ev = torch.cuda.Event()
            self._fold_ev.record(self._side)

    def forward(self):
        self.generation += 1
        self.nbt_bump = []
        lib.label = "pack:fwd"
        self.pack_all()
        self._prepack_folds()
        for nd_ in self.nodes:
            lib.label = nd_.label + ":fwd"
            if self.trace:
                self.trace("fwd", nd_, "pre")
            nd_.fwd(self)
            if self.trace:
                self.trace("fwd", nd_, "post")
        if self.nbt_bump:
            counts: Dict[int, list] = {}
            for t in self.nbt_bump:
                counts.setdefault(id(t), [t, 0])[1] += 1
            by_k: Dict[int, list] = {}
            for t, k in counts.values():
                by_k.setdefault(k, []).append(t)
            for k, ts in by_k.items():
                torch._foreach_add_(ts, k)

    def chain_stream(self):
        if self.trace or _NO_SIDE_CHAIN or (torch.cuda.is_current_stream_capturing() and _NO_CAPTURE_FORK):
            return None
        if self._side is None:
            self._side = torch.cuda.Stream(device=self.device)
        return self._side

    def defer_grads(self, done: "torch.cuda.Event", grads, keep=()):
        self._deferred.append((done, grads, keep))

    def _flush_deferred(self, keep_last: int):
        while len(self._deferred) > keep_last:
            done, grads, _ = self._deferred.pop(0)
            torch.cuda.current_stream().wait_event(done)
            for p, g in grads:
                self.add_grad(p, g)

    def backward(self, head_grads: Sequence[Optional[torch.Tensor]]):
        self.grads = {}
        self._deferred = []
        self._pseen: Dict[nn.Parameter, int] = {}
        self._zero_flat, self._zero_used = None, 0
        for b in self.bufs:
            for k in b.leaves:
                b.leaves[k] = False
                b.nwr[k] = 0
        lib.label = "head:bwd"
        if self.trace:
            self.trace("bwd", ("heads", head_grads), "pre")
        self._backward_heads(head_grads)
        if self.trace:
            self.trace("bwd", ("heads", head_grads), "post")
        for nd_ in reversed(self.nodes):
            if isinstance(nd_, HeadNode):
                continue
            lib.label = nd_.label + ":bwd"
            if self.trace:
                self.trace("bwd", nd_, "pre")
            self._flush_deferred(2)
            nd_.bwd(self)
            if self.trace:
                self.trace("bwd", nd_, "post")
        self._flush_deferred(0)
        return self.grads

    def _backward_heads(self, head_grads):
        live = [(h, g) for h, g in zip(self.heads, head_grads) if g is not None]
        if not live:
            return
        groups: Dict[int, list] = {}
        for h, g in live:
            groups.setdefault(id(h.xin), []).append((h, g))
        for grp in groups.values():
            self._backward_head_group(grp)

    def _backward_head_group(self, live):
        if len(live) == 1:
            h, (gl, ga, a) = live[0]
            h.bwd_with(self, h.dlogits(self, gl, ga, a))
            return
        x = live[0][0].xin
        assert all(h.xin is x for h, _ in live)
        cout = sum(h.cout for h, _ in live)
        shp = live[0][0].out_shape(self)
        dl = torch.empty((shp[0], cout) + tuple(shp[2:]), dtype=torch.float32, device=self.device)
        key = tuple(id(h) for h, _ in live)
        if not hasattr(self, "_stack_w"):
            self._stack_w = {}
        if key not in self._stack_w:
            self._stack_w[key] = torch.empty((cout, x.c), dtype=torch.float32, device=self.device)
        w, o = self._stack_w[key], 0
        for h, (gl, ga, a) in live:
            w[o:o + h.cout].copy_(h.conv.weight.data.reshape(h.cout, x.c))
            h.dlogits(self, gl, ga, a, dst=dl, ctot=cout, c0=o)
            o += h.cout
        dw = torch.empty_like(w)
        db = torch.empty(cout, dtype=torch.float32, device=self.device)
        up = None
        if self.wants_grad(x) and x.xf() is not None and not x.g_written() and len(x.leaves) == 1:
            k = x.leaves[0]
            cand = x.buf.producer.get(k)
            if (x.buf.ncons.get(k, 0) == len(live) and cand is not None and getattr(cand, "batch_stats", False)
                    and cand.y.c == x.c and cand.y.c0 == x.c0):
                up = cand
        if up is not None:
            part = up.red_buffer(self, up.kd, 0)
            n_up = C.c_int(0)
            check(lib.biu_head_bwd_bnred(x.a(), x.xf(), _ptr(w), cout, _ptr(dl), x.g(), _ptr(dw), _ptr(db), _ptr(self.ws), self.ws_bytes,
                                         _ptr(up.save_mean), _ptr(up.save_invstd), _ptr(part), part.numel(), C.byref(n_up), self.dtype,
                                         _stream()), "head_bwd_bnred(stacked)")
            up.red_nblk = n_up.value
        else:
            check(lib.biu_head_bwd(x.a(), x.xf(), _ptr(w), cout, _ptr(dl), x.g(), _ptr(dw), _ptr(db), _ptr(self.ws),
                                   self.ws_bytes, self.dtype, _stream()), "head_bwd(stacked)")
        x.mark_g()
        o = 0
        for h, _ in live:
            self.add_grad(h.conv.weight, dw[o:o + h.cout].reshape(h.conv.weight.shape).clone())
            self.add_grad(h.conv.bias, db[o:o + h.cout].clone())
            o += h.cout

    def input_grads(self) -> List[Optional[torch.Tensor]]:
        outs = []
        st = _stream()
        for act in self.inputs:
            if not self.input_requires_grad or not act.g_written():
                outs.append(None)
                continue
            shp = (act.n, act.c, act.d, act.h, act.w) if self.nd == 3 else (act.n, act.c, act.h, act.w)
            t = torch.empty(shp, dtype=torch.float32, device=self.device)
            ga = biu_act(act.buf.grad().data_ptr(), act.n, act.d, act.h, act.w, act.c, act.buf.shape[4])
            check(lib.biu_to_nchw(C.byref(ga), None, _ptr(t), self.dtype, st), "to_nchw")
            outs.append(t)
        return outs


class _Token:
    __slots__ = ("__weakref__",)


class _NetFn(torch.autograd.Function):

    @staticmethod
    def forward(ctx, eng: Engine, n_inputs: int, out_spec, *tensors):
        xs, ctx.n_inputs = tensors[:n_inputs], n_inputs
        if eng.busy():
            raise RuntimeError("engine re-entered while an earlier forward still awaits its backward (models take a second "
                               "engine for that case: this is a bug in the caller of engine.run)")
        eng.load_inputs(xs)
        eng.forward()
        ctx.eng, ctx.out_spec = eng, out_spec
        ctx.generation = eng.generation
        if eng.grad_mode:
            ctx.token = _Token()
            eng._live = weakref.ref(ctx.token)
        else:
            eng._live = None
        outs = []
        for hi, kind in out_spec:
            h = eng.heads[hi]
            outs.append(h.logits if kind == "logits" else h.activated)
        ctx.act_slot = {hi: i for i, (hi, kind) in enumerate(out_spec) if kind == "act"}
        ctx.save_for_backward(*[outs[i] for i in ctx.act_slot.values()])
        for h in eng.heads:
            h.logits = h.activated = None
        return tuple(outs)

    @staticmethod
    def backward(ctx, *gouts):
        eng: Engine = ctx.eng
        if ctx.generation != eng.generation:
            raise RuntimeError("backward of a forward whose activations were overwritten: the engine ran another forward of the "
                               "same input shape in between (generation %d, now %d)" % (ctx.generation, eng.generation))
        per_head: Dict[int, List[Optional[torch.Tensor]]] = {}
        for (hi, kind), g in zip(ctx.out_spec, gouts):
            slot = per_head.setdefault(hi, [None, None])
            slot[0 if kind == "logits" else 1] = g
        saved = dict(zip(ctx.act_slot.keys(), ctx.saved_tensors))
        head_grads = []
        for hi, h in enumerate(eng.heads):
            gl, ga = per_head.get(hi, [None, None])
            head_grads.append((gl, ga, saved.get(hi)) if (gl is not None or ga is not None) else None)
        grads = eng.backward(head_grads)
        dxs = eng.input_grads()
        pg = [grads.pop(p, None) for p in eng.params]
        eng.grads = {}
        del grads
        ctx.token = None
        eng._live = None
        eng.generation += 1
        return (None, None, None, *dxs, *pg)


def run(eng: Engine, xs: Sequence[torch.Tensor], out_spec):
    eng.grad_mode = torch.is_grad_enabled()
    eng.input_requires_grad = eng.grad_mode and any(x.requires_grad for x in xs)
    return _NetFn.apply(eng, len(xs), tuple(out_spec), *xs, *eng.params)
```

include/biu.h:

```cpp
#ifndef BIU_H
#define BIU_H

#include <stddef.h>
#include <stdint.h>

#ifdef __cplusplus
extern "C" {
#endif

typedef void* biu_stream;

enum { BIU_F32 = 0, BIU_BF16 = 1 };

typedef enum {
    BIU_OK = 0,
    BIU_ERR_SHAPE = -1,
    BIU_ERR_UNSUPPORTED = -2,
    BIU_ERR_ALIGN = -3,
    BIU_ERR_WORKSPACE = -4,
    BIU_ERR_LAUNCH = -5
} biu_status;

typedef struct {
    void*   p;
    int32_t n, d, h, w;
    int32_t c;
    int32_t pitch;
} biu_act;

typedef struct {
    const float* scale;
    const float* shift;
    const float* slope;
} biu_xform;

const char* biu_last_error(void);
int  biu_version(void);

int  biu_set_fp32_products(int mode);

int  biu_set_fp32_products_3d(int mode);


size_t biu_conv_packed_bytes(int kind, int cin, int cout, int kd, int kh, int kw, int dilation, int dtype);
int    biu_conv_pack(int kind, const float* w, int cin, int cout, int kd, int kh, int kw, int dtype,
                     void* packed, biu_stream stream);

typedef struct biu_pack_job {
    const void* w;
    void* packed;
    int32_t transposed, kind, cin, cout, kd, kh, kw, reserved;
} biu_pack_job;
int biu_pack_batch(const biu_pack_job* jobs, int n, int dtype, biu_stream stream);

size_t biu_conv_split_workspace(int cin, const biu_act* y, const biu_act* y1, int kd, int kh, int kw, int dilation, int dtype);

int biu_conv_fwd(const biu_act* x, const biu_xform* xf, const float* w, const void* packed,
                 const float* bias, int kd, int kh, int kw, int dilation,
                 const biu_act* y, void* ws, size_t ws_bytes, int dtype, biu_stream stream);

size_t biu_conv_fwd_stats_floats(const biu_act* y, int kd);
int biu_conv_fwd_stats(const biu_act* x, const biu_xform* xf, const float* w, const void* packed,
                       const float* bias, int kd, int kh, int kw, int dilation, const biu_act* y,
                       float* bn_partial, size_t bn_partial_floats, int* bn_nblk, void* ws, size_t ws_bytes, int dtype,
                       biu_stream stream);

int biu_conv_bwd_data(const biu_act* dy, const float* w, const void* packed,
                      int kd, int kh, int kw, int dilation,
                      const biu_act* dx, int accumulate, void* ws, size_t ws_bytes, int dtype, biu_stream stream);

size_t biu_bwd_data_bnred_floats(const biu_act* dx, int kd, int transposed);
int biu_conv_bwd_data_bnred(const biu_act* dy, const float* w, const void* packed, int kd, int kh, int kw, int dilation,
                            const biu_act* dx, const biu_act* y_up, const float* scale, const float* shift,
                            const float* slope, const float* mean, const float* invstd, float* partial,
                            size_t partial_floats, int* nblk, void* ws, size_t ws_bytes, int dtype, biu_stream stream);
int biu_convt_bwd_data_bnred(const biu_act* dy, const float* w, const void* packed, int kd, const biu_act* dx,
                             const biu_act* y_up, const float* scale, const float* shift, const float* slope,
                             const float* mean, const float* invstd, float* partial, size_t partial_floats, int* nblk,
                             int dtype, biu_stream stream);

size_t biu_conv_bwd_weight_workspace(int cin, int cout, int kd, int kh, int kw, int dtype);
int biu_conv_bwd_weight(const biu_act* x, const biu_xform* xf, const biu_act* dy,
                        int kd, int kh, int kw, int dilation,
                        float* dw, float* dbias, void* ws, size_t ws_bytes, int dtype, biu_stream stream);

int biu_conv_bwd_weight_bn(const biu_act* x, const biu_xform* xf, const biu_act* da, const biu_act* y,
                           const float* scale, const float* shift, const float* slope, const float* coefA,
                           const float* coefB, const float* coefC, int kd, int kh, int kw, int dilation,
                           float* dw, void* ws, size_t ws_bytes, int dtype, biu_stream stream);

#define BIU_BN_MAX_PARTIALS 1024
int biu_bn_stats(const biu_act* y, float* partial, int* nblk_out, int dtype, biu_stream stream);

int biu_bn_finalize(const float* partial, int nblk, int c, double count,
                    const float* gamma, const float* beta, float* running_mean, float* running_var,
                    float momentum, float eps, float* scale, float* shift,
                    float* save_mean, float* save_invstd, biu_stream stream);

int biu_bn_eval_affine(int c, const float* gamma, const float* beta, const float* running_mean,
                       const float* running_var, float eps, float* scale, float* shift, biu_stream stream);

int biu_xform_apply(const biu_act* x, const biu_xform* xf, const biu_act* out, int dtype, biu_stream stream);

int biu_bn_bwd_reduce(const biu_act* da, const biu_act* y, const float* scale, const float* shift,
                      const float* slope, const float* save_mean, const float* save_invstd,
                      float* partial, int* nblk_out, int dtype, biu_stream stream);
int biu_bn_bwd_finalize(const float* partial, int nblk, int c, double count,
                        const float* scale, const float* save_mean, const float* save_invstd,
                        float* dgamma, float* dbeta, float* coefA, float* coefB, float* coefC,
                        biu_stream stream);
int biu_bn_bwd_finalize_eval(const float* partial, int nblk, int c, const float* scale,
                             float* dgamma, float* dbeta, float* dbias, float* coefA, float* coefB, float* coefC,
                             biu_stream stream);
int biu_bn_bwd_apply(const biu_act* da, const biu_act* y, const float* scale, const float* shift,
                     const float* slope, const float* coefA, const float* coefB, const float* coefC,
                     const biu_act* dy, int dtype, biu_stream stream);

int biu_maxpool_fwd(const biu_act* x, const biu_xform* xf, const biu_act* out, int dtype, biu_stream stream);
int biu_maxpool_bwd(const biu_act* x, const biu_xform* xf, const biu_act* dout, const biu_act* dx,
                    int accumulate, int dtype, biu_stream stream);
int biu_maxpool_bwd_bnred(const biu_act* x, const biu_xform* xf, const biu_act* dout, const biu_act* dx, int accumulate,
                          const float* mean, const float* invstd, float* partial, size_t partial_floats, int* nblk,
                          int dtype, biu_stream stream);
int biu_nearest_down_fwd(const biu_act* x, const biu_xform* xf, const biu_act* out, int dtype, biu_stream stream);
int biu_nearest_down_bwd(const biu_act* dout, const biu_act* dx, int accumulate, int dtype, biu_stream stream);
int biu_nearest_up_fwd(const biu_act* x, const biu_xform* xf, const biu_act* out, int dtype, biu_stream stream);
int biu_nearest_up_bwd(const biu_act* dout, const biu_act* dx, int accumulate, int dtype, biu_stream stream);

int    biu_upconv_ok(const biu_act* x, const biu_act* y, int dtype);
size_t biu_upconv_packed_bytes(int kind, int cin, int cout, int dtype);
int    biu_upconv_pack(int kind, const float* w, int cin, int cout, int dtype, void* packed, biu_stream stream);
int    biu_upconv_bwd_data(const biu_act* dy, const void* packed, const biu_act* dx, int accumulate, int dtype, biu_stream stream);
size_t biu_upconv_bwd_weight_workspace(int cin, int cout, int dtype);
int    biu_upconv_bwd_weight_bn(const biu_act* x, const biu_xform* xf, const biu_act* da, const biu_act* y, const float* scale,
                                const float* shift, const float* slope, const float* coefA, const float* coefB, const float* coefC,
                                float* dw, void* ws, size_t ws_bytes, int dtype, biu_stream stream);
size_t biu_upconv_fwd_stats_floats(const biu_act* x, const biu_act* y);
int    biu_upconv_fwd(const biu_act* x, const biu_xform* xf, const void* packed, const float* bias, const biu_act* y,
                      float* bn_partial, size_t bn_partial_floats, int* bn_nblk, int dtype, biu_stream stream);

int biu_bce_dice_blocks(long long per_sample);
int biu_bce_dice_fwd(const float* logits, const float* target, int n, long long per_sample, float* partial, biu_stream stream);
int biu_bce_dice_bwd(const float* logits, const float* target, int n, long long per_sample, const float* coef, float* dlogits,
                     int accumulate, biu_stream stream);

int biu_pair_smooth_l1_blocks(long long pairs);
int biu_pair_smooth_l1_fwd(const float* logits, int n, long long per_sample, float* partial, biu_stream stream);
int biu_pair_smooth_l1_bwd(const float* logits, int n, long long per_sample, const float* coef, float* dlogits, int accumulate,
                           biu_stream stream);
int biu_seg_loss_finish(const float* partial, int n, int nb, long long per_sample, const float* time_partial, int nbt,
                        float a_bce, float a_dice, float smooth, int has_tversky, float tv_alpha, float tv_beta, float tv_smooth,
                        int logcosh, float w_time, float* saved, biu_stream stream);
int biu_seg_loss_coef(const float* g, const float* saved, int n, long long per_sample, float a_bce, float a_dice, float smooth,
                      int has_tversky, float tv_alpha, float tv_beta, float tv_smooth, int logcosh, float w_time, float* coef,
                      float* time_coef, biu_stream stream);
int biu_head_dlogits(const float* g_logits, const float* g_act, const float* activated, int act, int n, int ch, long long spatial,
                     float* dst, int dst_channels, int dst_c0, biu_stream stream);

#define BIU_MO2D_MAX_LEVELS 4
#define BIU_MO2D_MAX_TERMS 32
#define BIU_MO2D_SLOTS 8
typedef struct biu_mo2d_term {
    int kind, nb;
    long long partial_off;
    long long numel, pixels;
    float p0, p1, p2, weight;
} biu_mo2d_term;
int biu_mo2d_loss_blocks(long long numel);
int biu_mo2d_loss_fwd(int kind, float ea, float eb, const float* const* pred, int nlev, const float* target, int n, int c, int h, int w,
                      float* partial, biu_stream stream);
int biu_mo2d_loss_finish(const biu_mo2d_term* terms, int nterms, const float* workspace, float* saved, biu_stream stream);
int biu_mo2d_loss_coef(const biu_mo2d_term* terms, int nterms, const float* g, const float* saved, float* coef, biu_stream stream);
int biu_mo2d_loss_bwd(int kind, float ea, float eb, const float* const* pred, int nlev, const float* target, int n, int c, int h, int w,
                      const float* coef, float* const* dpred, biu_stream stream);

int biu_trilinear_up_fwd(const biu_act* x, const biu_xform* xf, const biu_act* out, int dtype, biu_stream stream);
int biu_trilinear_up_bwd(const biu_act* dout, const biu_act* dx, int accumulate, int dtype, biu_stream stream);

int biu_bilinear_up_fwd(const biu_act* x, const biu_xform* xf, const biu_act* out, int dtype, biu_stream stream);
int biu_bilinear_up_bwd(const biu_act* dout, const biu_act* dx, int accumulate, int dtype, biu_stream stream);

int biu_xcorr_fwd(const biu_act* cur, const biu_xform* xc, const biu_act* prev, const biu_xform* xp, const biu_act* out,
                  int dtype, biu_stream stream);
int biu_xcorr_bwd(const biu_act* cur, const biu_xform* xc, const biu_act* prev, const biu_xform* xp, const biu_act* dout,
                  const biu_act* dcur, const biu_act* dprev, int accumulate, int dtype, biu_stream stream);

int biu_conv_cat_ok(const biu_act* x0, const biu_act* x1, const biu_act* y, int kd, int kh, int kw, int dilation, int dtype);
int biu_conv_fwd_cat(const biu_act* x0, const biu_xform* xf0, const biu_act* x1, const biu_xform* xf1, const float* w,
                     const void* packed, const float* bias, int kd, int kh, int kw, int dilation, const biu_act* y,
                     float* bn_partial, size_t bn_partial_floats, int* bn_nblk, void* ws, size_t ws_bytes, int dtype,
                     biu_stream stream);
int biu_conv_bwd_data_cat(const biu_act* dy, const float* w, const void* packed, int kd, int kh, int kw, int dilation,
                          const biu_act* dx0, int accumulate0, const biu_act* dx1, int accumulate1, void* ws, size_t ws_bytes,
                          int dtype, biu_stream stream);
int biu_conv_bwd_weight_cat(const biu_act* x0, const biu_xform* xf0, const biu_act* x1, const biu_xform* xf1,
                            const biu_act* da, const biu_act* y, const float* scale, const float* shift, const float* slope,
                            const float* coefA, const float* coefB, const float* coefC, int kd, int kh, int kw, int dilation,
                            float* dw, void* ws, size_t ws_bytes, int dtype, biu_stream stream);

size_t biu_convt_packed_bytes(int kind, int cin, int cout, int kd, int dtype);
int    biu_convt_pack(int kind, const float* w, int cin, int cout, int kd, int dtype, void* packed, biu_stream stream);
int biu_convt_fwd(const biu_act* x, const biu_xform* xf, const float* w, const void* packed, const float* bias,
                  int kd, const biu_act* y, int dtype, biu_stream stream);
int biu_convt_bwd_data(const biu_act* dy, const float* w, const void* packed, int kd, const biu_act* dx,
                       int accumulate, int dtype, biu_stream stream);
size_t biu_convt_bwd_weight_workspace(int cin, int cout, int kd, int dtype);
int biu_convt_bwd_weight(const biu_act* x, const biu_xform* xf, const biu_act* dy, int kd, float* dw, float* dbias,
                         void* ws, size_t ws_bytes, int dtype, biu_stream stream);

int    biu_foldt_ok(const biu_act* x_low, const biu_act* skip, const biu_act* y, int dtype);
size_t biu_foldt_packed_bytes(int cin_low, int cskip, int cout, int dtype);
int    biu_foldt_pack(const float* w_conv, const float* b_conv, const float* w_t, const float* b_t, int cin_low, int cup, int cskip, int cout,
                      int dtype, void* packed, biu_stream stream);
size_t biu_foldt_fwd_stats_floats(const biu_act* x_low, const biu_act* y);
int    biu_foldt_fwd_form(const biu_act* x_low, const biu_act* skip, const biu_act* y, int dtype);
int    biu_foldt_fwd(const biu_act* x_low, const biu_xform* xf_low, const biu_act* skip, const biu_xform* xf_skip, const void* packed,
                     const biu_act* y, float* bn_partial, size_t bn_partial_floats, int* bn_nblk, int dtype, biu_stream stream);
size_t biu_foldt_bwd_data_bnred_floats(const biu_act* dx_low);
int    biu_foldt_bwd_data(const biu_act* dy, const void* packed, const biu_act* dx_low, int acc_low, const biu_act* dskip, int acc_skip,
                          const biu_act* y_low, const float* scale, const float* shift, const float* slope, const float* mean,
                          const float* invstd, float* partial, size_t partial_floats, int* nblk, void* ws, size_t ws_bytes, int dtype,
                          biu_stream stream);
size_t biu_foldt_bwd_weight_workspace(int cin_low, int cskip, int cout, int dtype);
int    biu_foldt_bwd_weight_bn(const biu_act* x_low, const biu_xform* xf_low, const biu_act* skip, const biu_xform* xf_skip, const biu_act* da,
                               const biu_act* y, const float* scale, const float* shift, const float* slope, const float* coefA,
                               const float* coefB, const float* coefC, const float* dy_sum, const float* w_conv, const float* w_t, const float* b_t,
                               int cup, float* dw_conv, float* dw_t, float* db_t, void* ws, size_t ws_bytes, int dtype, biu_stream stream);
int    biu_foldt_bwd_weight_bn_phase(const biu_act* x_low, const biu_xform* xf_low, const biu_act* skip, const biu_xform* xf_skip, const biu_act* da,
                                     const biu_act* y, const float* scale, const float* shift, const float* slope, const float* coefA,
                                     const float* coefB, const float* coefC, const float* dy_sum, const float* w_conv, const float* w_t,
                                     const float* b_t, int cup, float* dw_conv, float* dw_t, float* db_t, void* ws, size_t ws_bytes, int dtype,
                                     int phases, biu_stream stream);

int biu_head_fwd(const biu_act* x, const biu_xform* xf, const float* w, const float* bias, int cout,
                 int act, float* logits, float* activated, int dtype, biu_stream stream);
size_t biu_head_bwd_workspace(int cin);
int biu_head_bwd(const biu_act* x, const biu_xform* xf, const float* w, int cout, const float* dlogits,
                 const biu_act* dx, float* dw, float* dbias, void* ws, size_t ws_bytes, int dtype,
                 biu_stream stream);
int biu_head_bwd_bnred(const biu_act* x, const biu_xform* xf, const float* w, int cout, const float* dlogits, const biu_act* dx,
                       float* dw, float* dbias, void* ws, size_t ws_bytes, const float* mean, const float* invstd,
                       float* partial, size_t partial_floats, int* nblk, int dtype, biu_stream stream);

int biu_max_join_fwd(const biu_act* a, const biu_xform* xa, const biu_act* b, const biu_xform* xb,
                     const biu_act* out, int dtype, biu_stream stream);
int biu_max_join_bwd(const biu_act* a, const biu_xform* xa, const biu_act* b, const biu_xform* xb,
                     const biu_act* dout, const biu_act* da, const biu_act* db, int accumulate,
                     int dtype, biu_stream stream);
int biu_act_add(const biu_act* src, const biu_act* dst, int accumulate, int dtype, biu_stream stream);
int biu_from_nchw(const float* src, const biu_act* dst, int dtype, biu_stream stream);
int biu_to_nchw(const biu_act* src, const biu_xform* xf, float* dst, int dtype, biu_stream stream);

int biu_add_relu_fwd(const biu_act* a, const biu_xform* xa, const biu_act* b, const biu_xform* xb, const biu_act* out, int dtype,
                     biu_stream stream);
int biu_add_relu_bwd(const biu_act* out, const biu_act* dout, const biu_act* da, const biu_act* db, int accumulate, int dtype,
                     biu_stream stream);
int biu_gate_fwd(const biu_act* e, const biu_xform* xe, const biu_act* psi, const biu_xform* xpsi, const biu_act* out, int dtype,
                 biu_stream stream);
int biu_gate_bwd(const biu_act* e, const biu_xform* xe, const biu_act* psi, const biu_xform* xpsi, const biu_act* dout,
                 const biu_act* de, int accumulate_e, const biu_act* dpsi, int dtype, biu_stream stream);

int biu_from_nchw_u8(const uint8_t* src, float scale, const biu_act* dst, int dtype, biu_stream stream);
int biu_u8_to_f32(const uint8_t* src, float scale, float* dst, long long n, biu_stream stream);
int biu_quantize_u8(const float* src, float scale, uint8_t* dst, long long n, biu_stream stream);
int biu_stitch_add(const void* patch, int patch_is_u8, const float* weight, int channels, int pd, int ph, int pw, float* acc, float* wsum,
                   int D, int H, int W, int z0, int y0, int x0, int set, biu_stream stream);
int biu_stitch_finish(const float* acc, const float* wsum, int layers, int channels, long long spatial, void* out, int out_is_u8,
                      biu_stream stream);

#define BIU_AUG_GATE 1u
#define BIU_AUG_SSR 2u
#define BIU_AUG_BC 4u
#define BIU_AUG_BLUR 8u
#define BIU_AUG_MULT 16u
#define BIU_AUG_GAUSS 32u
#define BIU_AUG_ORDER_UNET 0
#define BIU_AUG_ORDER_SIAM 1
#define BIU_AUG_STAGE_MULT 1u
#define BIU_AUG_STAGE_GAUSS 2u
#define BIU_AUG_MAX_BLUR 15
typedef struct biu_aug_params {
    uint32_t flags, rot_k, blur_k, index;
    double m[6];
    float alpha, beta, noise_a, noise_b;
    float angle, scale, dx, dy;
} biu_aug_params;
int biu_augment_u8(const uint8_t* src, uint8_t* dst, int n, int planes, int h, int w, int is_mask, const biu_aug_params* params,
                   int stage_order, int max_blur_k, unsigned long long seed, unsigned epoch, unsigned field_id, biu_stream stream);
int biu_philox_u32(uint32_t* out, long long blocks, unsigned long long seed, unsigned c0, unsigned c1, unsigned c2, unsigned c3,
                   biu_stream stream);

#define BIU_AUGF_IMAGE 0
#define BIU_AUGF_MASK 1
#define BIU_AUGF_VECTOR 2
#define BIU_AUGF_ROT 1u
#define BIU_AUGF_SCALE 2u
#define BIU_AUGF_BLUR 4u
#define BIU_AUGF_SHOT 8u
#define BIU_AUGF_GAUSS 16u
#define BIU_AUGF_BC 32u
#define BIU_AUGF_STAGE_SHOT 3u
#define BIU_AUGF_STAGE_GAUSS 4u
#define BIU_AUGF_POISSON_CAP 128
typedef struct biu_augf_params {
    uint32_t flags, rot_k, blur_k, index;
    double m[6];
    float cos_t, sin_t, alpha, beta, shot_s, gauss_sigma;
    float angle, scale, dx, dy;
} biu_augf_params;
int biu_augment_f32(const void* src, int src_is_u8, float* dst, int n, int planes, int h, int w, int kind, const biu_augf_params* params,
                    int max_blur_k, unsigned long long seed, unsigned epoch, unsigned field_id, biu_stream stream);

int biu_adam_step(int n, float* const* params, const float* const* grads, float* const* exp_avg,
                  float* const* exp_avg_sq, const int64_t* numel, float lr, float beta1, float beta2,
                  float eps, int step, float grad_scale, biu_stream stream);

int biu_adam_set_hyper(float* hyper, float lr, float beta1, float beta2, float eps, int step, float grad_scale, biu_stream stream);
int biu_adam_step_hyper(int n, float* const* params, const float* const* grads, float* const* exp_avg,
                        float* const* exp_avg_sq, const int64_t* numel, const float* hyper, biu_stream stream);

size_t biu_grad_clip_scratch_floats(int n);
int biu_grad_clip(int n, float* const* grads, const int64_t* numel, float max_norm, float* scratch, size_t scratch_floats, float* total_norm,
                  biu_stream stream);

#ifdef __cplusplus
}
#endif
#endif
```

Measured before the change: 741.3 million voxels/s.

## Skip writing BN-applied gradient in first-layer wgrad; use buffer loads and per-wave sums

Adds a 'keep' variant of the first-layer fused BN-backward weight-gradient kernel. It skips writing the BN-applied gradient back to memory when no input gradient is needed, saving a full-resolution store. The change also switches the forward and wgrad first-layer kernels to buffer loads and stores with out-of-bounds offsets instead of branches. It precomputes halo offsets per thread and replaces LDS atomics with per-wave partial sums. It specializes the kernel on PPV (pieces per voxel: 2 or 4, from the 16- or 32-channel chunk), which adds template instances and relies on per-sample byte sizes staying under 4GB.

```diff
diff --git a/bio_image_unet_amd/_lib.py b/bio_image_unet_amd/_lib.py
--- a/bio_image_unet_amd/_lib.py
+++ b/bio_image_unet_amd/_lib.py
@@ -74,6 +74,8 @@
     "biu_conv_bwd_weight_workspace": (_Z, [_I, _I, _I, _I, _I, _I]),
     "biu_conv_bwd_weight": (_I, [_A, _X, _A, _I, _I, _I, _I, _P, _P, _P, _Z, _I, _P]),
     "biu_conv_bwd_weight_bn": (_I, [_A, _X, _A, _A, _P, _P, _P, _P, _P, _P, _I, _I, _I, _I, _P, _P, _Z, _I, _P]),
+    "biu_conv_bwd_weight_bn_keep_ok": (_I, [_A, _A, _A, _I, _I, _I, _I, _I]),
+    "biu_conv_bwd_weight_bn_keep": (_I, [_A, _X, _A, _A, _P, _P, _P, _P, _P, _P, _I, _I, _I, _I, _P, _P, _Z, _I, _P]),
     "biu_bn_stats": (_I, [_A, _P, C.POINTER(C.c_int), _I, _P]),
     "biu_bn_finalize": (_I, [_P, _I, _I, _D, _P, _P, _P, _P, _F, _F, _P, _P, _P, _P, _P]),
     "biu_bn_eval_affine": (_I, [_I, _P, _P, _P, _P, _F, _P, _P, _P]),
diff --git a/bio_image_unet_amd/csrc/biu_api.hip b/bio_image_unet_amd/csrc/biu_api.hip
--- a/bio_image_unet_amd/csrc/biu_api.hip
+++ b/bio_image_unet_amd/csrc/biu_api.hip
@@ -8,7 +8,7 @@
     "conv_fwd", "conv_dgrad", "conv_wgrad", "convt_fwd", "convt_dgrad", "convt_wgrad", "convt_all", "c1", "c1_mfma", "cat",
     "fused_stats", "wgrad_bn", "dgrad_bnred", "pool_pair", "pool_pipe", "pool_bnred", "head_bnred", "ksplit", "m16", "m16x2", "rr16",
     "wroll", "wroll16", "wroll2d", "upconv", "foldt", "foldall", "foldck8", "foldgemm", "croll", "froll", "prepack", "wsplitbn",
-    "capturefork", "sidechain",
+    "capturefork", "sidechain", "c1keep",
 };
 constexpr int kNumOffTokens = sizeof(kOffTokens) / sizeof(kOffTokens[0]);
 static_assert(kNumOffTokens <= 64, "BiuEnv::off holds one bit per token");
@@ -307,6 +307,31 @@
     int rc = biu_bn_bwd_apply(da, y, scale, shift, slope, coefA, coefB, coefC, da, dtype, stream);
     if (rc != BIU_OK) return rc;
     return biu_conv_bwd_weight(x, xf, da, kd, kh, kw, dilation, dw, nullptr, ws, ws_bytes, dtype, stream);
+}
+
+static bool bn_keep_ok(const biu_act* x, const biu_act* da, const biu_act* y, int kd, int kh, int kw, int dilation, int dtype) {
+    if (!x || !da || !y || !conv_args_ok(x, da, kd, kh, kw, dilation) || !valid_act(y) || !same_space(y, da) || y->c != da->c) return false;
+    const bool yok = ((uintptr_t)y->p % 16) == 0 && ((size_t)y->pitch * dsize(dtype)) % 16 == 0 &&
+                     (i64)y->d * y->h * y->w * y->pitch * (i64)dsize(dtype) < (1LL << 32) - 65536;
+    return !biu_off("c1") && !biu_off("wgrad_bn") && yok && biu_c1m_ok(x, da, kd, kh, kw, dilation, dtype);
+}
+extern "C" int biu_conv_bwd_weight_bn_keep_ok(const biu_act* x, const biu_act* da, const biu_act* y, int kd, int kh, int kw, int dilation,
+                                              int dtype) {
+    return bn_keep_ok(x, da, y, kd, kh, kw, dilation, dtype) ? 1 : 0;
+}
+extern "C" int biu_conv_bwd_weight_bn_keep(const biu_act* x, const biu_xform* xf, const biu_act* da, const biu_act* y,
+                                           const float* scale, const float* shift, const float* slope, const float* coefA,
+                                           const float* coefB, const float* coefC, int kd, int kh, int kw, int dilation,
+                                           float* dw, void* ws, size_t ws_bytes, int dtype, biu_stream stream) {
+    BIU_REQUIRE(x && da && y && conv_args_ok(x, da, kd, kh, kw, dilation) && valid_act(y) && same_space(y, da) && y->c == da->c, BIU_ERR_SHAPE,
+                "conv_bwd_weight_bn_keep: extents differ");
+    BIU_REQUIRE(dw && scale && shift && coefA && coefB && coefC, BIU_ERR_SHAPE, "conv_bwd_weight_bn_keep: null pointer");
+    BIU_REQUIRE(bn_keep_ok(x, da, y, kd, kh, kw, dilation, dtype), BIU_ERR_UNSUPPORTED,
+                "conv_bwd_weight_bn_keep: only the bf16 first-layer shapes (one input channel, 3x3 / 3x3x3, a multiple of 16 output channels, "
+                "16-byte aligned da and y) are served; use biu_conv_bwd_weight_bn");
+    BIU_REQUIRE(ws && ws_bytes >= biu_c1m_wgrad_workspace(da->c, kd), BIU_ERR_WORKSPACE, "conv_bwd_weight_bn_keep: workspace too small");
+    BnBwdFuse bn{y, scale, shift, slope, coefA, coefB, coefC};
+    return biu_c1m_wgrad(x, xf, da, &bn, kd, dw, ws, ws_bytes, (hipStream_t)stream, true);
 }
 
 extern "C" int biu_conv_cat_ok(const biu_act* x0, const biu_act* x1, const biu_act* y, int kd, int kh, int kw, int dilation, int dtype) {
diff --git a/bio_image_unet_amd/csrc/biu_c1.hip b/bio_image_unet_amd/csrc/biu_c1.hip
--- a/bio_image_unet_amd/csrc/biu_c1.hip
+++ b/bio_image_unet_amd/csrc/biu_c1.hip
@@ -23,7 +23,14 @@
     float* partial;
     int ctot;
     const float* bn_scale; const float* bn_shift; const float* bn_slope; const float* bn_cA; const float* bn_cB; const float* bn_cC;
+    unsigned xsamp, ysamp, rsamp;
 };
+
+typedef unsigned v4u_t __attribute__((ext_vector_type(4)));
+constexpr unsigned OOB = 0xffffff00u;
+__device__ __forceinline__ __amdgpu_buffer_rsrc_t sample_rsrc(const char* base, int n, unsigned samp) {
+    return __builtin_amdgcn_make_buffer_rsrc((void*)(base + (size_t)n * samp), 0, (int)samp, 0x00020000);
+}
 
 __device__ __forceinline__ unsigned pack2(float a, float b) {
     typedef __bf16 bf2 __attribute__((ext_vector_type(2)));
@@ -49,19 +56,36 @@
 struct XpRegs { unsigned short v[(Geo<KD, HALF>::HV + NTHR - 1) / NTHR]; unsigned inside; };
 
 template <int KD, int NTHR, int HALF = 0>
-__device__ __forceinline__ void xp_request(const C1Args& a, int n, int d0, int h0, int w0, XpRegs<KD, NTHR, HALF>& xr) {
+struct XpPlan { unsigned crd[(Geo<KD, HALF>::HV + NTHR - 1) / NTHR]; int off[(Geo<KD, HALF>::HV + NTHR - 1) / NTHR]; };
+
+template <int KD, int NTHR, int HALF = 0>
+__device__ __forceinline__ void xp_plan(const C1Args& a, XpPlan<KD, NTHR, HALF>& pl) {
     using G = Geo<KD, HALF>;
     constexpr int NX = (G::HV + NTHR - 1) / NTHR;
-    const int tid = threadIdx.x;
-    xr.inside = 0;
 #pragma unroll
     for (int k = 0; k < NX; ++k) {
-        const int i = tid + NTHR * k;
+        const int i = (int)threadIdx.x + NTHR * k;
         const int hw = i % G::HW, t = i / G::HW;
         const int hh = t % G::HH, hd = t / G::HH;
-        const int gd = d0 + hd - (KD == 3 ? 1 : 0), gh = h0 + hh - 1, gw = w0 + hw - 1;
-        const bool ok = i < G::HV && gd >= 0 && gd < a.D && gh >= 0 && gh < a.H && gw >= 0 && gw < a.W;
-        xr.v[k] = ok ? *(const unsigned short*)(a.x + ((size_t)(((size_t)n * a.D + gd) * a.H + gh) * a.W + gw) * a.xpitch * 2) : (unsigned short)0;
+        pl.crd[k] = (unsigned)hd | ((unsigned)hh << 8) | ((unsigned)hw << 16);
+        pl.off[k] = (((hd - (KD == 3 ? 1 : 0)) * a.H + (hh - 1)) * a.W + (hw - 1)) * a.xpitch * 2;
+    }
+}
+template <int KD, int NTHR, int HALF = 0>
+__device__ __forceinline__ void xp_request(const C1Args& a, const XpPlan<KD, NTHR, HALF>& pl, int n, int d0, int h0, int w0, XpRegs<KD, NTHR, HALF>& xr) {
+    using G = Geo<KD, HALF>;
+    constexpr int NX = (G::HV + NTHR - 1) / NTHR;
+    const __amdgpu_buffer_rsrc_t rs = sample_rsrc(a.x, n, a.xsamp);
+    const unsigned base = (unsigned)((d0 * a.H + h0) * a.W + w0) * (unsigned)(a.xpitch * 2);
+    const int dlo = d0 - (KD == 3 ? 1 : 0), hlo = h0 - 1, wlo = w0 - 1;
+    xr.inside = 0;
+#pragma unroll
+    for (int k = 0; k < NX; ++k) {
+        const unsigned c = pl.crd[k];
+        bool ok = (unsigned)(dlo + (int)(c & 0xffu)) < (unsigned)a.D && (unsigned)(hlo + (int)((c >> 8) & 0xffu)) < (unsigned)a.H &&
+                  (unsigned)(wlo + (int)(c >> 16)) < (unsigned)a.W;
+        if (k == NX - 1) ok = ok && (int)threadIdx.x + NTHR * k < G::HV;
+        xr.v[k] = (unsigned short)__builtin_amdgcn_raw_buffer_load_b16(rs, (int)(ok ? base + (unsigned)pl.off[k] : OOB), 0, 0);
         xr.inside |= ok ? (1u << k) : 0u;
     }
 }
@@ -116,7 +140,7 @@
     unsigned short* lx = (unsigned short*)(smem + G::BV * ROWB);
     float* lred = (float*)(smem + G::BV * ROWB + ((G::HV * 2 + 15) & ~15));
     float* lbias = lred + 4 * 64;
-    const int tid = threadIdx.x, lane = tid & 63, wave = tid >> 6, r = lane & 31, hf = lane >> 5;
+    const int tid = threadIdx.x, lane = tid & 63, wave = __builtin_amdgcn_readfirstlane(tid >> 6), r = lane & 31, hf = lane >> 5;
     lred[tid] = 0.f;
     if (tid < 32) lbias[tid] = (a.bias && tid < a.cout) ? a.bias[a.co0 + tid] : 0.f;
     uint4 wf[2];
@@ -144,42 +168,46 @@
         d0 = (b % a.nbd) * G::TD;
         n = b / a.nbd;
     };
+    floatx16 bias16;
+#pragma unroll
+    for (int e = 0; e < 16; ++e) bias16[e] = lbias[8 * (e >> 2) + 4 * hf + (e & 3)];
+    XpPlan<KD, 256> pl;
+    xp_plan<KD, 256>(a, pl);
     XpRegs<KD, 256> xr;
-    if ((int)blockIdx.x < a.nbricks) { int n, d0, h0, w0; origin_of(blockIdx.x, n, d0, h0, w0); xp_request<KD, 256>(a, n, d0, h0, w0, xr); }
+    if ((int)blockIdx.x < a.nbricks) { int n, d0, h0, w0; origin_of(blockIdx.x, n, d0, h0, w0); xp_request<KD, 256>(a, pl, n, d0, h0, w0, xr); }
+    const unsigned ypb = (unsigned)(a.ypitch * 2);
+    const unsigned lane_off = (unsigned)r * ypb + (unsigned)(a.co0 + 8 * hf) * 2u;
     for (int brick = blockIdx.x; brick < a.nbricks; brick += gridDim.x) {
         int n, d0, h0, w0;
         origin_of(brick, n, d0, h0, w0);
         xp_commit<KD, 256>(a, xr, lx, lxp);
-        if (brick + (int)gridDim.x < a.nbricks) { int n2, d2, h2, w2; origin_of(brick + gridDim.x, n2, d2, h2, w2); xp_request<KD, 256>(a, n2, d2, h2, w2, xr); }
+        if (brick + (int)gridDim.x < a.nbricks) { int n2, d2, h2, w2; origin_of(brick + gridDim.x, n2, d2, h2, w2); xp_request<KD, 256>(a, pl, n2, d2, h2, w2, xr); }
+        const __amdgpu_buffer_rsrc_t rsy = sample_rsrc(a.y, n, a.ysamp);
+        const unsigned brick_off = (unsigned)((d0 * a.H + h0) * a.W + w0) * ypb + lane_off;
+        const bool wok = w0 + r < a.W;
         for (int tile = wave; tile < G::BV / 32; tile += 4) {
             const int v = tile * 32 + r;
-            floatx16 acc;
-#pragma unroll
-            for (int e = 0; e < 16; ++e) acc[e] = lbias[8 * (e >> 2) + 4 * hf + (e & 3)];
+            floatx16 acc = bias16;
 #pragma unroll
             for (int ks = 0; ks < 2; ++ks) {
                 const uint4 bx = *(const uint4*)(lxp + v * ROWB + (16 * ks + 8 * hf) * 2);
                 acc = __builtin_amdgcn_mfma_f32_32x32x16_bf16(__builtin_bit_cast(bf16x8, wf[ks]), __builtin_bit_cast(bf16x8, bx), acc, 0, 0, 0);
             }
-            const int lw = v % G::TW, t = v / G::TW;
-            const int gd = d0 + t / G::TH, gh = h0 + t % G::TH, gw = w0 + lw;
-            const bool vok = gd < a.D && gh < a.H && gw < a.W;
-            char* orow = a.y + ((size_t)(((size_t)n * a.D + gd) * a.H + gh) * a.W + gw) * a.ypitch * 2;
+            const int ld = tile / G::TH, lh = tile % G::TH;
+            const bool vok = wok && d0 + ld < a.D && h0 + lh < a.H;
+            const unsigned ooff = vok ? brick_off + (unsigned)((ld * a.H + lh) * a.W) * ypb : OOB;
 #pragma unroll
             for (int q = 0; q < NQ; ++q) {
                 unsigned a0 = pack2(acc[8 * q + 0], acc[8 * q + 1]), a1 = pack2(acc[8 * q + 2], acc[8 * q + 3]);
                 unsigned b0 = pack2(acc[8 * q + 4], acc[8 * q + 5]), b1 = pack2(acc[8 * q + 6], acc[8 * q + 7]);
                 const u32x2 r0 = __builtin_amdgcn_permlane32_swap(a0, b0, false, false);
                 const u32x2 r1 = __builtin_amdgcn_permlane32_swap(a1, b1, false, false);
-                const uint4 piece = make_uint4(r0[0], r1[0], r0[1], r1[1]);
-                const int c = 16 * q + 8 * hf;
-                if (vok && c < a.cout) {
-                    *(uint4*)(orow + (size_t)(a.co0 + c) * 2) = piece;
-                    float f[8];
-                    unpack8(piece, f);
-#pragma unroll
-                    for (int e = 0; e < 8; ++e) { s1[q][e] += f[e]; s2[q][e] = fmaf(f[e], f[e], s2[q][e]); }
-                }
+                const uint4 piece = vok ? make_uint4(r0[0], r1[0], r0[1], r1[1]) : make_uint4(0, 0, 0, 0);
+                __builtin_amdgcn_raw_buffer_store_b128(v4u_t{piece.x, piece.y, piece.z, piece.w}, rsy, (int)(ooff + 32u * q), 0, 0);
+                float f[8];
+                unpack8(piece, f);
+#pragma unroll
+                for (int e = 0; e < 8; ++e) { s1[q][e] += f[e]; s2[q][e] = fmaf(f[e], f[e], s2[q][e]); }
             }
         }
         __syncthreads();
@@ -203,21 +231,23 @@
     }
 }
 
-template <int KD>
+template <int KD, int PPV, bool KEEP>
 __global__ __launch_bounds__(256, 3) void k_c1_wgrad_mfma(C1Args a) {
     using G = Geo<KD, 1>;
+    static_assert(G::TD == 1 && G::TW == 32, "a brick is TH rows of 32 voxels");
     constexpr int NTHR = 256, NWV = 4;
+    constexpr int NPC = G::BV * PPV / NTHR;
+    constexpr int VSTEP = NTHR / PPV, RSTEP = VSTEP / G::TW;
     extern __shared__ __attribute__((aligned(16))) char smem[];
     char* lxp = smem;
     char* ldy = smem + G::BV * ROWB;
     unsigned short* lx = (unsigned short*)(ldy + G::BV * ROWB);
-    float* lacc = (float*)((char*)lx + ((G::HV * 2 + 15) & ~15));
-    const int tid = threadIdx.x, lane = tid & 63, wave = tid >> 6;
+    float* lsum = (float*)smem;
+    const int tid = threadIdx.x, lane = tid & 63, wave = __builtin_amdgcn_readfirstlane(tid >> 6);
     const bool fused = a.yraw != nullptr;
-    const int ppv = a.cout / 8;
-    const int mypiece = tid % 4;
+    const int mypiece = tid % PPV, v0 = tid / PPV, lw = v0 % G::TW, lh0 = v0 / G::TW;
     float ks[8], kh[8], kl[8], ka[8], kb[8], kc[8];
-    if (fused && mypiece < ppv) {
+    if (fused) {
 #pragma unroll
         for (int e = 0; e < 8; ++e) {
             const int c = a.co0 + mypiece * 8 + e;
@@ -225,17 +255,21 @@
             ka[e] = a.bn_cA[c]; kb[e] = a.bn_cB[c]; kc[e] = a.bn_cC[c];
         }
     }
-    for (int i = tid; i < 32 * 32; i += NTHR) lacc[i] = 0.f;
+    if (PPV < 4)
+        for (int i = tid; i < G::BV * 2; i += NTHR) *(uint4*)(ldy + (i >> 1) * ROWB + 32 + (i & 1) * 16) = make_uint4(0, 0, 0, 0);
     floatx16 acc;
 #pragma unroll
     for (int e = 0; e < 16; ++e) acc[e] = 0.f;
     const int g = lane >> 4, li = lane & 15, qrow = li >> 2, p = li & 3, cg = g & 1, h = g >> 1;
     const int tr_lane = (8 * h + qrow) * ROWB + (16 * cg + 4 * p) * 2;
 
-    constexpr int NPC = G::BV * 4 / NTHR;
+    const unsigned apb = (unsigned)(a.ypitch * 2), rpb = (unsigned)(a.yrawpitch * 2);
+    const unsigned lane_a = (unsigned)(lh0 * a.W + lw) * apb + (unsigned)(a.co0 + mypiece * 8) * 2u;
+    const unsigned lane_r = (unsigned)(lh0 * a.W + lw) * rpb + (unsigned)(a.co0 + mypiece * 8) * 2u;
+    const unsigned step_a = (unsigned)(RSTEP * a.W) * apb, step_r = (unsigned)(RSTEP * a.W) * rpb;
     uint4 pda[NPC], pyr[NPC];
-    size_t pvox[NPC];
-    unsigned pmask = 0;
+    unsigned poff[NPC];
+    __amdgpu_buffer_rsrc_t rsa = sample_rsrc(a.y, 0, 0), rsr = sample_rsrc(a.y, 0, 0);
     auto origin = [&](int brick, int& n, int& d0, int& h0, int& w0) {
         int b = brick;
         w0 = (b % a.nbw) * G::TW; b /= a.nbw;
@@ -243,41 +277,38 @@
         d0 = (b % a.nbd) * G::TD;
         n = b / a.nbd;
     };
-    auto request = [&](int brick) {
-        int n, d0, h0, w0;
-        origin(brick, n, d0, h0, w0);
-        pmask = 0;
+    auto request = [&](int n, int d0, int h0, int w0) {
+        rsa = sample_rsrc(a.y, n, a.ysamp);
+        if (fused) rsr = sample_rsrc(a.yraw, n, a.rsamp);
+        const unsigned vox = (unsigned)((d0 * a.H + h0) * a.W + w0);
+        const unsigned ba = vox * apb + lane_a, br = vox * rpb + lane_r;
+        const bool wok = w0 + lw < a.W;
 #pragma unroll
         for (int k = 0; k < NPC; ++k) {
-            const int v = (tid + NTHR * k) / 4;
-            const int lw = v % G::TW, t = v / G::TW;
-            const int gd = d0 + t / G::TH, gh = h0 + t % G::TH, gw = w0 + lw;
-            pda[k] = make_uint4(0, 0, 0, 0);
-            pyr[k] = make_uint4(0, 0, 0, 0);
-            if (mypiece < ppv && gd < a.D && gh < a.H && gw < a.W) {
-                const size_t vox = (((size_t)n * a.D + gd) * a.H + gh) * a.W + gw;
-                pvox[k] = vox;
-                pda[k] = *(const uint4*)(a.y + (vox * a.ypitch + a.co0 + mypiece * 8) * 2);
-                if (fused) pyr[k] = *(const uint4*)(a.yraw + (vox * a.yrawpitch + a.co0 + mypiece * 8) * 2);
-                pmask |= 1u << k;
+            const bool ok = wok && h0 + lh0 + RSTEP * k < a.H;
+            poff[k] = ok ? ba + step_a * k : OOB;
+            const v4u_t va = __builtin_amdgcn_raw_buffer_load_b128(rsa, (int)poff[k], 0, 0);
+            pda[k] = make_uint4(va[0], va[1], va[2], va[3]);
+            if (fused) {
+                const v4u_t vr = __builtin_amdgcn_raw_buffer_load_b128(rsr, (int)(ok ? br + step_r * k : OOB), 0, 0);
+                pyr[k] = make_uint4(vr[0], vr[1], vr[2], vr[3]);
             }
         }
     };
+    XpPlan<KD, NTHR, 1> pl;
+    xp_plan<KD, NTHR, 1>(a, pl);
     XpRegs<KD, NTHR, 1> xr;
     if ((int)blockIdx.x < a.nbricks) {
-        request(blockIdx.x);
         int n0, d00, h00, w00;
         origin(blockIdx.x, n0, d00, h00, w00);
-        xp_request<KD, NTHR, 1>(a, n0, d00, h00, w00, xr);
+        request(n0, d00, h00, w00);
+        xp_request<KD, NTHR, 1>(a, pl, n0, d00, h00, w00, xr);
     }
     for (int brick = blockIdx.x; brick < a.nbricks; brick += gridDim.x) {
-        int n, d0, h0, w0;
-        origin(brick, n, d0, h0, w0);
 #pragma unroll
         for (int k = 0; k < NPC; ++k) {
-            const int v = (tid + NTHR * k) / 4;
             uint4 out = pda[k];
-            if (fused && ((pmask >> k) & 1u)) {
+            if (fused) {
                 float gg[8], yy[8];
                 unpack8(out, gg);
                 unpack8(pyr[k], yy);
@@ -286,17 +317,17 @@
                     const float dz = gg[e] * (fmaf(ks[e], yy[e], kh[e]) > 0.f ? 1.f : kl[e]);
                     gg[e] = fmaf(ka[e], dz, fmaf(kb[e], yy[e], kc[e]));
                 }
-                out = make_uint4(pack2(gg[0], gg[1]), pack2(gg[2], gg[3]), pack2(gg[4], gg[5]), pack2(gg[6], gg[7]));
-                *(uint4*)(a.y + (pvox[k] * a.ypitch + a.co0 + mypiece * 8) * 2) = out;
-            }
-            *(uint4*)(ldy + v * ROWB + mypiece * 16) = out;
+                out = poff[k] != OOB ? make_uint4(pack2(gg[0], gg[1]), pack2(gg[2], gg[3]), pack2(gg[4], gg[5]), pack2(gg[6], gg[7])) : make_uint4(0, 0, 0, 0);
+                if (!KEEP) __builtin_amdgcn_raw_buffer_store_b128(v4u_t{out.x, out.y, out.z, out.w}, rsa, (int)poff[k], 0, 0);
+            }
+            *(uint4*)(ldy + (v0 + VSTEP * k) * ROWB + mypiece * 16) = out;
         }
         xp_commit<KD, NTHR, 1>(a, xr, lx, lxp);
         if (brick + (int)gridDim.x < a.nbricks) {
-            request(brick + gridDim.x);
             int n2, d2, h2, w2;
             origin(brick + gridDim.x, n2, d2, h2, w2);
-            xp_request<KD, NTHR, 1>(a, n2, d2, h2, w2, xr);
+            request(n2, d2, h2, w2);
+            xp_request<KD, NTHR, 1>(a, pl, n2, d2, h2, w2, xr);
         }
         typedef bf16x4 __attribute__((address_space(3))) * lp;
         for (int ksx = wave; ksx < G::BV / 16; ksx += NWV) {
@@ -314,12 +345,14 @@
     {
         const int j = lane & 31, hf = lane >> 5;
 #pragma unroll
-        for (int e = 0; e < 16; ++e) atomicAdd(&lacc[((e & 3) + 8 * (e >> 2) + 4 * hf) * 32 + j], acc[e]);
+        for (int e = 0; e < 16; ++e) lsum[wave * 1024 + ((e & 3) + 8 * (e >> 2) + 4 * hf) * 32 + j] = acc[e];
     }
     __syncthreads();
-    for (int i = tid; i < G::TAPS * a.cout; i += NTHR) {
-        const int tap = i / a.cout, co = i % a.cout;
-        a.partial[(size_t)blockIdx.x * (G::TAPS * a.cout) + i] = lacc[tap * 32 + co];
+    constexpr int COUT = 8 * PPV;
+    for (int i = tid; i < G::TAPS * COUT; i += NTHR) {
+        const int tap = i / COUT, co = i % COUT;
+        const int s = tap * 32 + co;
+        a.partial[(size_t)blockIdx.x * (G::TAPS * COUT) + i] = (lsum[s] + lsum[1024 + s]) + (lsum[2048 + s] + lsum[3072 + s]);
     }
 }
 
@@ -360,6 +393,8 @@
     if (biu_off("c1_mfma") || dtype != BIU_BF16 || x->c != 1 || dil != 1 || kh != 3 || kw != 3 || (kd != 1 && kd != 3)) return false;
     if (y->c % 16 != 0 || y->c < 16) return false;
     if ((uintptr_t)y->p % 16 || (y->pitch * 2) % 16 || (uintptr_t)x->p % 2) return false;
+    const long long svox = (long long)y->d * y->h * y->w, lim = (1LL << 32) - 65536;
+    if (svox * y->pitch * 2 >= lim || svox * x->pitch * 2 >= lim) return false;
     return nvox(y) < (1LL << 31);
 }
 
@@ -379,6 +414,7 @@
         a.xs = xf->scale; a.xb = xf->shift; a.xl = xf->slope;
     }
     a.N = y->n; a.D = y->d; a.H = y->h; a.W = y->w; a.ctot = y->c; a.partial = bn_partial;
+    a.xsamp = (unsigned)((size_t)y->d * y->h * y->w * x->pitch * 2); a.ysamp = (unsigned)((size_t)y->d * y->h * y->w * y->pitch * 2);
     const int rows = biu_c1m_fwd_rows(y, kd);
     if (kd == 3) bricks_of<3>(a); else bricks_of<1>(a);
     for (int co0 = 0; co0 < y->c;) {
@@ -395,7 +431,7 @@
 size_t biu_c1m_wgrad_workspace(int cout, int kd) { return (size_t)3 * cus() * kd * 9 * 32 * sizeof(float); }
 
 int biu_c1m_wgrad(const biu_act* x, const biu_xform* xf, const biu_act* da, const BnBwdFuse* bn, int kd, float* dw, void* ws, size_t ws_bytes,
-                  hipStream_t st) {
+                  hipStream_t st, bool keep_da) {
     BIU_REQUIRE(ws && ws_bytes >= biu_c1m_wgrad_workspace(da->c, kd), BIU_ERR_WORKSPACE, "c1_wgrad_mfma: workspace too small");
     C1Args a{};
     if (xf && (xf->scale || xf->shift || xf->slope)) {
@@ -404,8 +440,10 @@
     }
     a.x = (const char*)x->p; a.xpitch = x->pitch; a.y = (char*)da->p; a.ypitch = da->pitch;
     a.N = da->n; a.D = da->d; a.H = da->h; a.W = da->w; a.partial = (float*)ws; a.ctot = da->c;
+    const size_t svox = (size_t)da->d * da->h * da->w;
+    a.xsamp = (unsigned)(svox * x->pitch * 2); a.ysamp = (unsigned)(svox * da->pitch * 2);
     if (bn) {
-        a.yraw = (const char*)bn->y->p; a.yrawpitch = bn->y->pitch;
+        a.yraw = (const char*)bn->y->p; a.yrawpitch = bn->y->pitch; a.rsamp = (unsigned)(svox * bn->y->pitch * 2);
         a.bn_scale = bn->scale; a.bn_shift = bn->shift; a.bn_slope = bn->slope; a.bn_cA = bn->cA; a.bn_cB = bn->cB; a.bn_cC = bn->cC;
     }
     const int taps = kd * 9;
@@ -413,12 +451,17 @@
     int grid = 3 * cus();
     if (grid > a.nbricks) grid = a.nbricks;
     const size_t hv = kd == 3 ? (size_t)Geo<3, 1>::HV : (size_t)Geo<1, 1>::HV;
-    const size_t lds = (size_t)2 * 256 * ROWB + ((hv * 2 + 15) & ~(size_t)15) + 32 * 32 * sizeof(float);
+    const size_t lds = (size_t)2 * 256 * ROWB + ((hv * 2 + 15) & ~(size_t)15);
     for (int co0 = 0; co0 < da->c;) {
         const int chunk = (da->c - co0) >= 32 ? 32 : 16;
         a.co0 = co0; a.cout = chunk;
-        if (kd == 3) hipLaunchKernelGGL(k_c1_wgrad_mfma<3>, dim3(grid), dim3(256), lds, st, a);
-        else hipLaunchKernelGGL(k_c1_wgrad_mfma<1>, dim3(grid), dim3(256), lds, st, a);
+        const int form = (kd == 3 ? 4 : 0) | (chunk == 32 ? 2 : 0) | ((bn && keep_da) ? 1 : 0);
+        switch (form) {
+#define BIU_C1_WGRAD(F, KD_, PPV_, KEEP_) case F: hipLaunchKernelGGL((k_c1_wgrad_mfma<KD_, PPV_, KEEP_>), dim3(grid), dim3(256), lds, st, a); break;
+            BIU_C1_WGRAD(0, 1, 2, false) BIU_C1_WGRAD(1, 1, 2, true) BIU_C1_WGRAD(2, 1, 4, false) BIU_C1_WGRAD(3, 1, 4, true)
+            BIU_C1_WGRAD(4, 3, 2, false) BIU_C1_WGRAD(5, 3, 2, true) BIU_C1_WGRAD(6, 3, 4, false) BIU_C1_WGRAD(7, 3, 4, true)
+#undef BIU_C1_WGRAD
+        }
         BIU_CHECK_LAUNCH("c1_wgrad_mfma");
         hipLaunchKernelGGL(k_c1m_finalize, dim3(taps * chunk), dim3(256), 0, st, (const float*)ws, grid, taps, chunk, co0, dw);
         BIU_CHECK_LAUNCH("c1_wgrad_mfma_finalize");
diff --git a/bio_image_unet_amd/csrc/biu_internal.h b/bio_image_unet_amd/csrc/biu_internal.h
--- a/bio_image_unet_amd/csrc/biu_internal.h
+++ b/bio_image_unet_amd/csrc/biu_internal.h
@@ -156,4 +156,4 @@
 int biu_c1m_fwd(const biu_act* x, const biu_xform* xf, const float* w, const float* bias, int kd, const biu_act* y, float* bn_partial, hipStream_t st);
 size_t biu_c1m_wgrad_workspace(int cout, int kd);
 int biu_c1m_wgrad(const biu_act* x, const biu_xform* xf, const biu_act* da, const BnBwdFuse* bn, int kd, float* dw, void* ws, size_t ws_bytes,
-                  hipStream_t st);
+                  hipStream_t st, bool keep_da = false);
diff --git a/bio_image_unet_amd/engine.py b/bio_image_unet_amd/engine.py
--- a/bio_image_unet_amd/engine.py
+++ b/bio_image_unet_amd/engine.py
@@ -29,6 +29,7 @@
 _NO_CAPTURE_FORK = _disabled("capturefork")
 _NO_SIDE_CHAIN = _disabled("sidechain")
 _NO_PREPACK = _disabled("prepack")
+_NO_C1_KEEP = _disabled("c1keep")
 _SIDE_WGRAD_VOX = int(os.environ.get("BIU_SIDE_WGRAD_VOX", str(4 * 32 ** 3)))
 
 class Buf:
@@ -491,6 +492,11 @@
         elif self.fold_wg:
             check(lib.biu_upconv_bwd_weight_bn(self.fold_src.a(), self.fold_src.xf(), y.g(), y.a(), scale, shift, slope, _ptr(A), _ptr(B),
                                                _ptr(Cc), _ptr(dw), _ptr(eng.ws), eng.ws_bytes, eng.dtype, st), "upconv_bwd_weight_bn")
+        elif isinstance(self.xin, Act) and not eng.wants_grad(self.xin) and self._c1_keep_ok(eng):
+            keep = not _NO_C1_KEEP and eng.trace is None
+            fn = lib.biu_conv_bwd_weight_bn_keep if keep else lib.biu_conv_bwd_weight_bn
+            check(fn(self.xin.a(), self.xin.xf(), y.g(), y.a(), scale, shift, slope, _ptr(A), _ptr(B), _ptr(Cc), self.kd, self.kh, self.kw,
+                     self.dil, _ptr(dw), _ptr(eng.ws), eng.ws_bytes, eng.dtype, st), "conv_bwd_weight_bn_keep" if keep else "conv_bwd_weight_bn")
         elif self.kd == 3 and eng.tdtype == torch.bfloat16 and y.nvox <= _SIDE_WGRAD_VOX and eng.chain_stream() is not None:
             side = eng.chain_stream()
             check(lib.biu_bn_bwd_apply(y.g(), y.a(), scale, shift, slope, _ptr(A), _ptr(B), _ptr(Cc), y.g(), eng.dtype, st), "bn_bwd_apply")
@@ -550,6 +556,13 @@
                                             self.xin.g(), int(self.xin.g_written()), _ptr(eng.ws), eng.ws_bytes, eng.dtype, st), "conv_bwd_data")
             self.xin.mark_g()
 
+    def _c1_keep_ok(self, eng) -> bool:
+        ok = self.__dict__.get("_c1_keep")
+        if ok is None:
+            ok = self._c1_keep = bool(lib.biu_conv_bwd_weight_bn_keep_ok(self.xin.a(), self.y.g(), self.y.a(), self.kd, self.kh, self.kw, self.dil,
+                                                                         eng.dtype))
+        return ok
+
     def red_buffer(self, eng, kd, transposed) -> torch.Tensor:
         need = lib.biu_bwd_data_bnred_floats(self.y.a(), kd, transposed)
         if self.red_partial is None or self.red_partial.numel() < need:
diff --git a/include/biu.h b/include/biu.h
--- a/include/biu.h
+++ b/include/biu.h
@@ -88,6 +88,13 @@
                            const float* scale, const float* shift, const float* slope, const float* coefA,
                            const float* coefB, const float* coefC, int kd, int kh, int kw, int dilation,
                            float* dw, void* ws, size_t ws_bytes, int dtype, biu_stream stream);
+
+int biu_conv_bwd_weight_bn_keep_ok(const biu_act* x, const biu_act* da, const biu_act* y, int kd, int kh, int kw, int dilation,
+                                   int dtype);
+int biu_conv_bwd_weight_bn_keep(const biu_act* x, const biu_xform* xf, const biu_act* da, const biu_act* y,
+                                const float* scale, const float* shift, const float* slope, const float* coefA,
+                                const float* coefB, const float* coefC, int kd, int kh, int kw, int dilation,
+                                float* dw, void* ws, size_t ws_bytes, int dtype, biu_stream stream);
 
 #define BIU_BN_MAX_PARTIALS 1024
 int biu_bn_stats(const biu_act* y, float* partial, int* nblk_out, int dtype, biu_stream stream);
```

Measured after the change: 748.3 million voxels/s (median of 6 runs). Within noise of the previous version (+0.9%).
